# mozack/vdjer

Hardware: AMD Instinct MI355X
Metric: M paired-reads/sec (k-mer build + contig score), IgH 50bp PE (higher is better)
Workload: dtype u8/u64 (2-bit packed bases, integer counts)

## Files before the change

### vdjer_amd/csrc/vdjx_common.h

```cpp
#pragma once

#include <hip/hip_runtime.h>
#include <stdint.h>
#include <stddef.h>
#include <string>
#include <vector>
#include <chrono>
#include <map>
#include <mutex>
#include <utility>

#include "../../include/vdjx.h"
#include "vdjx_env.h"

typedef unsigned long long u64;
typedef unsigned int u32;
typedef unsigned __int128 u128;

#define VDJX_WAVE 64

#define RI_R1 1u
#define RI_RC 2u
#define RI_RCA 4u
#define RI_RCB 8u
#define VDJX_RI_SLOT_WORDS(W) ((W) == 2 ? 4 : 8)
#define RI_TAB_EPOCH_SHIFT 25
#define RI_ENT_NONE 0x3FFFFFFu
#define RI_ENT_MAXCNT 255u
__host__ __device__ inline unsigned long long ri_entry(unsigned y, unsigned z, unsigned fl, unsigned cnt) {
	return (unsigned long long) y | ((unsigned long long) z << 26) | ((unsigned long long) fl << 52) | ((unsigned long long) cnt << 56);
}

void vdjx_set_error(const char* fmt, ...);
inline void vdjx_clear_errors() { (void) hipGetLastError(); }

#define HIP_TRY(expr)                                                                            \
	do {                                                                                         \
		hipError_t e_ = (expr);                                                                  \
		if (e_ != hipSuccess) {                                                                  \
			vdjx_set_error("%s failed: %s (%s:%d)", #expr, hipGetErrorString(e_), __FILE__, __LINE__); \
			return VDJX_EHIP;                                                                    \
		}                                                                                        \
	} while (0)

struct vdjx_prof_entry {
	double ms = 0;
	uint64_t launches = 0;
};

struct vdjx_arena {
	char* base = nullptr;
	size_t reserved = 0, mapped = 0;
	std::vector<std::pair<void*, size_t>> pieces;
	size_t gran = 0;
	int mode = 0;
	struct chunk { char* p; size_t cap; };
	std::vector<chunk> chunks;
	size_t cur = 0;
	size_t used = 0;
	void* alloc(size_t bytes);
	void reset();
	void release(bool for_good = false);
	struct mark_t { size_t cur, used; };
	mark_t mark() const { return {cur, used}; }
	void release_to(mark_t m);
	bool grow(size_t upto);
};

struct vdjx_shard;

#define VDJX_HPIN_BYTES 16384
#define VDJX_HPIN_SYNC_BYTES ((64 * 16 + 2) * 8)
#define VDJX_HPIN_ROOT_RUN 3072
static_assert(VDJX_HPIN_ROOT_RUN * 4 >= VDJX_HPIN_SYNC_BYTES + 64 && VDJX_HPIN_ROOT_RUN * 4 + 4 <= VDJX_HPIN_BYTES, "h_pin layout");

struct vdjx_block_cache {
	struct blk { char* p; size_t cap; };
	std::vector<blk> free_list;
	hipError_t acquire(size_t need, char** out, size_t* cap);
	void release(char* p, size_t cap);
	void drop();
	static void discard(char* p) { if (p) (void) hipFree(p); }
};

struct vdjx_kept {
	void* p = nullptr;
	size_t bytes = 0;
	const bool pinned;
	u32 allocs = 0;
	explicit vdjx_kept(bool pinned_ = false) : pinned(pinned_) {}
	vdjx_kept(const vdjx_kept&) = delete;
	vdjx_kept& operator=(const vdjx_kept&) = delete;
	template <typename T> T* as() const { return (T*) p; }
	hipError_t reserve(size_t need, size_t margin) {
		if (need <= bytes) return hipSuccess;
		release();
		const hipError_t e = pinned ? hipHostMalloc(&p, need + margin, hipHostMallocDefault) : hipMalloc(&p, need + margin);
		if (e != hipSuccess) { p = nullptr; return e; }
		bytes = need + margin;
		allocs++;
		return hipSuccess;
	}
	void release() {
		if (p) (void) (pinned ? hipHostFree(p) : hipFree(p));
		p = nullptr;
		bytes = 0;
	}
};
template <typename T> struct vdjx_buf : vdjx_kept {
	using vdjx_kept::vdjx_kept;
	operator T*() const { return (T*) p; }
	template <typename U> explicit operator U*() const { return (U*) p; }
};
enum vdjx_kept_tag { VDJX_KEPT_INDEX, VDJX_KEPT_RESULT, VDJX_KEPT_OTHER };

struct vdjx_recset {
	vdjx_buf<uint8_t> d_cols;
	bool loaded = false;
	int ncls = 0;
	std::vector<u32> rec[2];
	std::vector<u64> at[2];
	std::vector<u32> len[2];
	size_t given = 0;
};

struct vdjx_ctx {
	int device = 0;
	vdjx_arena arena;
	vdjx_block_cache blocks;
	vdjx_arena shard_arena;
	hipStream_t ri_stream = nullptr;
	hipEvent_t ev_ri_go = nullptr;
	vdjx_arena ri_arena;
	struct vdjx_ri_job* ri_job = nullptr;
	vdjx_shard* live_shard = nullptr;
	hipStream_t stream = nullptr;
	hipStream_t copy_stream = nullptr;
	hipStream_t pairs_stream = nullptr;
	vdjx_buf<void> h_pin{true};
	vdjx_buf<void> d_stage[2];
	hipEvent_t ev_copied[2] = {nullptr, nullptr}, ev_packed[2] = {nullptr, nullptr};
	bool profiling = false;
	std::string prof_only;
	std::vector<std::string> prof_names;
	std::map<std::string, vdjx_prof_entry> prof;
	struct pending_ev { std::string name; hipEvent_t a, b; };
	std::vector<pending_ev> prof_pending;
	std::vector<hipEvent_t> ev_free;
	vdjx_buf<u32> d_vbits, d_jbits;
	bool anchors_loaded = false;
	u32 sub_tuples_set = 0;
	vdjx_buf<u32> d_anchor_tmp;
	vdjx_buf<char> d_vtext;
	vdjx_buf<u32> d_line_off;
	vdjx_buf<u32> d_seed_code;
	vdjx_buf<u32> d_seed_pos;
	size_t n_lines = 0, n_seeds = 0;
	int vk = 0;
	std::vector<u32> h_line_off;
	const vdjx_pool* ri_pool = nullptr;
	vdjx_buf<void> d_ri_tab;
	u32 ri_tab_mask = 0;
	u32 ri_tab_epoch = 0;
	bool ri_canon = false;
	vdjx_buf<u32> d_ri_start;
	vdjx_buf<u32> d_ri_cnt1;
	vdjx_buf<u32> d_ri_recs;
	vdjx_buf<u64> d_ri_csr8;
	vdjx_buf<u32> d_ri_csr_pair;
	vdjx_buf<u32> d_pair_r2;
	vdjx_buf<u32> d_ri_dstart;
	vdjx_buf<u64> d_ri_d8;
	std::vector<std::pair<const char*, size_t>> host_blocks;
	std::mutex host_blocks_mu;
	uint64_t me_key = 0;
	const void* me_src = nullptr;
	vdjx_buf<void> me_pairs;
	vdjx_buf<void> me_hit;
	vdjx_buf<void> wp_buf;
	size_t wp_n = 0;
	std::vector<u64> wp_off;
	std::vector<u32> wp_cnt;
	vdjx_buf<void> me_dense;
	size_t me_gathered_cap = 0;
	std::vector<u64> me_cnt;
	vdjx_buf<void> h_plan{true};
	vdjx_buf<void> h_res{true};
	vdjx_buf<void> me_book;
	size_t me_nsl = 0;
	u32 me_slice_hits = 0;
	hipEvent_t ev_gathered = nullptr;
	hipStream_t up_stream = nullptr;
	hipEvent_t ev_up[5] = {};
	hipEvent_t ev_pairs_copied = nullptr;
	uint32_t root_dp_hint = 0;
	hipEvent_t ev_plan = nullptr;
	bool root_pending = false;
	const vdjx_graph* root_pending_g = nullptr;
	int root_pending_thr = 0;
	uint32_t root_pending_first = 0, root_pending_stride = 1, root_pending_ahead = 0;
	bool root_pending_by_wave = false;
	uint32_t* root_pending_ids = nullptr;
	uint8_t* root_pending_out = nullptr;
	hipEvent_t ev_root_done = nullptr;
	vdjx_buf<char> d_sam_names;
	vdjx_buf<u64> d_sam_noff;
	u32 sam_pairs = 0;
	vdjx_buf<void> d_sam_text;
	vdjx_buf<void> h_sam_text{true};
	vdjx_buf<void> d_sam_keys, d_sam_lens;
	vdjx_buf<void> h_sam_merge{true};
	u32 n_pairs = 0, n_classes = 0;
	vdjx_recset germline, constant, dsegment;
	std::map<std::string, uint64_t> stats;
	template <typename F> void each_kept(F f) {
		vdjx_kept* const index[] = {&d_ri_tab, &d_ri_start, &d_ri_cnt1, &d_ri_recs, &d_ri_csr8, &d_ri_csr_pair, &d_ri_dstart, &d_ri_d8, &d_pair_r2};
		vdjx_kept* const result[] = {&wp_buf, &me_pairs, &me_hit, &me_dense, &me_book, &d_sam_text, &h_sam_text, &d_sam_keys, &d_sam_lens};
		vdjx_kept* const other[] = {&h_pin, &d_stage[0], &d_stage[1], &d_vbits, &d_jbits, &d_anchor_tmp, &d_vtext, &d_line_off, &d_seed_code, &d_seed_pos,
		                            &h_plan, &h_res, &d_sam_names, &d_sam_noff, &h_sam_merge, &germline.d_cols, &constant.d_cols, &dsegment.d_cols};
		for (vdjx_kept* b : index) f(*b, VDJX_KEPT_INDEX);
		for (vdjx_kept* b : result) f(*b, VDJX_KEPT_RESULT);
		for (vdjx_kept* b : other) f(*b, VDJX_KEPT_OTHER);
	}
};

#define VDJX_LONG_W 5
#define VDJX_LONG_M 3
struct vdjx_pool {
	vdjx_ctx* ctx = nullptr;
	int device = 0;
	size_t n_primary = 0, n_records = 0;
	int rl = 0;
	int qstride = 0;
	int W = 2, M = 1, ob = 6;
	bool sym = false;
	char* d_block = nullptr;
	size_t block_cap = 0;
	u64* d_bases = nullptr;
	u64* d_nmask = nullptr;
	u64* d_lowq = nullptr;
	const uint8_t* d_quals = nullptr;
	const uint8_t* d_quals2 = nullptr;
	size_t q_split = ~(size_t) 0;
	u32* pending_bad = nullptr;
};

struct vdjx_graph {
	vdjx_ctx* ctx = nullptr;
	int device = 0;
	int k = 0;
	size_t n = 0, pre_nodes = 0;
	size_t export_bytes = 0;
	char* d_block = nullptr;
	size_t block_cap = 0;
	u64* d_first_inst = nullptr;
	u32 *d_gcnt = nullptr, *d_freq = nullptr, *d_to_ids = nullptr, *d_from_ids = nullptr;
	uint8_t *d_hv = nullptr, *d_hj = nullptr, *d_to_deg = nullptr, *d_from_deg = nullptr;
	char* d_kmers = nullptr;
	u32* d_roots = nullptr;
	size_t n_roots = 0;
};

bool vdjx_ctx_alive(const vdjx_ctx* c);
int vdjx_ri_join(vdjx_ctx* c);
void vdjx_ri_open_gate(vdjx_ctx* c);
bool vdjx_host_block_holds(vdjx_ctx* c, const void* p, size_t bytes);
int vdjx_map_emit_device(vdjx_ctx* c, const char* contigs, size_t n, int len, uint64_t* offsets, const vdjx_pair** d_pairs);

struct vdjx_work {
	vdjx_ctx* c;
	vdjx_arena* ar;
	explicit vdjx_work(vdjx_ctx* ctx) : c(ctx), ar(&ctx->arena) {}
	vdjx_work(vdjx_ctx* ctx, vdjx_arena* arena) : c(ctx), ar(arena) {}
	~vdjx_work() { ar->reset(); }
	template <typename T> hipError_t alloc(T** out, size_t n) {
		*out = (T*) ar->alloc((n ? n : 1) * sizeof(T));
		return *out ? hipSuccess : hipErrorOutOfMemory;
	}
	vdjx_arena::mark_t mark() const { return ar->mark(); }
	void release_to(vdjx_arena::mark_t m) { ar->release_to(m); }
};

struct vdjx_prof_scope {
	vdjx_ctx* c;
	const char* name;
	hipEvent_t a = nullptr, b = nullptr;
	vdjx_prof_scope(vdjx_ctx* ctx, const char* nm);
	~vdjx_prof_scope();
};
void vdjx_prof_collect(vdjx_ctx* ctx, bool force = true);

int vdjx_sort_pairs(vdjx_work& db, hipStream_t st, u64* k_in, u64* k_out, u32* v_in, u32* v_out, u32 n, unsigned end_bit);
int vdjx_sort_pairs_raw(void* tmp, size_t* tmp_bytes, hipStream_t st, u64* k_in, u64* k_out, u32* v_in, u32* v_out, u32 n, unsigned end_bit);

struct vdjx_laps {
	vdjx_ctx* c;
	bool on;
	std::chrono::steady_clock::time_point t;
	explicit vdjx_laps(vdjx_ctx* ctx) : c(ctx) { static const bool e = vdjx_env_set("VDJX_LAPS"); on = e; if (on) t = std::chrono::steady_clock::now(); }
	void mark(const char* name) {
		if (!on) return;
		const auto n = std::chrono::steady_clock::now();
		c->stats[std::string("us_") + name] += (uint64_t) std::chrono::duration_cast<std::chrono::microseconds>(n - t).count();
		t = n;
	}
};

struct vdjx_qrows {
	const uint8_t* a; const uint8_t* b; size_t split; int stride;
	__host__ __device__ inline const uint8_t* row(size_t rec) const { return rec < split ? a + rec * (size_t) stride : b + (rec - split) * (size_t) stride; }
};
__host__ __device__ inline u64 vdjx_mix64(u64 x) {
	u64 z = x + 0x9E3779B97F4A7C15ull;
	z = (z ^ (z >> 30)) * 0xBF58476D1CE4E5B9ull;
	z = (z ^ (z >> 27)) * 0x94D049BB133111EBull;
	return z ^ (z >> 31);
}
__host__ __device__ inline u64 vdjx_mix(u64 lo, u64 hi) {
	u64 x = lo ^ (hi * 0x9E3779B97F4A7C15ull) ^ 0x2545F4914F6CDD1Dull;
	x ^= x >> 32; x *= 0xD6E8FEB86659FD93ull;
	x ^= x >> 32; x *= 0xD6E8FEB86659FD93ull;
	x ^= x >> 32;
	return x;
}

__host__ __device__ inline u64 vdjx_bucket_mix(u64 lo, u64 hi) {
	u32 c = (u32) hi ^ ((u32) (hi >> 32) << 26);
	u32 h = (c ^ (c >> 15)) * 0x9E3779B1u;
	h ^= h >> 15;
	h = (h ^ (u32) lo) * 0x85EBCA6Bu;
	h ^= h >> 13;
	const u32 b = (u32) (lo >> 32);
	h = (h ^ b ^ (b >> 16)) * 0xC2B2AE35u;
	h ^= h >> 16;
	h *= 0x27D4EB2Fu;
	h ^= h >> 15;
	return (u64) h << 32;
}

template <int W>
__device__ inline u64 ri_hash(const u64* __restrict__ w) {
	if (W == 2) return vdjx_mix(w[1], w[0]);
	u64 h = vdjx_mix(w[1], w[0]);
#pragma unroll
	for (int i = 2; i < W; i += 2) h = vdjx_mix(h ^ w[i], i + 1 < W ? w[i + 1] : 0ull);
	return h;
}

__host__ __device__ inline void vdjx_kmer_at(u64 bhi, u64 blo, int rl, int k, int o, u64& khi, u64& klo) {
	u128 b = ((u128) bhi << 64) | blo;
	int sh = 2 * (rl - k - o);
	u128 v = b >> sh;
	if (k < 64) v &= (((u128) 1) << (2 * k)) - 1;
	khi = (u64) (v >> 64);
	klo = (u64) v;
}

__device__ inline void vdjx_wave_lds_fence() {
	__builtin_amdgcn_fence(__ATOMIC_ACQ_REL, "wavefront");
	__builtin_amdgcn_wave_barrier();
}

__device__ inline void vdjx_kmer_at_lane(u64 bhi, u64 blo, int rl, int k, int o, u64& khi, u64& klo) {
	const u32 sh = (u32) (2 * (rl - k - o));
	const u64 big = 0ull - (u64) (sh >> 6);
	const u64 x_lo = (bhi & big) | (blo & ~big), x_hi = bhi & ~big;
	const u32 s = sh & 63u;
	u64 lo = (x_lo >> s) | ((x_hi << 1) << (63u - s));
	u64 hi = x_hi >> s;
	if (k < 32) { lo &= (1ull << (2 * k)) - 1ull; hi = 0; }
	else if (k < 64) hi &= (1ull << (2 * k - 64)) - 1ull;
	khi = hi;
	klo = lo;
}

// ... 224 lines not shown
```

### vdjer_amd/csrc/vdjx_kmer.hip

```cpp
#include "vdjx_common.h"
#include "vdjx_scan.h"
#include "vdjx_part.h"

#include <algorithm>
#include <numeric>
#include <type_traits>
#include <string.h>
#include <stdlib.h>

#define HIST_THREADS 512
#define HIST_BLOCKS 512u
#define LOCAL_SLOTS 2048u
#define K3_SUB_TUPLES g_sub_tuples
__device__ u32 g_sub_tuples = 262144u;
#define NONE32 0xFFFFFFFFu
#define INST_MASK 0x7FFFFFFFu

struct RecView {
	u64 bhi, blo, nm, lq;
};

__device__ inline RecView load_rec(const u64* __restrict__ bases, const u64* __restrict__ nmask,
                                   const u64* __restrict__ lowq, size_t r) {
	RecView v;
	const ulonglong2 b = ((const ulonglong2*) bases)[r];
	v.bhi = b.x; v.blo = b.y;
	v.nm = nmask[r];
	v.lq = lowq ? lowq[r] : 0ull;
	return v;
}

__global__ void k_pick_u32(const u32* __restrict__ src, u32 step, u32 n, u32* __restrict__ out) {
	const u32 i = blockIdx.x * blockDim.x + threadIdx.x;
	if (i < n) out[i] = src[(size_t) i * step];
}

template <typename THI, u32 SLOTS>
__device__ inline int lds_insert(u64* s_klo, THI* s_khi, u64 lo, THI hi, u32 h) {
	const THI EMPTY = (THI) ~(THI) 0, LOCKED = (THI) (EMPTY - 1);
	u32 slot = h & (SLOTS - 1);
	u32 probes = 0;
	while (probes < SLOTS) {
		THI cur = vdjx_peek_acquire(&s_khi[slot]);
		if (cur == EMPTY) {
			THI old = atomicCAS(&s_khi[slot], EMPTY, LOCKED);
			if (old == EMPTY) {
				vdjx_poke(&s_klo[slot], lo);
				vdjx_poke_release(&s_khi[slot], hi);
				return (int) slot;
			}
			cur = old;
			if (cur != LOCKED) cur = vdjx_peek_acquire(&s_khi[slot]);
		}
		if (cur == LOCKED) continue;
		if (cur == hi && vdjx_peek(&s_klo[slot]) == lo) return (int) slot;
		slot = (slot + 1) & (SLOTS - 1);
		probes++;
	}
	return -1;
}

template <typename THI, u32 SLOTS>
__device__ inline int lds_lookup(const u64* s_klo, const THI* s_khi, u64 lo, THI hi, u32 h) {
	const THI EMPTY = (THI) ~(THI) 0;
	u32 slot = h & (SLOTS - 1);
	for (u32 probes = 0; probes < SLOTS; probes++) {
		THI cur = s_khi[slot];
		if (cur == EMPTY) return -1;
		if (cur == hi && s_klo[slot] == lo) return (int) slot;
		slot = (slot + 1) & (SLOTS - 1);
	}
	return -1;
}

#define INST_BITS 38
#define INST_MASK64 ((1ull << INST_BITS) - 1ull)
#define NONE64 0xFFFFFFFFFFFFFFFFull

struct Tup16 {
	u64 lo, x;
	typedef u32 hi_t;
	__device__ inline u64 hi() const { return x >> INST_BITS; }
	__device__ inline u64 inst() const { return x & INST_MASK64; }
	__device__ static inline Tup16 make(u64 lo, u64 hi, u64 inst) { Tup16 t; t.lo = lo; t.x = (hi << INST_BITS) | inst; return t; }
	__device__ static inline Tup16 load(const Tup16* p) { const ulonglong2 v = *(const ulonglong2*) p; Tup16 t; t.lo = v.x; t.x = v.y; return t; }
	__device__ static inline void store(Tup16* p, const Tup16& t) { *(ulonglong2*) p = make_ulonglong2(t.lo, t.x); }
};
struct Tup24 {
	u64 lo, h, i;
	typedef u64 hi_t;
	__device__ inline u64 hi() const { return h; }
	__device__ inline u64 inst() const { return i; }
	__device__ static inline Tup24 make(u64 lo, u64 hi, u64 inst) { Tup24 t; t.lo = lo; t.h = hi; t.i = inst; return t; }
	__device__ static inline Tup24 load(const Tup24* p) { return *p; }
	__device__ static inline void store(Tup24* p, const Tup24& t) { *p = t; }
};

__device__ inline u64 vdjx_clean_offsets(u64 bad, int k, int P) {
	u64 inv = bad;
	int cur = 1;
	while (cur * 2 <= k) { inv |= inv >> cur; cur *= 2; }
	inv |= inv >> (k - cur);
	return ~inv & (P >= 64 ? ~0ull : (1ull << P) - 1ull);
}

#define GL_WAVE_BYTES 3072u

#define GL_ROW_LONG (VDJX_LONG_W + 2)
#define GL_WAVE_BYTES_LONG (64u * GL_ROW_LONG * 8u + 2048u)
struct GateView { u64 bhi, blo, bad; };
__device__ inline GateView load_gate(const u64* __restrict__ bases, const u64* __restrict__ gate, size_t r) {
	GateView v;
	const ulonglong2 b = ((const ulonglong2*) bases)[r];
	v.bhi = b.x; v.blo = b.y;
	v.bad = gate[r];
	return v;
}
__device__ inline vdjx_mask3 load_gate3(const u64* __restrict__ gate, size_t r) {
	vdjx_mask3 b;
	b.w0 = gate[r * VDJX_LONG_M]; b.w1 = gate[r * VDJX_LONG_M + 1]; b.w2 = gate[r * VDJX_LONG_M + 2];
	return b;
}
__device__ inline vdjx_mask3 load_bad3(const u64* __restrict__ nmask, const u64* __restrict__ lowq, size_t r) {
	vdjx_mask3 b;
	b.w0 = nmask[r * VDJX_LONG_M] | (lowq ? lowq[r * VDJX_LONG_M] : 0ull);
	b.w1 = nmask[r * VDJX_LONG_M + 1] | (lowq ? lowq[r * VDJX_LONG_M + 1] : 0ull);
	b.w2 = nmask[r * VDJX_LONG_M + 2] | (lowq ? lowq[r * VDJX_LONG_M + 2] : 0ull);
	return b;
}
__device__ inline void stage_row_long(u64* row, const u64* __restrict__ bases, size_t r) {
#pragma unroll
	for (int w = 0; w < VDJX_LONG_W; w++) row[w] = bases[r * VDJX_LONG_W + w];
	row[VDJX_LONG_W] = 0; row[VDJX_LONG_W + 1] = 0;
}

__device__ inline bool sym_canonical(const ulonglong2 f, int rl, int k, int o, u64& khi, u64& klo) {
	u64 xh, xl, yh, yl;
	vdjx_kmer_at_lane(f.x, f.y, rl, k, o, xh, xl);
	vdjx_kmer_rc(xh, xl, k, yh, yl);
	const bool flip = yh < xh || (yh == xh && yl < xl);
	khi = flip ? yh : xh;
	klo = flip ? yl : xl;
	return flip;
}

template <bool LONG, bool SYM = false>
__global__ __launch_bounds__(HIST_THREADS) void k_gated_hist(const u64* __restrict__ bases, const u64* __restrict__ nmask,
                                                             const u64* __restrict__ lowq, size_t R, int rl, int k, u32 nb_bits,
                                                             size_t rpb, u32* __restrict__ bucket_cnt, u32 dbg_in) {
#ifdef VDJX_ABLATE
	const u32 dbg = dbg_in;
#else
	const u32 dbg = 0u;
#endif
	u32 sink = 0;
	extern __shared__ __attribute__((aligned(16))) u32 hist[];
	const u32 NB = 1u << nb_bits;
	for (u32 i = threadIdx.x; i < NB; i += HIST_THREADS) hist[i] = 0;
	__syncthreads();
	static_assert(!(LONG && SYM), "SYM is the short-read form");
	uint8_t* wv = (uint8_t*) (hist + NB) + (threadIdx.x >> 6) * (LONG ? GL_WAVE_BYTES_LONG : GL_WAVE_BYTES);
	ulonglong2* wb = (ulonglong2*) wv;
	u64* wrow = (u64*) wv;
	uint16_t* wl = (uint16_t*) (wv + (LONG ? 64u * GL_ROW_LONG * 8u : 1024u));
	const u32 lane = threadIdx.x & 63u;
	const size_t r0 = (size_t) blockIdx.x * rpb;
	const size_t r1 = r0 + rpb < R ? r0 + rpb : R;
	const int P = rl - k + 1;
	for (size_t rb = r0; rb < r1; rb += HIST_THREADS) {
		const size_t r = rb + threadIdx.x;
		u64 G = 0;
		vdjx_mask3 bad{~0ull, ~0ull, ~0ull};
		if (r < r1) {
			if (LONG) { bad = load_gate3(lowq, r); stage_row_long(wrow + lane * GL_ROW_LONG, bases, r); }
			else {
				const GateView v = load_gate(bases, lowq, SYM ? 2 * r : r);
				G = vdjx_clean_offsets(v.bad, k, P);
				wb[lane] = make_ulonglong2(v.bhi, v.blo);
			}
		}
		constexpr int LSTEP = 16;
		for (int ob = 0; ob < P; ob += LSTEP) {
			const u32 g = LONG ? vdjx_clean16(bad, ob, k, P) : (u32) (G >> ob) & 0xFFFFu;
			const u32 c = (u32) __popc(g);
			const u32 incl = (u32) vdjx_wave_scan_add((int) c);
			const u32 total = (u32) __builtin_amdgcn_readlane((int) incl, 63);
			if (dbg == 1) { sink += incl; continue; }
			if (!total) continue;
			u32 at = incl - c;
			for (u32 gg = g; gg; gg &= gg - 1) wl[at++] = (uint16_t) ((lane << (LONG ? 8 : 6)) | (u32) (ob + __builtin_ctz(gg)));
			vdjx_wave_lds_fence();
			if (dbg == 2) { sink += wl[lane]; vdjx_wave_lds_fence(); continue; }
			for (u32 i = lane; i < total; i += 64) {
				const u32 e = wl[i];
				u64 khi, klo;
				if (LONG) vdjx_kmer_at_words(wrow + (e >> 8) * GL_ROW_LONG, k, (int) (e & 255u), khi, klo);
				else if (SYM) (void) sym_canonical(wb[e >> 6], rl, k, (int) (e & 63u), khi, klo);
				else {
					const ulonglong2 bb = wb[e >> 6];
					vdjx_kmer_at_lane(bb.x, bb.y, rl, k, (int) (e & 63u), khi, klo);
				}
				if (dbg == 3) { sink += (u32) (vdjx_bucket_mix(klo, khi) >> (64 - nb_bits)); continue; }
				atomicAdd(&hist[(u32) (vdjx_bucket_mix(klo, khi) >> (64 - nb_bits))], 1u);
			}
			vdjx_wave_lds_fence();
		}
	}
	__syncthreads();
	if (dbg) { if (sink == 0x12345u) bucket_cnt[0] = sink; return; }
	for (u32 i = threadIdx.x; i < NB; i += HIST_THREADS) if (hist[i]) atomicAdd(&bucket_cnt[i], hist[i]);
}

template <typename TUP> struct TupBucket {
	u32 shift, mask;
	__device__ inline u32 operator()(const TUP& t) const { return (u32) (vdjx_bucket_mix(t.lo, t.hi()) >> shift) & mask; }
};

#define PARTR_STAGE_BYTES 98304u
template <typename TUP, bool LONG, bool SYM = false>
__global__ __launch_bounds__(PART_THREADS) void k_part_records_g(const u64* __restrict__ bases, const u64* __restrict__ nmask,
                                                                 const u64* __restrict__ lowq, size_t R, u64 rec_base, int rl, int k,
                                                                 u32 shift, u32 nbk, size_t rpb, u32 rr0, u32* __restrict__ gcur,
                                                                 TUP* __restrict__ out) {
	extern __shared__ __attribute__((aligned(16))) uint8_t smem[];
	TUP* stage = (TUP*) smem;
	u32* desc = (u32*) (smem + PARTR_STAGE_BYTES);
	__shared__ part_round pr;
	__shared__ u32 s_n;
	constexpr u32 ROUND = PARTR_STAGE_BYTES / sizeof(TUP);
	constexpr int OB = LONG ? 8 : 6;
	const int P = rl - k + 1;
	const u32 rr_min = ROUND / (u32) P;
	u32 rr = rr0 > rr_min ? rr0 : rr_min;
	const u32 mask = nbk - 1;
	const u32 lane = threadIdx.x & 63u, wave = threadIdx.x >> 6;
	static_assert(!(LONG && SYM), "SYM is the short-read form");
	uint8_t* wv = smem + wave * (LONG ? GL_WAVE_BYTES_LONG : GL_WAVE_BYTES);
	ulonglong2* wb = (ulonglong2*) wv;
	u64* wrow = (u64*) wv;
	uint16_t* wl = (uint16_t*) (wv + (LONG ? 64u * GL_ROW_LONG * 8u : 1024u));
	const size_t r0 = (size_t) blockIdx.x * rpb;
	const size_t r1 = r0 + rpb < R ? r0 + rpb : R;
	size_t rs = r0;
	while (rs < r1) {
		const size_t re = rs + rr < r1 ? rs + rr : r1;
		if (threadIdx.x == 0) s_n = 0;
		pr.begin(nbk);
		for (size_t rb = rs; rb < re; rb += PART_THREADS) {
			const size_t r = rb + threadIdx.x;
			u64 G = 0;
			vdjx_mask3 bad{~0ull, ~0ull, ~0ull};
			if (r < re) {
				if (LONG) { bad = load_gate3(lowq, r); stage_row_long(wrow + lane * GL_ROW_LONG, bases, r); }
				else {
					const GateView v = load_gate(bases, lowq, SYM ? 2 * r : r);
					G = vdjx_clean_offsets(v.bad, k, P);
					wb[lane] = make_ulonglong2(v.bhi, v.blo);
				}
			}
			const u32 loc0 = (u32) (rb - rs) + wave * 64u;
			constexpr int LSTEP = 16;
			for (int ob = 0; ob < P; ob += LSTEP) {
				const u32 g = LONG ? vdjx_clean16(bad, ob, k, P) : (u32) (G >> ob) & 0xFFFFu;
				const u32 c = (u32) __popc(g);
				const u32 incl = (u32) vdjx_wave_scan_add((int) c);
				const u32 total = (u32) __builtin_amdgcn_readlane((int) incl, 63);
				if (!total) continue;
				u32 at = incl - c;
				for (u32 gg = g; gg; gg &= gg - 1) wl[at++] = (uint16_t) ((lane << OB) | (u32) (ob + __builtin_ctz(gg)));
				vdjx_wave_lds_fence();
				u32 dbase = 0;
				if (lane == 0) dbase = atomicAdd(&s_n, total);
				dbase = (u32) __builtin_amdgcn_readlane((int) dbase, 0);
				for (u32 i = lane; i < total; i += 64) {
					const u32 e = wl[i];
					u64 khi, klo;
					if (LONG) vdjx_kmer_at_words(wrow + (e >> 8) * GL_ROW_LONG, k, (int) (e & 255u), khi, klo);
					else if (SYM) (void) sym_canonical(wb[e >> 6], rl, k, (int) (e & 63u), khi, klo);
					else {
						const ulonglong2 bb = wb[e >> 6];
						vdjx_kmer_at_lane(bb.x, bb.y, rl, k, (int) (e & 63u), khi, klo);
					}
					const u32 b = (u32) (vdjx_bucket_mix(klo, khi) >> shift) & mask;
					pr.count(b);
					if (dbase + i < ROUND) desc[dbase + i] = ((loc0 + (e >> OB)) << (OB + 10)) | ((e & ((1u << OB) - 1u)) << 10) | b;
				}
				vdjx_wave_lds_fence();
			}
		}
		__syncthreads();
		if (s_n > ROUND) {
			rr = rr / 2 > rr_min ? rr / 2 : rr_min;
			__syncthreads();
			continue;
		}
		const u32 n = pr.reserve(nbk, gcur);
		for (u32 i = threadIdx.x; i < n; i += PART_THREADS) {
			const u32 d = desc[i];
			const size_t r = rs + (d >> (OB + 10));
			const u32 o = (d >> 10) & ((1u << OB) - 1u);
			u64 khi, klo;
			u64 inst = ((rec_base + (u64) r) << OB) | (u64) o;
			if (LONG) vdjx_kmer_at_words(bases + r * VDJX_LONG_W, k, (int) o, khi, klo);
			else if (SYM) {
				const bool flip = sym_canonical(((const ulonglong2*) bases)[2 * r], rl, k, (int) o, khi, klo);
				inst = flip ? ((rec_base + 2 * (u64) r + 1) << OB) | (u64) (rl - k - (int) o) : ((rec_base + 2 * (u64) r) << OB) | (u64) o;
			} else {
				const ulonglong2 bb = ((const ulonglong2*) bases)[r];
				vdjx_kmer_at_lane(bb.x, bb.y, rl, k, (int) o, khi, klo);
			}
			TUP::store(&stage[pr.slot(d & 1023u)], TUP::make(klo, khi, inst));
		}
		__syncthreads();
		pr.flush(stage, n, out, TupBucket<TUP>{shift, mask});
		rs = re;
	}
}

template <typename TUP>
__global__ __launch_bounds__(512) void k_seg_hist_g(const TUP* __restrict__ in, const u32* __restrict__ seg_start, u32 seg_shift, u32 slices,
                                                    u32 shift, u32 sub_bits, u32* __restrict__ fine_cnt) {
	__shared__ u32 h[PART_MAXB];
	const u32 nbk = 1u << sub_bits;
	for (u32 i = threadIdx.x; i < nbk; i += 512) h[i] = 0;
	__syncthreads();
	size_t t0, t1;
	const u32 seg = part_slice(seg_start, seg_shift, slices, t0, t1);
	for (size_t t = t0 + threadIdx.x; t < t1; t += 512) {
		const TUP x = TUP::load(&in[t]);
		atomicAdd(&h[(u32) (vdjx_bucket_mix(x.lo, x.hi()) >> shift) & (nbk - 1)], 1u);
	}
	__syncthreads();
	for (u32 i = threadIdx.x; i < nbk; i += 512) if (h[i]) atomicAdd(&fine_cnt[((size_t) seg << sub_bits) | i], h[i]);
}

#ifndef RD_THREADS
#define RD_THREADS 768
#define RD_UNR 4
#define RD_WAVES 6
#endif
#define RD_SLOTS 2048u
#define RD_SLOT_BITS 11
#define RD_PQ 4096u
#define RD_LI 512u
#define RD_LROWS 128u
#define RD_MAXLOW 11u
#define ST_CAND 1u
#define ST_MULTI 2u
#define ST_QOK 4u
#define ST_QOK_R 8u
#define ST_ID_SHIFT 8
#define ST_NOID 0xFFFFFFu

struct SurvOutG { u64* lo; u64* hi; u32* gcnt; u64* gfirst; u32* n; u32 cap; u32* n_real; };
#define GC_SHADOW 0x80000000u
#define GC_MASK 0x7FFFFFFFu

__device__ inline bool reads_equal(const u64* __restrict__ bases, const u64* __restrict__ nmask, int rl, u64 a, u64 b) {
	if (rl <= VDJX_SHORT_READ_LEN) {
		const ulonglong2 x = ((const ulonglong2*) bases)[a];
		const ulonglong2 y = ((const ulonglong2*) bases)[b];
		return x.x == y.x && x.y == y.y && nmask[a] == nmask[b];
	}
	u64 d = 0;
#pragma unroll
	for (int w = 0; w < VDJX_LONG_W; w++) d |= bases[a * VDJX_LONG_W + w] ^ bases[b * VDJX_LONG_W + w];
#pragma unroll
	for (int w = 0; w < VDJX_LONG_M; w++) d |= nmask[a * VDJX_LONG_M + w] ^ nmask[b * VDJX_LONG_M + w];
	return d == 0;
}

__device__ inline u32 rd_hash(u64 lo, u64 hi) {
	u32 x = (u32) lo ^ ((u32) (lo >> 32) * 0x9E3779B1u) ^ (((u32) hi ^ (u32) (hi >> 32) * 0x27D4EB2Fu) * 0x85EBCA6Bu);
	x ^= x >> 15; x *= 0xC2B2AE35u; x ^= x >> 13;
	return x;
}

__device__ inline u32 rd_count_min(u32* cnt, u64* mn, u32 idx, u64 val, bool active) {
	u32 c0 = 0;
	const u64 act = __ballot(active);
	if (act) {
		const int leader = __ffsll((long long) act) - 1;
		const u32 lidx = (u32) __builtin_amdgcn_readlane((int) idx, leader);
		const bool same = active && idx == lidx;
		const u64 m = __ballot(same);
		if (__popcll(m) >= 8) {
			const u32 hi_min = vdjx_wave_min(same ? (u32) (val >> 32) : 0xFFFFFFFFu);
			const u32 lo_min = vdjx_wave_min(same && (u32) (val >> 32) == hi_min ? (u32) val : 0xFFFFFFFFu);
			u32 old = 0;
			if (__lane_id() == leader) {
				old = atomicAdd(&cnt[lidx], (u32) __popcll(m));
				atomicMin((unsigned long long*) &mn[lidx], ((unsigned long long) hi_min << 32) | lo_min);
			}
			old = (u32) __builtin_amdgcn_readlane((int) old, leader);
			if (same) c0 = old + (u32) __popcll(m & ((1ull << __lane_id()) - 1ull));
			active = active && !same;
		}
	}
	if (active) { c0 = atomicAdd(&cnt[idx], 1u); atomicMin((unsigned long long*) &mn[idx], (unsigned long long) val); }
	return c0;
}

__global__ __launch_bounds__(1024) void k_bucket_order(const u32* __restrict__ bucket_start, u32 NB, u32* __restrict__ order) {
	__shared__ u32 cls_cnt[33], cls_at[33];
	if (threadIdx.x < 33) cls_cnt[threadIdx.x] = 0;
	__syncthreads();
	for (u32 b = threadIdx.x; b < NB; b += 1024) {
		const u32 n = bucket_start[b + 1] - bucket_start[b];
		atomicAdd(&cls_cnt[n ? 32u - (u32) __builtin_clz(n) : 0u], 1u);
	}
	__syncthreads();
	if (threadIdx.x == 0) { u32 at = 0; for (int cl = 32; cl >= 0; cl--) { cls_at[cl] = at; at += cls_cnt[cl]; } }
	__syncthreads();
	for (u32 b = threadIdx.x; b < NB; b += 1024) {
		const u32 n = bucket_start[b + 1] - bucket_start[b];
		order[atomicAdd(&cls_at[n ? 32u - (u32) __builtin_clz(n) : 0u], 1u)] = b;
	}
}

template <typename TUP, bool SYM = false>
__global__ __launch_bounds__(RD_THREADS, sizeof(TUP) == 16 ? RD_WAVES : RD_WAVES / 2) void k_gated_reduce(const TUP* __restrict__ tup, const u32* __restrict__ bucket_start,
                                                             const u64* __restrict__ bases, const u64* __restrict__ nmask,
                                                             vdjx_qrows quals, int rl, int ob, int k, u64 rec_base,
                                                             u32 mf, u32 cmin, u32 mqq, u32 tlow, SurvOutG so,
                                                             u64* __restrict__ g_distinct, u32* __restrict__ g_err, u32 dbg_in,
                                                             const u32* __restrict__ order) {
#ifdef VDJX_ABLATE
	const u32 dbg = dbg_in;
#else
	const u32 dbg = dbg_in == 9u ? 9u : 0u;
#endif
	typedef typename TUP::hi_t THI;
	__shared__ u64 s_klo[RD_SLOTS];
	__shared__ THI s_khi[RD_SLOTS];
	__shared__ u64 s_first[RD_SLOTS];
	__shared__ u32 s_cnt[RD_SLOTS], s_state[RD_SLOTS];
	__shared__ u32 pq[RD_PQ];
	__shared__ u64 low_inst[RD_LI];
	__shared__ u32 low_n[RD_LROWS];
	__shared__ unsigned short low_slot[RD_LROWS];
	__shared__ u32 s_over, s_ndist, s_nlow, s_npq, s_nsurv, s_base, s_nreal;
	const THI EMPTY = (THI) ~(THI) 0;
	const u32 b = order ? order[blockIdx.x] : blockIdx.x;
	const u32 base = bucket_start[b];
	const u32 n = bucket_start[b + 1] - base;
	const u32 tid = threadIdx.x;
	if (n == 0) return;
	const TUP* T = tup + base;
	const u32 om = (1u << ob) - 1u;
	const u32 per_low = tlow > 1 ? (tlow - 1 < RD_MAXLOW ? tlow - 1 : RD_MAXLOW) : 1;
	const u32 lrows = RD_LI / per_low < RD_LROWS ? RD_LI / per_low : RD_LROWS;
	u32 S = 1;
	while ((u64) S * K3_SUB_TUPLES < n) S <<= 1;
	u32 ndist_total = 0;
	bool verify = S > 1;
	for (;;) {
		if (tid == 0) { s_over = 0; s_ndist = 0; }
		__syncthreads();
		for (u32 s = 0; s < S; s++) {
			for (u32 i = tid; i < RD_SLOTS; i += RD_THREADS) { s_khi[i] = EMPTY; s_cnt[i] = 0; s_first[i] = NONE64; s_state[i] = 0; }
			if (tid == 0) { s_nlow = 0; s_npq = (n >> (32 - RD_SLOT_BITS) || dbg == 9) ? RD_PQ + 1 : 0; s_nsurv = 0; s_nreal = 0; }
			__syncthreads();
			for (u32 t0 = 0; t0 < n; t0 += RD_UNR * RD_THREADS) {
				TUP r_t[RD_UNR];
#pragma unroll
				for (int j = 0; j < RD_UNR; j++) {
					const u32 t = t0 + j * RD_THREADS + tid;
					if (t < n) r_t[j] = TUP::load(&T[t]);
				}
#pragma unroll
				for (int j = 0; j < RD_UNR; j++) {
					const u32 t = t0 + j * RD_THREADS + tid;
					int slot = -1;
					if (t < n) {
						const u32 h = rd_hash(r_t[j].lo, r_t[j].hi());
						if (!(S > 1 && ((h >> 12) & (S - 1)) != s)) {
							slot = lds_insert<THI, RD_SLOTS>(s_klo, s_khi, r_t[j].lo, (THI) r_t[j].hi(), h);
							if (slot < 0) s_over = 1;
						}
					}
					const bool live = slot >= 0 && !verify;
					const u64 inst = r_t[j].inst();
					const u32 c0 = rd_count_min(s_cnt, s_first, (u32) (live ? slot : 0), inst, live);
					bool list = false;
					if (live) {
						u32 st = vdjx_peek(&s_state[slot]);
						if (!(st & ST_MULTI)) {
							const u64 f = vdjx_peek(&s_first[slot]);
							if (f != NONE64 && (f >> ob) != (inst >> ob)) {
								const u32 o1 = (u32) inst & om, o0 = (u32) f & om;
								const u32 d = o1 > o0 ? o1 - o0 : o0 - o1;
								if (d && d < (u32) k && !vdjx_kmer_has_period(r_t[j].hi(), r_t[j].lo, k, d)) { atomicOr(&s_state[slot], ST_MULTI); st |= ST_MULTI; }
							}
						}
						list = !((st & ST_MULTI) && c0 + 1 >= tlow);
					}
					const u32 qi = vdjx_wave_inc(&s_npq, list);
					if (list && qi < RD_PQ) pq[qi] = (t << RD_SLOT_BITS) | (u32) slot;
				}
			}
			__syncthreads();
			if (s_over || verify) { if (s_over) break; continue; }
			if (dbg == 1) return;
			for (u32 i = tid; i < RD_SLOTS; i += RD_THREADS) {
				if (s_khi[i] == EMPTY) continue;
				atomicAdd(&s_ndist, SYM ? 2u : 1u);
				const u32 c = s_cnt[i];
				if (c >= cmin) s_state[i] = (s_state[i] & ST_MULTI) | ST_CAND | ((c < tlow ? atomicAdd(&s_nlow, 1u) : ST_NOID) << ST_ID_SHIFT);
			}
			__syncthreads();
			const u32 nlow = s_nlow;
			const bool listed = s_npq <= RD_PQ;
			const u32 nscan = listed ? s_npq : n;
			for (u32 l0 = 0; l0 == 0 || l0 < nlow; l0 += lrows) {
				for (u32 i = tid; i < RD_LROWS; i += RD_THREADS) low_n[i] = 0;
				__syncthreads();
				for (u32 e = tid; e < nscan; e += RD_THREADS) {
					u32 slot, t;
					TUP x;
					if (listed) {
						slot = pq[e] & (RD_SLOTS - 1); t = pq[e] >> RD_SLOT_BITS;
						if (!(vdjx_peek(&s_state[slot]) & ST_CAND)) continue;
						x = TUP::load(&T[t]);
					} else {
						x = TUP::load(&T[e]);
						const u32 h = rd_hash(x.lo, x.hi());
						if (S > 1 && ((h >> 12) & (S - 1)) != s) continue;
						const int sl = lds_lookup<THI, RD_SLOTS>(s_klo, s_khi, x.lo, (THI) x.hi(), h);
						if (sl < 0) continue;
						slot = (u32) sl;
					}
					const u32 st = vdjx_peek(&s_state[slot]);
					if (!(st & ST_CAND)) continue;
					const u64 inst = x.inst(), fi = s_first[slot];
					const u32 lid = st >> ST_ID_SHIFT;
					if (lid != ST_NOID && lid >= l0 && lid < l0 + lrows) {
						const u32 pos = atomicAdd(&low_n[lid - l0], 1u);
						if (pos < per_low) low_inst[(lid - l0) * per_low + pos] = inst;
						low_slot[lid - l0] = (unsigned short) slot;
					}
					if (l0 == 0 && !(st & ST_MULTI) && (inst >> ob) != (fi >> ob)) {
						const u32 o1 = (u32) inst & om, o0 = (u32) fi & om;
						const u32 d = o1 > o0 ? o1 - o0 : o0 - o1;
						if ((d && d < (u32) k && !vdjx_kmer_has_period(x.hi(), x.lo, k, d))
						    || !reads_equal(bases, nmask, rl, (inst >> ob) - rec_base, (fi >> ob) - rec_base)) atomicOr(&s_state[slot], ST_MULTI);
					}
				}
				__syncthreads();
				if (dbg == 4) return;
				const u32 rows = nlow - l0 < lrows ? nlow - l0 : lrows;
				const u32 lane = tid & 63u;
				for (u32 r = tid >> 6; r < (nlow ? rows : 0u); r += RD_THREADS / 64) {
					const u32 slot = low_slot[r], cnt = low_n[r];
					const u64 fi = s_first[slot];
					u32 qv[RD_MAXLOW];
#pragma unroll
					for (u32 i = 0; i < RD_MAXLOW; i++) {
						qv[i] = 33u;
						if (i < cnt && i < per_low) {
							const u64 inst = low_inst[r * per_low + i];
							const uint8_t* q = quals.row((inst >> ob) - rec_base) + (inst == fi ? 0u : (u32) inst & om);
							if (lane < (u32) k) qv[i] = q[lane];
						}
					}
					u32 sum = 0;
#pragma unroll
					for (u32 i = 0; i < RD_MAXLOW; i++) sum += (u32) (uint8_t) (qv[i] - 33u);
					const bool lowq = lane < (u32) k && sum < mqq;
					if (!__ballot(lowq) && lane == 0) atomicOr(&s_state[slot], ST_QOK);
					if (SYM) {
						u64 fr = NONE64;
#pragma unroll
						for (u32 i = 0; i < RD_MAXLOW; i++)
							if (i < cnt && i < per_low) { const u64 m = vdjx_inst_mirror(low_inst[r * per_low + i], ob, rl, k); fr = m < fr ? m : fr; }
#pragma unroll
						for (u32 i = 0; i < RD_MAXLOW; i++) {
							qv[i] = 33u;
							if (i < cnt && i < per_low) {
								const u64 inst = vdjx_inst_mirror(low_inst[r * per_low + i], ob, rl, k);
								const uint8_t* q = quals.row((inst >> ob) - rec_base) + (inst == fr ? 0u : (u32) inst & om);
								if (lane < (u32) k) qv[i] = q[lane];
							}
						}
						u32 sum_r = 0;
#pragma unroll
						for (u32 i = 0; i < RD_MAXLOW; i++) sum_r += (u32) (uint8_t) (qv[i] - 33u);
						const bool lowq_r = lane < (u32) k && sum_r < mqq;
						if (!__ballot(lowq_r) && lane == 0) atomicOr(&s_state[slot], ST_QOK_R);
					}
				}
				__syncthreads();
			}
			if (dbg == 5) return;
			for (u32 i = tid; i < RD_SLOTS; i += RD_THREADS) {
				const u32 st = s_state[i];
				bool keep = false, keep_r = false;
				if (st & ST_CAND) {
					const u32 craw = s_cnt[i];
					const u32 c = craw > 32765u ? 32765u : craw;
					keep = c >= mf && (st & ST_MULTI) && (craw >= tlow || (st & ST_QOK));
					if (SYM) keep_r = c >= mf && (st & ST_MULTI) && (craw >= tlow || (st & ST_QOK_R));
				}
				if (SYM) {
					s_state[i] = (keep || keep_r) ? (atomicAdd(&s_nsurv, 2u) << 2) | (u32) keep | ((u32) keep_r << 1) : NONE32;
					if (keep || keep_r) atomicAdd(&s_nreal, (u32) keep + (u32) keep_r);
				} else s_state[i] = keep ? atomicAdd(&s_nsurv, 1u) : NONE32;
			}
			__syncthreads();
			if (tid == 0) { s_base = s_nsurv ? atomicAdd(so.n, s_nsurv) : 0; if (SYM && s_nreal) atomicAdd(so.n_real, s_nreal); }
			__syncthreads();
			for (u32 i = tid; i < RD_SLOTS; i += RD_THREADS) {
				if (s_state[i] == NONE32) continue;
				u32 pos = s_base + (SYM ? s_state[i] >> 2 : s_state[i]);
				const u32 cgo = s_cnt[i] > 32765u ? 32765u : s_cnt[i];
				if (pos < so.cap) {
					so.lo[pos] = s_klo[i];
					so.hi[pos] = (u64) s_khi[i];
					so.gcnt[pos] = cgo | (SYM && !(s_state[i] & 1u) ? GC_SHADOW : 0u);
					so.gfirst[pos] = s_first[i];
				}
				if (SYM) {
					pos += 1u;
					if (pos < so.cap) {
						u64 rh, rlo;
						vdjx_kmer_rc((u64) s_khi[i], s_klo[i], k, rh, rlo);
						so.lo[pos] = rlo;
						so.hi[pos] = rh;
						so.gcnt[pos] = cgo | (!(s_state[i] & 2u) ? GC_SHADOW : 0u);
						so.gfirst[pos] = vdjx_inst_mirror(s_first[i], ob, rl, k);
					}
				}
			}
			__syncthreads();
		}
		__syncthreads();
		if (s_over) {
			if (S >= (1u << 20)) { if (tid == 0) atomicAdd(g_err, 1u); break; }
			S <<= 1;
			verify = true;
			__syncthreads();
			continue;
		}
		if (verify) { verify = false; __syncthreads(); continue; }
		ndist_total = s_ndist;
		break;
	}
	if (tid == 0) atomicAdd(&g_distinct[(b & 63u) * 16u], (u64) ndist_total);
}

struct Partial { u64 lo, hi; u32 cg, h; u64 fg; };
#define PART_FLAG 0x80000000u
#define CNT_CAP 32765u
struct PartialS { u64 lo, hic, fgh, fgr; };
static_assert(sizeof(PartialS) == sizeof(Partial), "vdjx_shard_record_bytes(0) is one number");
#define PS_H_BITS 26
#define PS_MAX_SPLIT (1u << (PS_H_BITS - 12))
__device__ inline u64 ps_hi(const PartialS& p) { return p.hic & 0xFFFFFFFFFFFFull; }
__device__ inline u32 ps_cg(const PartialS& p) { const u32 c = (u32) (p.hic >> 48); return (c & 0x7FFFu) | ((c & 0x8000u) ? PART_FLAG : 0u); }
__device__ inline u64 ps_fg(const PartialS& p) { return p.fgh & INST_MASK64; }
__device__ inline u32 ps_h(const PartialS& p) { return (u32) (p.fgh >> INST_BITS); }
#define NEED_SEQ 1u
#define NEED_Q 2u
#define PID_MASK 0x3FFFFFFFu
#define REPLY_KQ 52
#define REPLY_BYTES 408

#define LG_THREADS 768
#define LG_UNR 4
#define LG_FLAG 0x80000000u
#define LG_NOLIST 0x7FFFFFFFu
template <typename TUP, bool SYM = false>
__global__ __launch_bounds__(LG_THREADS, sizeof(TUP) == 16 ? 6 : 3) void k_gated_local(const TUP* __restrict__ tup, const u32* __restrict__ bucket_start,
                                                            const u64* __restrict__ bases, const u64* __restrict__ nmask, u64 rec_base, int k, int rl, int ob,
                                                            u32 tlow, Partial* __restrict__ sparse_g, u32* __restrict__ sparse_ref,
                                                            u32* __restrict__ nd_g, u64* __restrict__ low_inst, u32* __restrict__ g_err,
                                                            const u32* __restrict__ order) {
	typedef typename TUP::hi_t THI;
	const size_t obase = (size_t) bucket_start[order ? order[blockIdx.x] : blockIdx.x];
	__shared__ u64 s_klo[LOCAL_SLOTS];
	__shared__ THI s_khi[LOCAL_SLOTS];
	__shared__ u64 s_mg[LOCAL_SLOTS];
	__shared__ u32 s_cg[LOCAL_SLOTS], s_st[LOCAL_SLOTS];
	__shared__ u32 pq[RD_PQ];
	__shared__ u32 s_ng, s_nlow, s_over, s_npq;
	static_assert(LOCAL_SLOTS == (1u << RD_SLOT_BITS), "list entries carry the slot in RD_SLOT_BITS bits");
	const THI EMPTY = (THI) ~(THI) 0;
	const u32 b = order ? order[blockIdx.x] : blockIdx.x;
	const u32 base = bucket_start[b];
	const u32 n = bucket_start[b + 1] - base;
	const u32 tid = threadIdx.x;
	const u32 om = (1u << ob) - 1u;
	if (n == 0) { if (tid == 0) nd_g[b] = 0; return; }
	const TUP* T = tup + base;
	u32 S = 1;
	while ((u64) S * K3_SUB_TUPLES < n) S <<= 1;
	for (;;) {
		if (tid == 0) { s_ng = 0; s_nlow = 0; s_over = 0; }
		for (u32 s = 0; s < S; s++) {
			for (u32 i = tid; i < LOCAL_SLOTS; i += LG_THREADS) { s_khi[i] = EMPTY; s_cg[i] = 0; s_mg[i] = NONE64; s_st[i] = 0; }
			if (tid == 0) s_npq = n >> (32 - RD_SLOT_BITS) ? RD_PQ + 1 : 0;
			__syncthreads();
			for (u32 t0 = 0; t0 < n; t0 += LG_UNR * LG_THREADS) {
				TUP r_t[LG_UNR];
#pragma unroll
				for (int j = 0; j < LG_UNR; j++) {
					const u32 t = t0 + j * LG_THREADS + tid;
					if (t < n) r_t[j] = TUP::load(&T[t]);
				}
#pragma unroll
				for (int j = 0; j < LG_UNR; j++) {
					const u32 t = t0 + j * LG_THREADS + tid;
					int slot = -1;
					if (t < n) {
						const u32 h = rd_hash(r_t[j].lo, r_t[j].hi());
						if (!(S > 1 && ((h >> 12) & (S - 1)) != s)) {
							slot = lds_insert<THI, LOCAL_SLOTS>(s_klo, s_khi, r_t[j].lo, (THI) r_t[j].hi(), h);
							if (slot < 0) s_over = 1;
						}
					}
					const bool live = slot >= 0;
					const u64 inst = r_t[j].inst();
					const u32 c0 = rd_count_min(s_cg, s_mg, (u32) (live ? slot : 0), inst, live);
					bool list = false;
					if (live) {
						u32 st = vdjx_peek(&s_st[slot]);
						if (!(st & LG_FLAG)) {
							const u64 f = vdjx_peek(&s_mg[slot]);
							if (f != NONE64 && (f >> ob) != (inst >> ob)) {
								const u32 o1 = (u32) inst & om, o0 = (u32) f & om;
								const u32 d = o1 > o0 ? o1 - o0 : o0 - o1;
								if (d && d < (u32) k && !vdjx_kmer_has_period(r_t[j].hi(), r_t[j].lo, k, d)) { atomicOr(&s_st[slot], LG_FLAG); st |= LG_FLAG; }
							}
						}
						list = !((st & LG_FLAG) && c0 + 1 >= tlow);
					}
					const u32 qi = vdjx_wave_inc(&s_npq, list);
					if (list && qi < RD_PQ) pq[qi] = (t << RD_SLOT_BITS) | (u32) slot;
				}
			}
			__syncthreads();
			if (s_over) break;
			for (u32 i = tid; i < LOCAL_SLOTS; i += LG_THREADS) {
				const u32 cg = s_cg[i];
				s_st[i] = (s_st[i] & LG_FLAG) | ((cg && cg < tlow) ? atomicAdd(&s_nlow, cg) : LG_NOLIST);
			}
			__syncthreads();
			const bool listed = s_npq <= RD_PQ;
			const u32 nscan = listed ? s_npq : n;
			for (u32 e = tid; e < nscan; e += LG_THREADS) {
				u32 slot;
				TUP x;
				if (listed) {
					slot = pq[e] & (LOCAL_SLOTS - 1);
					const u32 st0 = vdjx_peek(&s_st[slot]);
					if ((st0 & LG_NOLIST) == LG_NOLIST && (st0 & LG_FLAG)) continue;
					x = TUP::load(&T[pq[e] >> RD_SLOT_BITS]);
				} else {
					x = TUP::load(&T[e]);
					const u32 h = rd_hash(x.lo, x.hi());
					if (S > 1 && ((h >> 12) & (S - 1)) != s) continue;
					const int sl = lds_lookup<THI, LOCAL_SLOTS>(s_klo, s_khi, x.lo, (THI) x.hi(), h);
					if (sl < 0) continue;
					slot = (u32) sl;
				}
				const u32 st = vdjx_peek(&s_st[slot]);
				const u32 loff = st & LG_NOLIST;
				const u64 inst = x.inst();
				u32 cg = vdjx_peek(&s_cg[slot]);
				if (loff != LG_NOLIST) {
					cg &= 0xFFFFu;
					low_inst[base + loff + (atomicAdd(&s_cg[slot], 0x10000u) >> 16)] = inst;
				}
				if (cg < 2 || (st & LG_FLAG)) continue;
				const u64 fi = s_mg[slot];
				const u64 rec = (inst >> ob) - rec_base, frec = (fi >> ob) - rec_base;
				if (rec != frec) {
					const u32 o1 = (u32) inst & om, o0 = (u32) fi & om;
					const u32 d = o1 > o0 ? o1 - o0 : o0 - o1;
					if (d && d < (u32) k && !vdjx_kmer_has_period(x.hi(), x.lo, k, d)) atomicOr(&s_st[slot], LG_FLAG);
					else if (!reads_equal(bases, nmask, rl, rec, frec)) atomicOr(&s_st[slot], LG_FLAG);
				}
			}
			__syncthreads();
			for (u32 i = tid; i < LOCAL_SLOTS; i += LG_THREADS) {
				if (s_khi[i] == EMPTY) continue;
				const u32 st = s_st[i];
				const u32 loff = st & LG_NOLIST;
				const u32 cg = loff != LG_NOLIST ? s_cg[i] & 0xFFFFu : s_cg[i];
				Partial p;
				p.lo = s_klo[i]; p.hi = (u64) s_khi[i];
				p.fg = s_mg[i];
				p.cg = (cg > CNT_CAP ? CNT_CAP : cg) | ((st & LG_FLAG) ? PART_FLAG : 0u);
				p.h = rd_hash(p.lo, p.hi);
				const u32 gi = atomicAdd(&s_ng, 1u);
				sparse_ref[obase + gi] = loff != LG_NOLIST ? base + loff : NONE32;
				if (SYM) {
					u64 fr = vdjx_inst_mirror(p.fg, ob, rl, k);
					if (loff != LG_NOLIST)
						for (u32 j = 0; j < cg; j++) { const u64 m = vdjx_inst_mirror(low_inst[base + loff + j], ob, rl, k); fr = m < fr ? m : fr; }
					PartialS q;
					q.lo = p.lo;
					q.hic = p.hi | ((u64) ((p.cg & 0x7FFFu) | ((p.cg & PART_FLAG) ? 0x8000u : 0u)) << 48);
					q.fgh = p.fg | ((u64) (p.h & ((1u << PS_H_BITS) - 1u)) << INST_BITS);
					q.fgr = fr;
					((PartialS*) sparse_g)[obase + gi] = q;
				} else sparse_g[obase + gi] = p;
			}
			__syncthreads();
		}
		if (!s_over) break;
		S <<= 1;
		if (S > (1u << 20)) { if (tid == 0) atomicAdd(g_err, 1u); break; }
		__syncthreads();
	}
	if (tid == 0) nd_g[b] = s_over ? 0 : s_ng;
}

__global__ __launch_bounds__(256) void k_compact_partials(const Partial* __restrict__ sparse, const u32* __restrict__ sparse_ref,
                                                          const u32* __restrict__ bucket_start, const u32* __restrict__ nd,
                                                          const u32* __restrict__ dstart, Partial* __restrict__ dense, u32* __restrict__ dense_ref,
                                                          const u32* __restrict__ scan, int ob, bool sym) {
	const u32 b = blockIdx.x;
	const u64* src = (const u64*) (sparse + (size_t) bucket_start[b]);
	u64* dst = (u64*) (dense + dstart[b]);
	const u32 m = nd[b];
	const u64 om = (1ull << ob) - 1ull;
	for (u32 i = threadIdx.x; i < m * 4; i += 256) {
		u64 v = src[i];
		if (scan) {
			if ((i & 3u) == 3u) v = ((u64) scan[v >> ob] << ob) | (v & om);
			else if (sym && (i & 3u) == 2u) { const u64 f = v & INST_MASK64; v = (v & ~INST_MASK64) | ((u64) scan[f >> ob] << ob) | (f & om); }
		}
		dst[i] = v;
	}
	for (u32 i = threadIdx.x; i < m; i += 256) dense_ref[dstart[b] + i] = sparse_ref[(size_t) bucket_start[b] + i];
}

__global__ __launch_bounds__(1024) void k_seg_offsets(const u32* __restrict__ seg_cnt, const u32* __restrict__ src_base, u32 G, u32 NBo,
                                                      u32* __restrict__ seg_off) {
	__shared__ u32 tmp[16];
	const u32 s = blockIdx.x;
	const u32* cnt = seg_cnt + (size_t) s * NBo;
	u32* off = seg_off + (size_t) s * (NBo + 1);
	const u32 per = (NBo + 1023) / 1024;
	const u32 lo = threadIdx.x * per;
	const u32 hi = lo + per < NBo ? lo + per : NBo;
	u32 sum = 0;
	for (u32 i = lo; i < hi; i++) sum += cnt[i];
	u32 total;
	u32 run = src_base[s] + vdjx_block_scan(sum, tmp, total);
	for (u32 i = lo; i < hi; i++) { off[i] = run; run += cnt[i]; }
	if (threadIdx.x == 1023) off[NBo] = src_base[s] + total;
}

struct PendOut { u64* lo; u64* hi; u32* cg; u64* mg; u32* need; u32* n; u32 cap; u64* mgr; };

#define MERGE_THREADS 512
#define MERGE_SLOTS 2048u
#define MS_FLAG 0x10000u
__device__ inline bool ms_open(u32 st) { return st != NONE32 && (st >> 30) != 0u; }
template <typename THI, bool SYM = false>
__global__ __launch_bounds__(MERGE_THREADS) void k_bucket_merge(const Partial* __restrict__ recv, const u32* __restrict__ seg_off,
                                                                u32 MG, u32 G, u32 NBo,
                                                                const u32* __restrict__ src_base, u32 s_mult, u32 cmin, u32 tlow,
                                                                SurvOutG so, PendOut po,
                                                                uint2* __restrict__ queries, u32* __restrict__ g_nq,
                                                                u64* __restrict__ g_distinct, u32* __restrict__ g_err, int k) {
	__shared__ u64 s_klo[MERGE_SLOTS];
	__shared__ THI s_khi[MERGE_SLOTS];
	__shared__ u64 s_mg[MERGE_SLOTS];
	__shared__ u64 s_mgr[SYM ? MERGE_SLOTS : 1];
	__shared__ u32 s_cg[MERGE_SLOTS], s_st[MERGE_SLOTS];
	__shared__ u32 s_over, s_ndist, s_total, s_ns, s_np, s_sbase, s_pbase;
	__shared__ u32 s_pend[MERGE_SLOTS / 32];
	const THI EMPTY = (THI) ~(THI) 0;
	const u32 b = blockIdx.x;
	const u32 tid = threadIdx.x;
	if (tid == 0) {
		u32 tot = 0;
		for (u32 s = 0; s < G; s++) tot += seg_off[(size_t) s * (NBo + 1) + (b + 1) * MG] - seg_off[(size_t) s * (NBo + 1) + b * MG];
		s_total = tot;
	}
	__syncthreads();
	const u32 total = s_total;
	if (total == 0) return;
	u32 S = 1;
	while ((u64) S * (MERGE_SLOTS * 3 / 4) < total) S <<= 1;
	S *= s_mult;
	if (SYM && S > PS_MAX_SPLIT) { if (tid == 0) atomicAdd(g_err, 1u); return; }
	auto key_of = [&](u32 at, u64& lo, u64& hi, u32& h) {
		if (SYM) { const PartialS q = ((const PartialS*) recv)[at]; lo = q.lo; hi = ps_hi(q); h = ps_h(q); }
		else { const Partial q = recv[at]; lo = q.lo; hi = q.hi; h = q.h; }
	};
	{
		if (tid == 0) { s_over = 0; s_ndist = 0; }
		for (u32 sp = 0; sp < S; sp++) {
			for (u32 i = tid; i < MERGE_SLOTS; i += MERGE_THREADS) { s_khi[i] = EMPTY; s_cg[i] = 0; s_mg[i] = NONE64; s_st[i] = 0; if (SYM) s_mgr[i] = NONE64; }
			__syncthreads();
			for (u32 s = 0; s < G; s++) {
				const u32 off = seg_off[(size_t) s * (NBo + 1) + b * MG], cnt = seg_off[(size_t) s * (NBo + 1) + (b + 1) * MG] - off;
				for (u32 i = tid; i < cnt; i += MERGE_THREADS) {
					u64 lo, hi, fg, fgr = 0;
					u32 h, cg;
					if (SYM) { const PartialS q = ((const PartialS*) recv)[off + i]; lo = q.lo; hi = ps_hi(q); h = ps_h(q); cg = ps_cg(q); fg = ps_fg(q); fgr = q.fgr; }
					else { const Partial q = recv[off + i]; lo = q.lo; hi = q.hi; h = q.h; cg = q.cg; fg = q.fg; }
					if (((h >> 12) & (S - 1)) != sp) continue;
					const int slot = lds_insert<THI, MERGE_SLOTS>(s_klo, s_khi, lo, (THI) hi, h);
					if (slot < 0) { s_over = 1; continue; }
					atomicAdd(&s_cg[slot], cg & ~PART_FLAG);
					atomicMin((unsigned long long*) &s_mg[slot], (unsigned long long) fg);
					if (SYM) atomicMin((unsigned long long*) &s_mgr[slot], (unsigned long long) fgr);
					atomicAdd(&s_st[slot], 1u | ((cg & PART_FLAG) ? MS_FLAG : 0u));
				}
			}
			__syncthreads();
			if (s_over) break;
			if (tid == 0) { s_ns = 0; s_np = 0; }
			for (u32 i = tid; i < MERGE_SLOTS / 32; i += MERGE_THREADS) s_pend[i] = 0;
			__syncthreads();
			for (u32 i0 = 0; i0 < MERGE_SLOTS; i0 += MERGE_THREADS) {
				const u32 i = i0 + tid;
				u32 need = 0, cg = 0;
				bool live = s_khi[i] != EMPTY;
				if (live) {
					cg = s_cg[i];
					atomicAdd(&s_ndist, SYM ? 2u : 1u);
					if (cg < cmin) live = false;
				}
				const u32 st0 = s_st[i];
				if (live && !(st0 >> 16)) {
					if ((st0 & 0xFFFFu) < 2) live = false;
					else need |= NEED_SEQ;
				}
				if (live && cg < tlow) need |= NEED_Q;
				if (live && !need) s_st[i] = atomicAdd(&s_ns, SYM ? 2u : 1u);
				else s_st[i] = NONE32;
				if (live && need) {
					s_st[i] = atomicAdd(&s_np, 1u) | (need << 30);
					const u32 hm = rd_hash(s_klo[i], (u64) s_khi[i]) & (MERGE_SLOTS - 1);
					atomicOr(&s_pend[hm >> 5], 1u << (hm & 31));
				}
			}
			__syncthreads();
			if (tid == 0) {
				s_sbase = s_ns ? atomicAdd(so.n, s_ns) : 0;
				s_pbase = s_np ? atomicAdd(po.n, s_np) : 0;
			}
			__syncthreads();
			for (u32 i0 = 0; i0 < MERGE_SLOTS; i0 += MERGE_THREADS) {
				const u32 i = i0 + tid;
				const u32 st = s_st[i];
				if (st != NONE32 && !(st >> 30)) {
					const u32 pos = s_sbase + st;
					if (pos < so.cap) {
						const u32 cg = s_cg[i];
						so.lo[pos] = s_klo[i]; so.hi[pos] = (u64) s_khi[i];
						so.gcnt[pos] = cg > CNT_CAP ? CNT_CAP : cg; so.gfirst[pos] = s_mg[i];
					}
					if (SYM && pos + 1 < so.cap) {
						const u32 cg = s_cg[i];
						u64 rh, rlo;
						vdjx_kmer_rc((u64) s_khi[i], s_klo[i], k, rh, rlo);
						so.lo[pos + 1] = rlo; so.hi[pos + 1] = rh;
						so.gcnt[pos + 1] = cg > CNT_CAP ? CNT_CAP : cg; so.gfirst[pos + 1] = s_mgr[i];
					}
				} else if (st != NONE32) {
					const u32 need = st >> 30;
					const u32 pid = s_pbase + (st & PID_MASK);
					if (pid < po.cap) {
						po.lo[pid] = s_klo[i]; po.hi[pid] = (u64) s_khi[i];
						po.cg[pid] = s_cg[i]; po.mg[pid] = s_mg[i];
						if (SYM) po.mgr[pid] = s_mgr[i];
						po.need[pid] = need;
					}
					s_st[i] = pid | (need << 30);
				}
			}
			__syncthreads();
			for (u32 s = 0; s < G; s++) {
				const u32 off = seg_off[(size_t) s * (NBo + 1) + b * MG], cnt = seg_off[(size_t) s * (NBo + 1) + (b + 1) * MG] - off;
				if (tid == 0) s_ns = 0;
				__syncthreads();
				u32 mine = 0;
				for (u32 i = tid; i < cnt; i += MERGE_THREADS) {
					u64 lo, hi;
					u32 h;
					key_of(off + i, lo, hi, h);
					if (((h >> 12) & (S - 1)) != sp) continue;
					if (!((s_pend[(h & (MERGE_SLOTS - 1)) >> 5] >> (h & 31)) & 1u)) continue;
					const int slot = lds_lookup<THI, MERGE_SLOTS>(s_klo, s_khi, lo, (THI) hi, h);
					if (slot >= 0 && ms_open(s_st[slot])) mine++;
				}
// ... 652 lines not shown
		const size_t r = rb + threadIdx.x;
		walk_row(std::true_type{}, SYM ? 2 * r : r, r < r1, 0, make_ulonglong2(0ull, 0ull), 0ull);
		while (qn >= 64) walk_queued(64);
	}
	if (qn) walk_queued(qn);
	if (have_blk) for (u32 i = fill + (u32) lane; i < blk_items; i += 64) raw[blk + i] = IT_HOLE;
#ifdef WALK_STATS
	if ((dbg & 32u) && lane == 0) {
		atomicAdd(&g_cursor[1], (unsigned long long) st_rows); atomicAdd(&g_cursor[2], (unsigned long long) st_rounds); atomicAdd(&g_cursor[3], (unsigned long long) st_filter);
		atomicAdd(&g_cursor[4], (unsigned long long) st_lookup); atomicAdd(&g_cursor[5], (unsigned long long) st_chain); atomicAdd(&g_cursor[6], (unsigned long long) st_items);
	}
#endif
	__syncthreads();
	for (u32 i = threadIdx.x; i < n_ranges; i += WALK_THREADS) if (hist[i]) atomicAdd(&range_cnt[i], hist[i]);
}

static_assert(IT_HOLE == PART_HOLE, "the holes of the walk's blocks are what the partition drops");
struct ItemRange {
	ItemFmt f;
	u32 range_shift, mask;
	__device__ inline u32 operator()(u64 x) const { return (it_scat(f, it_surv(f, x)) >> range_shift) & mask; }
};

#define RC_THREADS 1024
#define RC_UNR 4
template <typename IT> struct RcNone;
template <> struct RcNone<u32> { static constexpr u32 v = 0xFFFFFFFFu; };
template <> struct RcNone<u64> { static constexpr u64 v = 0xFFFFFFFFFFFFFFFFull; };
__device__ inline void rc_min(u32* p, u32 v) { atomicMin(p, v); }
__device__ inline void rc_min(u64* p, u64 v) { atomicMin((unsigned long long*) p, (unsigned long long) v); }

#define RC_CS 17u
#define RC_MS 77u
__device__ inline u32 rc_win(u32 k, u32 s) { return 31u + ((0x261B0E00u >> (8u * k)) & 0xFFu) + s - 1u; }
template <u32 SB, typename IT>
__global__ __launch_bounds__(RC_THREADS) void k_recount(const u64* __restrict__ items, const u32* __restrict__ range_start, ItemFmt f, u32 ns, u64 rec_base, int ob,
                                                        const u32* __restrict__ fbw, u32* __restrict__ ucnt, u64* __restrict__ ufirst, u64* __restrict__ in_first,
                                                        unsigned long long* __restrict__ n_inst) {
	__shared__ u32 c[SB / 16 * RC_CS];
	__shared__ IT mv[SB / 16 * RC_MS];
	__shared__ IT ef[SB * 4];
	__shared__ u32 fbl[SB / 16];
	__shared__ unsigned long long tot;
	constexpr IT NONE = RcNone<IT>::v;
	const u32 b = blockIdx.x;
	const u32 s0 = b * SB;
	const u32 nb = (ns + 15u) >> 4;
	for (u32 i = threadIdx.x; i < SB / 16 * RC_CS; i += RC_THREADS) c[i] = 0;
	for (u32 i = threadIdx.x; i < SB / 16 * RC_MS; i += RC_THREADS) mv[i] = NONE;
	for (u32 i = threadIdx.x; i < SB * 4; i += RC_THREADS) ef[i] = NONE;
	for (u32 i = threadIdx.x; i < SB / 16; i += RC_THREADS) {
		const u32 sb = (s0 >> 4) + i;
		const u32 blk = (sb * f.inv) & f.bmask;
		fbl[i] = sb <= f.bmask && blk < nb ? fbw[blk] : 0u;
	}
	if (threadIdx.x == 0) tot = 0;
	__syncthreads();
	const u32 i0 = range_start[b], i1 = range_start[b + 1];
	const u32 iend = i0 + (i1 - i0 + RC_THREADS * RC_UNR - 1) / (RC_THREADS * RC_UNR) * (RC_THREADS * RC_UNR);
	for (u32 ib = i0 + threadIdx.x; ib < iend; ib += RC_THREADS * RC_UNR) {
		u64 xs[RC_UNR];
#pragma unroll
		for (int u = 0; u < RC_UNR; u++) { const u32 i = ib + (u32) u * RC_THREADS; xs[u] = i < i1 ? items[i] : IT_HOLE; }
#pragma unroll
		for (int u = 0; u < RC_UNR; u++) {
			const u64 x = xs[u];
			const bool live = x != IT_HOLE;
			const u32 p = it_surv(f, x);
			const u32 len = live ? it_len(f, x) : 1u;
			const u32 sl = live ? it_scat(f, p) - s0 : 0u;
			const u32 a = sl & 15u, e = a + len - 1u;
			const u64 inst = x & IT_INST_MASK;
			const bool shaped = live && (a == 0u || e == 15u);
			const u32 cb = (sl >> 4) * RC_CS, mb = (sl >> 4) * RC_MS;
			const u32 slot = mb + (a == 0u ? e : 15u + a);
			const IT val = (IT) (inst + 15u - a);
			bool mine = shaped;
			const u64 act = __ballot(shaped);
			if (act) {
				const int leader = __ffsll((long long) act) - 1;
				const u32 lslot = (u32) __builtin_amdgcn_readlane((int) slot, leader);
				const bool same = shaped && slot == lslot;
				const u64 m = __ballot(same);
				if (__popcll(m) >= 8) {
					const u64 v64 = inst + 15u - a;
					const u32 hi_min = vdjx_wave_min(same ? (u32) (v64 >> 32) : 0xFFFFFFFFu);
					const u32 lo_min = vdjx_wave_min(same && (u32) (v64 >> 32) == hi_min ? (u32) v64 : 0xFFFFFFFFu);
					if (__lane_id() == leader) {
						const u32 n = (u32) __popcll(m);
						atomicAdd(&c[cb + e], n);
						if (a) atomicAdd(&c[cb + a - 1u], 0u - n);
						rc_min(&mv[lslot], (IT) (((u64) hi_min << 32) | lo_min));
					}
					mine = shaped && !same;
				}
			}
			if (live && (mine || !shaped)) {
				atomicAdd(&c[cb + e], 1u);
				if (a) atomicAdd(&c[cb + a - 1u], 0xFFFFFFFFu);
			}
			if (mine) rc_min(&mv[slot], val);
			if (live && !shaped) {
				const u32 k = 31u - (u32) __builtin_clz(len), w = 1u << k;
				rc_min(&mv[mb + rc_win(k, a)], val);
				if (len != w) rc_min(&mv[mb + rc_win(k, e + 1u - w)], val);
			}
			if (live && ((x >> 37) & 1ull)) {
				IT* ep = &ef[sl * 4 + (u32) ((x >> 35) & 3ull)];
				if (vdjx_peek(ep) > (IT) inst) rc_min(ep, (IT) inst);
			}
		}
	}
	__syncthreads();
	const u64 add = rec_base << ob;
	u32 my_cnt = 0;
	for (u32 i = threadIdx.x; i < SB; i += RC_THREADS) {
		const u32 sb = (s0 + i) >> 4;
		const u32 blk = (sb * f.inv) & f.bmask;
		const u32 x = i & 15u, p = (blk << 4) | x;
		if (sb > f.bmask || blk >= nb || p >= ns) continue;
		const u32 cbase = (i >> 4) * RC_CS, mbase = (i >> 4) * RC_MS;
		u32 cc = 0;
		IT mm = NONE;
		IT me = NONE;
		for (u32 e = x; e < 16; e++) { cc += c[cbase + e]; const IT t = mv[mbase + e]; mm = t < mm ? t : mm; if (x) me = t < me ? t : me; }
		for (u32 a = 1; a <= x; a++) { const IT t = mv[mbase + 15 + a]; mm = t < mm ? t : mm; if (a < x) me = t < me ? t : me; }
#pragma unroll
		for (u32 k = 0; k < 4; k++) {
			const u32 w = 1u << k;
			const u32 lo = x >= w ? x - w + 1u : 1u, hi = x < 15u - w ? x : 15u - w;
			for (u32 s = lo ? lo : 1u; s <= hi; s++) { const IT t = mv[mbase + rc_win(k, s)]; mm = t < mm ? t : mm; if (s < x) me = t < me ? t : me; }
		}
		my_cnt += cc;
		ucnt[p] = cc;
		ufirst[p] = mm == NONE ? NONE64 : (u64) mm - 15u + x + add;
		IT e4[4] = {ef[i * 4], ef[i * 4 + 1], ef[i * 4 + 2], ef[i * 4 + 3]};
		if (x && me != NONE) {
			const u32 pa = (fbl[i >> 4] >> (2 * (x - 1))) & 3u;
			const IT t = (IT) (me - 15u + x);
			if (t < e4[pa]) e4[pa] = t;
		}
		for (u32 q = 0; q < 4; q++) in_first[(size_t) p * 4 + q] = e4[q] == NONE ? NONE64 : (u64) e4[q] + add;
	}
	if (my_cnt) atomicAdd(&tot, (unsigned long long) my_cnt);
	__syncthreads();
	if (threadIdx.x == 0 && tot) atomicAdd(n_inst, tot);
}

__global__ void k_count_unseen(const u64* __restrict__ ufirst, u32 n, u32* __restrict__ out) {
	const u32 i = blockIdx.x * blockDim.x + threadIdx.x;
	const bool un = i < n && ufirst[i] == NONE64;
	const u64 m = __ballot(un);
	if (m && __lane_id() == 0) atomicAdd(out, (u32) __popcll(m));
}

__global__ void k_edges_from_in(SurvTable t, u32 n, int k, const u64* __restrict__ in_first, u32* __restrict__ in_from,
                                u64* __restrict__ edge_first, u32* __restrict__ edge_to) {
	const u32 e = blockIdx.x * blockDim.x + threadIdx.x;
	if (e >= n * 4u) return;
	const u64 fs = in_first[e];
	if (fs == NONE64) { in_from[e] = NONE32; return; }
	const u32 v = e >> 2, a = e & 3u;
	const ulonglong2 kk = t.skey[v];
	const u128 kv = ((u128) kk.y << 64) | kk.x;
	const u128 ku = (kv >> 2) | ((u128) a << (2 * (k - 1)));
	const int u = surv_lookup2(t, (u64) ku, (u64) (ku >> 64));
	in_from[e] = u >= 0 ? (u32) u : NONE32;
	if (u >= 0) {
		const u32 oe = (u32) u * 4u + ((u32) kk.x & 3u);
		edge_first[oe] = fs;
		edge_to[oe] = v;
	}
}

struct SurvRec { u64 lo, hi; u32 gcnt, pad; u64 gfirst; };

__global__ void k_surv_pack(const u64* __restrict__ lo, const u64* __restrict__ hi, const u32* __restrict__ gcnt,
                            const u64* __restrict__ gfirst, u32 n, SurvRec* __restrict__ out) {
	u32 i = blockIdx.x * blockDim.x + threadIdx.x;
	if (i >= n) return;
	SurvRec r{lo[i], hi[i], gcnt[i], 0u, gfirst[i]};
	out[i] = r;
}

__global__ void k_surv_unpack(const SurvRec* __restrict__ in, u32 n, u64* __restrict__ lo, u64* __restrict__ hi, u32* __restrict__ gcnt,
                              u64* __restrict__ gfirst, u32* __restrict__ n_real) {
	u32 i = blockIdx.x * blockDim.x + threadIdx.x;
	const bool in_range = i < n;
	SurvRec r{0, 0, GC_SHADOW, 0, 0};
	if (in_range) {
		r = in[i];
		lo[i] = r.lo; hi[i] = r.hi; gcnt[i] = r.gcnt; gfirst[i] = r.gfirst;
	}
	(void) vdjx_wave_inc(n_real, in_range && !(r.gcnt & GC_SHADOW));
}

struct NodeOut {
	u64* first_inst; u32* gcnt; u32* freq; uint8_t* hv; uint8_t* hj; u64* klo; u64* khi; char* kmers;
	uint8_t* to_deg; u32* to_ids; uint8_t* from_deg; u32* from_ids;
};

__global__ void k_rank_keys(const u64* __restrict__ ufirst, const u32* __restrict__ gcnt, u32 n, u64* __restrict__ key, u32* __restrict__ idx) {
	const u32 i = blockIdx.x * blockDim.x + threadIdx.x;
	if (i < n) { key[i] = (gcnt[i] & GC_SHADOW) ? NONE64 : ufirst[i]; idx[i] = i; }
}
__global__ void k_rank_scatter(const u64* __restrict__ key, const u32* __restrict__ idx, u32 n, u32* __restrict__ rank) {
	const u32 j = blockIdx.x * blockDim.x + threadIdx.x;
	if (j >= n) return;
	const u32 i = idx[j];
	rank[i] = key[j] == NONE64 ? i : j;
}

__global__ __launch_bounds__(256) void k_root_count(const uint8_t* __restrict__ from_deg, u32 n, u32* __restrict__ block_cnt) {
	__shared__ u32 cnt;
	if (threadIdx.x == 0) cnt = 0;
	__syncthreads();
	const u32 i = blockIdx.x * 256 + threadIdx.x;
	const bool r = i < n && from_deg[i] == 0;
	const u64 b = __ballot(r);
	if ((threadIdx.x & 63) == 0 && b) atomicAdd(&cnt, (u32) __popcll(b));
	__syncthreads();
	if (threadIdx.x == 0) block_cnt[blockIdx.x] = cnt;
}

__global__ __launch_bounds__(256) void k_root_list(const uint8_t* __restrict__ from_deg, u32 n, const u32* __restrict__ block_start,
                                                   u32* __restrict__ roots) {
	__shared__ u32 wave_cnt[4];
	const u32 i = blockIdx.x * 256 + threadIdx.x;
	const bool r = i < n && from_deg[i] == 0;
	const u64 b = __ballot(r);
	const u32 w = threadIdx.x >> 6, lane = threadIdx.x & 63;
	if (lane == 0) wave_cnt[w] = (u32) __popcll(b);
	__syncthreads();
	u32 base = block_start[blockIdx.x];
	for (u32 j = 0; j < w; j++) base += wave_cnt[j];
	if (r) roots[base + (u32) __popcll(b & ((1ull << lane) - 1))] = i;
}

__device__ inline void sort4_desc64(u64 (&f)[4], u32 (&id)[4]) {
#define CSW(a, b) { const bool sw = kk[a] < kk[b]; if (sw) { u64 t = kk[a]; kk[a] = kk[b]; kk[b] = t; u32 u = id[a]; id[a] = id[b]; id[b] = u; } }
	u64 kk[4];
	for (int i = 0; i < 4; i++) kk[i] = f[i] == NONE64 ? 0ull : f[i] + 1;
	CSW(0, 1) CSW(2, 3) CSW(0, 2) CSW(1, 3) CSW(1, 2)
	for (int i = 0; i < 4; i++) f[i] = kk[i] ? kk[i] - 1 : NONE64;
#undef CSW
}

__global__ void k_node_emit2(const u64* __restrict__ s_lo, const u64* __restrict__ s_hi, const u32* __restrict__ s_gcnt,
                             const u32* __restrict__ s_ucnt, const u64* __restrict__ s_ufirst, const uint8_t* __restrict__ hv,
                             const uint8_t* __restrict__ hj, const u32* __restrict__ rank, const u64* __restrict__ edge_first,
                             const u32* __restrict__ edge_to, const u64* __restrict__ in_first, const u32* __restrict__ in_from,
                             u32 n, int k, NodeOut o) {
	const u32 s = blockIdx.x * blockDim.x + threadIdx.x;
	if (s >= n) return;
	if (s_gcnt[s] & GC_SHADOW) return;
	const u32 r = rank[s];
	o.first_inst[r] = s_ufirst[s];
	o.gcnt[r] = s_gcnt[s];
	o.freq[r] = s_ucnt[s] > 32765u ? 32765u : s_ucnt[s];
	o.hv[r] = hv[s];
	o.hj[r] = hj[s];
	const u128 key = ((u128) s_hi[s] << 64) | s_lo[s];
	for (int j = 0; j < k; j++) {
		const u32 b = (u32) (key >> (2 * (k - 1 - j))) & 3u;
		o.kmers[(size_t) r * k + j] = b == 0 ? 'A' : (b == 1 ? 'T' : (b == 2 ? 'C' : 'G'));
	}
	u64 f[4];
	u32 id[4];
	for (int e = 0; e < 4; e++) {
		f[e] = edge_first[(size_t) s * 4 + e];
		if (f[e] != NONE64 && (s_gcnt[edge_to[(size_t) s * 4 + e]] & GC_SHADOW)) f[e] = NONE64;
		id[e] = f[e] != NONE64 ? rank[edge_to[(size_t) s * 4 + e]] + 1 : 0;
	}
	sort4_desc64(f, id);
	u32 deg = 0;
	for (int e = 0; e < 4; e++) { o.to_ids[(size_t) r * 4 + e] = f[e] != NONE64 ? id[e] : 0; deg += f[e] != NONE64; }
	o.to_deg[r] = (uint8_t) deg;
	for (int e = 0; e < 4; e++) {
		f[e] = in_first[(size_t) s * 4 + e];
		if (f[e] != NONE64 && (in_from[(size_t) s * 4 + e] == NONE32 || (s_gcnt[in_from[(size_t) s * 4 + e]] & GC_SHADOW))) f[e] = NONE64;
		id[e] = f[e] != NONE64 ? rank[in_from[(size_t) s * 4 + e]] + 1 : 0;
	}
	sort4_desc64(f, id);
	deg = 0;
	for (int e = 0; e < 4; e++) { o.from_ids[(size_t) r * 4 + e] = f[e] != NONE64 ? id[e] : 0; deg += f[e] != NONE64; }
	o.from_deg[r] = (uint8_t) deg;
}

namespace {

struct PersistAlloc {
	vdjx_ctx* c;
	explicit PersistAlloc(vdjx_ctx* ctx) : c(ctx) {}
	template <typename T> hipError_t alloc(T** out, size_t n) {
		*out = (T*) c->shard_arena.alloc((n ? n : 1) * sizeof(T));
		return *out ? hipSuccess : hipErrorOutOfMemory;
	}
	vdjx_arena::mark_t mark() const { return c->shard_arena.mark(); }
	void release_to(vdjx_arena::mark_t m) { c->shard_arena.release_to(m); }
};

struct PoolView { const u64* bases; const u64* nmask; vdjx_qrows quals; int rl; int ob; };

template <typename TUP> struct GTuples {
	TUP* t = nullptr;
	u32* bucket_start = nullptr;
	u32 NB = 0, N = 0;
};

struct SurvivorsG {
	u64 *lo = nullptr, *hi = nullptr, *gfirst = nullptr, *ufirst = nullptr;
	u32 *gcnt = nullptr, *ucnt = nullptr;
	u32 n = 0, n_real = 0;
	u64 ndist = 0;
};

inline u32 ceil_log2_u64(u64 x) { u32 b = 0; while ((1ull << b) < x) b++; return b; }

static bool sync_debug() { static const bool on = vdjx_env_set("VDJX_SYNC_DEBUG"); return on; }
static void dbg_sync(vdjx_ctx* c, const char* what) {
	if (!sync_debug()) return;
	const hipError_t e = hipStreamSynchronize(c->stream);
	fprintf(stderr, "[vdjx] %s: %s\n", what, hipGetErrorString(e));
}

struct GatedHist { u32 HB = 0, NBH = 0, N = 0; u32* hstart = nullptr; bool sym = false; };
static bool build_sym(const vdjx_pool* pool, int k) {
	return pool->sym && pool->W == 2 && (k & 1) && pool->n_records % 2 == 0;
}
static bool sym_walk_wanted() { static const bool on = !vdjx_env_set("VDJX_NO_SYM_WALK"); return on; }
static size_t gated_bucket_default() { static const size_t v = (size_t) vdjx_env_num("VDJX_GATED_BUCKET", 3072, 1, 1ll << 32); return v; }
template <typename A>
int stage_gated_hist(vdjx_ctx* c, A& db, const vdjx_pool* pool, int k, size_t per_bucket, u64 geometry_instances, GatedHist* gh, bool sym = false) {
	hipStream_t st = c->stream;
	const size_t R = sym ? pool->n_records / 2 : pool->n_records;
	const int P = pool->rl - k + 1;
	const u64 NI = geometry_instances ? geometry_instances : (u64) R * (u64) P;
	const size_t per = per_bucket ? per_bucket : gated_bucket_default();
	const u32 hb_max = pool->W > 2 ? 14u : 15u;
	u32 HB = ceil_log2_u64((NI + per - 1) / per);
	HB = std::max(8u, std::min(hb_max, HB));
	const u32 NBH = 1u << HB;
#ifdef VDJX_ABLATE
	static const u32 hist_dbg = (u32) vdjx_env_num("VDJX_HIST_DBG", 0, 0, 4);
#else
	constexpr u32 hist_dbg = 0;
#endif
	u32 nblk = (u32) std::min<size_t>(HIST_BLOCKS, (R + 4095) / 4096);
	if (nblk == 0) nblk = 1;
	size_t rpb = (R + nblk - 1) / nblk;
	u32 *hcnt, *hstart;
	HIP_TRY(db.alloc(&hcnt, NBH));
	HIP_TRY(db.alloc(&hstart, NBH + 1));
	HIP_TRY(hipMemsetAsync(hcnt, 0, (size_t) NBH * 4, st));
	const bool lng = pool->W > 2;
	const size_t lds_hist = (size_t) NBH * 4 + (HIST_THREADS / 64) * (lng ? GL_WAVE_BYTES_LONG : GL_WAVE_BYTES);
	HIP_TRY(hipFuncSetAttribute((const void*) k_gated_hist<false>, hipFuncAttributeMaxDynamicSharedMemorySize, (int) lds_hist));
	HIP_TRY(hipFuncSetAttribute((const void*) k_gated_hist<true>, hipFuncAttributeMaxDynamicSharedMemorySize, (int) lds_hist));
	HIP_TRY(hipFuncSetAttribute((const void*) k_gated_hist<false, true>, hipFuncAttributeMaxDynamicSharedMemorySize, (int) lds_hist));
	{
		vdjx_prof_scope ps(c, "k_gated_hist");
		if (lng) hipLaunchKernelGGL(k_gated_hist<true>, dim3(nblk), dim3(HIST_THREADS), lds_hist, st, pool->d_bases, pool->d_nmask, pool->d_lowq, R, pool->rl, k, HB, rpb, hcnt, hist_dbg);
		else if (sym) hipLaunchKernelGGL((k_gated_hist<false, true>), dim3(nblk), dim3(HIST_THREADS), lds_hist, st, pool->d_bases, pool->d_nmask, pool->d_lowq, R, pool->rl, k, HB, rpb, hcnt, hist_dbg);
		else hipLaunchKernelGGL(k_gated_hist<false>, dim3(nblk), dim3(HIST_THREADS), lds_hist, st, pool->d_bases, pool->d_nmask, pool->d_lowq, R, pool->rl, k, HB, rpb, hcnt, hist_dbg);
	}
	dbg_sync(c, "k_gated_hist");
	vdjx_scan_one(st, hcnt, NBH, hstart);
	HIP_TRY(hipMemcpyAsync(c->h_pin, hstart + NBH, 4, hipMemcpyDeviceToHost, st));
	HIP_TRY(hipStreamSynchronize(st));
	HIP_TRY(hipGetLastError());
#ifdef VDJX_ABLATE
	if (hist_dbg) return VDJX_ESTATE;
#endif
	const u32 N = *(const u32*) c->h_pin;
	c->stats["gated_instances"] = sym ? 2ull * N : N;
	gh->HB = HB; gh->NBH = NBH; gh->N = N; gh->hstart = hstart; gh->sym = sym;
	return VDJX_OK;
}

template <typename TUP, typename A>
int stage_gated_cut(vdjx_ctx* c, A& db, const vdjx_pool* pool, u64 rec_base, int k, size_t per_bucket, u64 geometry_instances, const GatedHist& gh, GTuples<TUP>* out) {
	hipStream_t st = c->stream;
	const bool sym = gh.sym;
	const size_t R = sym ? pool->n_records / 2 : pool->n_records;
	const int P = pool->rl - k + 1;
	const size_t per = per_bucket ? per_bucket : gated_bucket_default();
	const u32 hb_max = pool->W > 2 ? 14u : 15u;
	const bool lng = pool->W > 2;
	const u32 HB = gh.HB, NBH = gh.NBH, N = gh.N;
	u32* hstart = gh.hstart;
	size_t rpb;
	out->N = N;
	const u64 Ng = geometry_instances ? geometry_instances : (u64) N;
	static const size_t refine = (size_t) vdjx_env_num("VDJX_REFINE_TUPLES", 4096, 1, 1ll << 32);
	u32 T = 8;
	while (T < HB && ((u64) per << T) < Ng) T++;
	u32 extra = 0;
	const size_t refine_at = per_bucket ? std::max<size_t>(per_bucket, refine / 2) : refine;
	if (T == HB && HB == hb_max && Ng / NBH > refine_at) {
		extra = 1;
		while (extra < 5 && (Ng >> extra) / NBH > refine_at) extra++;
	}
	const u32 Tt = T + extra;
	const u32 NBt = 1u << Tt;
	HIP_TRY(db.alloc(&out->t, (size_t) N + 1));
	constexpr u32 stage_tuples = PARTR_STAGE_BYTES / (u32) sizeof(TUP);
	constexpr u32 lds_partr = PARTR_STAGE_BYTES + stage_tuples * 4;
	u32 cbits = Tt, fbits = 0;
	if (Tt > 10) { cbits = extra ? Tt - 10 : 8; fbits = Tt - cbits; }
	const u32 NBc = 1u << cbits;
	u32 nblk2 = (u32) std::min<size_t>(1024, (R + 2047) / 2048);
	if (nblk2 == 0) nblk2 = 1;
	rpb = (R + nblk2 - 1) / nblk2;
	u32* gcur;
	HIP_TRY(db.alloc(&gcur, NBc));
	TUP* l1 = out->t;
	if (fbits) HIP_TRY(db.alloc(&l1, (size_t) N + 1));
	{
		vdjx_prof_scope ps(c, "k_part_records");
		const u64 NIl = (u64) R * (u64) P;
		u64 rr = N ? (u64) stage_tuples * 3 / 4 * NIl / ((u64) N * (u64) P) : 1u << 16;
		rr = std::max<u64>(PART_THREADS, std::min<u64>(rr / PART_THREADS * PART_THREADS, lng ? 1u << 14 : 1u << 16));
		auto* part_records = lng ? k_part_records_g<TUP, true> : sym ? k_part_records_g<TUP, false, true> : k_part_records_g<TUP, false>;
		HIP_TRY(part_launch(st, part_records, nblk2, lds_partr, hstart, NBc, HB - cbits, gcur, l1, pool->d_bases, pool->d_nmask, pool->d_lowq, R, rec_base,
		                    pool->rl, k, 64 - cbits, NBc, rpb, (u32) rr));
	}
	dbg_sync(c, "k_part_records");
	u32* tstart;
	HIP_TRY(db.alloc(&tstart, NBt + 1));
	out->NB = NBt;
	out->bucket_start = tstart;
	constexpr u32 slices = PART_SLICES;
	if (extra) {
		u32* fine_cnt;
		HIP_TRY(db.alloc(&fine_cnt, NBt));
		HIP_TRY(hipMemsetAsync(fine_cnt, 0, (size_t) NBt * 4, st));
		vdjx_prof_scope ps(c, "k_seg_hist");
		hipLaunchKernelGGL(k_seg_hist_g<TUP>, dim3(NBc * slices), dim3(512), 0, st, l1, hstart, HB - cbits, slices, 64 - Tt, fbits, fine_cnt);
		vdjx_scan_one(st, fine_cnt, NBt, tstart);
	} else {
		hipLaunchKernelGGL(k_pick_u32, dim3((NBt + 1 + 255) / 256), dim3(256), 0, st, hstart, 1u << (HB - Tt), NBt + 1, tstart);
	}
	if (fbits) {
		u32* gcur2;
		HIP_TRY(db.alloc(&gcur2, NBt));
		vdjx_prof_scope ps(c, "k_part_tuples");
		HIP_TRY(part_launch(st, k_part<TUP, TupBucket<TUP>, part_segs>, NBc * slices, PART_LDS_BYTES, tstart, NBt, 0u, gcur2, out->t,
		                    l1, part_segs{hstart, HB - cbits, slices, fbits}, TupBucket<TUP>{64 - Tt, (1u << fbits) - 1u}));
	}
	return VDJX_OK;
}

template <typename TUP, typename A>
int stage_gated_partition(vdjx_ctx* c, A& db, const vdjx_pool* pool, u64 rec_base, int k, size_t per_bucket, u64 geometry_instances, GTuples<TUP>* out, bool sym = false) {
	GatedHist gh;
	int rc = stage_gated_hist(c, db, pool, k, per_bucket, geometry_instances, &gh, sym);
	if (rc) return rc;
	return stage_gated_cut<TUP>(c, db, pool, rec_base, k, per_bucket, geometry_instances, gh, out);
}

static int set_sub_tuples(vdjx_ctx* c) {
	static const u32 sub = (u32) vdjx_env_num("VDJX_SUB_TUPLES", 262144, 1, 0xFFFFFFFFll);
	if (c->sub_tuples_set != sub) {
		HIP_TRY(hipMemcpyToSymbolAsync(HIP_SYMBOL(g_sub_tuples), &sub, 4, 0, hipMemcpyHostToDevice, c->stream));
		c->sub_tuples_set = sub;
	}
	return VDJX_OK;
}
template <typename TUP, typename A>
int bucket_order(vdjx_ctx* c, A& db, const GTuples<TUP>& t, u32** order) {
	*order = nullptr;
	if (t.NB < 1024) return VDJX_OK;
	HIP_TRY(db.alloc(order, t.NB));
	hipLaunchKernelGGL(k_bucket_order, dim3(1), dim3(1024), 0, c->stream, t.bucket_start, t.NB, *order);
	return VDJX_OK;
}

template <typename TUP, typename A>
int stage_gated_reduce(vdjx_ctx* c, A& db, const GTuples<TUP>& t, const PoolView& pv, u64 rec_base, int k, int mf, int mq, SurvivorsG* sv, bool sym = false) {
	hipStream_t st = c->stream;
	int rc = set_sub_tuples(c);
	if (rc) return rc;
	if (mq >= 255) mq = 254;
	const u32 mqq = (u32) (mq < 0 ? 0 : (mq > 214 ? 214 : mq));
	const u32 tlow = 1 + (mqq + 19) / 20;
	const u32 cmin = (u32) std::max(mf, 2);
	const u32 mfu = (u32) std::max(mf, 0);
	const u32 cap = (sym ? t.N : t.N / 2) + 16;
	u32 *g_err, *n_surv;
	u64* g_distinct;
	HIP_TRY(db.alloc(&sv->lo, cap)); HIP_TRY(db.alloc(&sv->hi, cap)); HIP_TRY(db.alloc(&sv->gcnt, cap)); HIP_TRY(db.alloc(&sv->gfirst, cap));
	HIP_TRY(db.alloc(&g_distinct, 64 * 16 + 2));
	g_err = (u32*) (g_distinct + 64 * 16);
	n_surv = g_err + 1;
	u32* n_real = g_err + 2;
	HIP_TRY(hipMemsetAsync(g_distinct, 0, (64 * 16 + 2) * 8, st));
	SurvOutG so{sv->lo, sv->hi, sv->gcnt, sv->gfirst, n_surv, cap, n_real};
	static const u32 rd_dbg = (u32) vdjx_env_num("VDJX_RD_DBG", 0, 0, 9);
	if (t.N) {
		vdjx_prof_scope ps(c, "k_gated_reduce");
		u32* order;
		if ((rc = bucket_order(c, db, t, &order))) return rc;
		if (sym) hipLaunchKernelGGL((k_gated_reduce<TUP, true>), dim3(t.NB), dim3(RD_THREADS), 0, st, t.t, t.bucket_start, pv.bases, pv.nmask, pv.quals, pv.rl, pv.ob, k, rec_base,
		                            mfu, cmin, mqq, tlow, so, g_distinct, g_err, rd_dbg, (const u32*) order);
		else hipLaunchKernelGGL(k_gated_reduce<TUP>, dim3(t.NB), dim3(RD_THREADS), 0, st, t.t, t.bucket_start, pv.bases, pv.nmask, pv.quals, pv.rl, pv.ob, k, rec_base,
		                        mfu, cmin, mqq, tlow, so, g_distinct, g_err, rd_dbg, (const u32*) order);
	}
	u64* spread = (u64*) c->h_pin;
	u32* tail = (u32*) (spread + 64 * 16);
	static_assert((64 * 16 + 2) * 8 == VDJX_HPIN_SYNC_BYTES, "h_pin layout (vdjx_common.h)");
	HIP_TRY(hipMemcpyAsync(spread, g_distinct, VDJX_HPIN_SYNC_BYTES, hipMemcpyDeviceToHost, st));
	HIP_TRY(hipStreamSynchronize(st));
	HIP_TRY(hipGetLastError());
	const u32 ns = tail[1], err = tail[0];
	if (err) { vdjx_set_error("k_gated_reduce: %u buckets could not be split to fit LDS", err); return VDJX_EHIP; }
	if (ns > cap) { vdjx_set_error("survivor capacity logic failed (%u > %u)", ns, cap); return VDJX_EHIP; }
	sv->ndist = 0;
	for (int i = 0; i < 64; i++) sv->ndist += spread[i * 16];
	sv->n = ns;
	sv->n_real = sym ? tail[2] : ns;
	c->stats["kmer_build_shadows"] = ns - sv->n_real;
	return VDJX_OK;
}

struct RecountOut { u32* ucnt; u64* ufirst; u64* in_first; u32* in_from; u64* edge_first; u32* edge_to; };
struct RecountStatus { const u32* g_err = nullptr; const u32* n_items = nullptr; const unsigned long long* n_inst = nullptr; u32 ns = 0; };
#define VDJX_ESYMWALK (-1000)
static int recount_status_check(vdjx_ctx* c, const u32* hp, u32 ns) {
	if (hp[6] || hp[7]) { vdjx_set_error("the mirrored walk found %u + %u places where the chains are not mirror images", hp[6], hp[7]); return VDJX_ESYMWALK; }
	if (hp[0]) { vdjx_set_error("k_walk_items: item buffer too small (%u waves stopped)", hp[0]); return VDJX_EHIP; }
	if (hp[1]) { vdjx_set_error("internal error: %u of %u surviving k-mers were not met again in the records (VDJX_SYNC_DEBUG=1 names them)", hp[1], ns); return VDJX_EHIP; }
	c->stats["recount_items"] = hp[2];
	c->stats["recount_instances"] = *(const unsigned long long*) (hp + 4);
	return VDJX_OK;
}

template <typename A>
int stage_recount(vdjx_ctx* c, A& db, const vdjx_pool* pool, u64 rec_base, int k, SurvivorsG& sv, const RecountOut& ro,
                  bool derive_edges, SurvTable* table_out = nullptr, RecountStatus* defer = nullptr, bool sym_walk = false) {
	hipStream_t st = c->stream;
	const size_t R = pool->n_records;
	const int P = pool->rl - k + 1;
	const u32 ns = sv.n;
	if (ns >= (1u << 26)) { vdjx_set_error("more than 2^26 surviving k-mers: not supported by the recount items"); return VDJX_ELIMIT; }
	if (R >= (1ull << 29)) { vdjx_set_error("more than 2^29 records on one GPU: not supported by the recount items"); return VDJX_ELIMIT; }
	if ((u64) R * (u64) P >= (1ull << 32)) { vdjx_set_error("records*offsets = %llu >= 2^32 on one GPU: shard the pool over more GPUs", (unsigned long long) ((u64) R * (u64) P)); return VDJX_ELIMIT; }
	u32 tmask = 1023;
	while ((size_t) tmask + 1 < (size_t) ns * 2) tmask = tmask * 2 + 1;
	unsigned long long* pred;
	ulonglong2* table;
	u32 *succ0, *succ, *bloom, *clen, *coff, *newidx, *jump_open, *fbw, *gcnt2, *bestsucc, *partner = nullptr;
	u64 *pd, *lo2, *hi2, *gfirst2, *linw;
	ulonglong2 *skey0, *skey;
	u32 bloom_bits = 1u << 16;
	while (bloom_bits < (1u << 30) && (size_t) bloom_bits < (size_t) ns * 16) bloom_bits <<= 1;
	const u32 nb16 = (ns + 15u) >> 4;
	const u32 n_jump = (ceil_log2_u64((u64) ns + 1) + 4) / 5 + 1;
	{
		auto up = [](size_t b) { return (b + 255) & ~(size_t) 255; };
		const size_t b_bloom = up(bloom_bits / 8), b_table = up(((size_t) tmask + 1) * 16), b_pred = up((size_t) ns * 8), b_clen = up((size_t) ns * 4),
		             b_jump = up((size_t) (n_jump + 1) * 4), b_linw = up(((size_t) nb16 + 1) * 8);
		uint8_t* z;
		const size_t zb = b_bloom + b_table + b_pred + b_clen + b_jump + b_linw;
		HIP_TRY(db.alloc(&z, zb));
		HIP_TRY(hipMemsetAsync(z, 0, zb, st));
		table = (ulonglong2*) z; z += b_table;
		bloom = (u32*) z; z += b_bloom;
		pred = (unsigned long long*) z; z += b_pred;
		clen = (u32*) z; z += b_clen;
		jump_open = (u32*) z; z += b_jump;
		linw = (u64*) z;
	}
	HIP_TRY(db.alloc(&skey0, ns)); HIP_TRY(db.alloc(&skey, ns));
	HIP_TRY(db.alloc(&succ0, (size_t) ns * 4)); HIP_TRY(db.alloc(&succ, (size_t) ns * 4));
	HIP_TRY(db.alloc(&pd, ns)); HIP_TRY(db.alloc(&coff, (size_t) ns + 1)); HIP_TRY(db.alloc(&newidx, ns));
	HIP_TRY(db.alloc(&lo2, ns)); HIP_TRY(db.alloc(&hi2, ns)); HIP_TRY(db.alloc(&gcnt2, ns)); HIP_TRY(db.alloc(&gfirst2, ns));
	HIP_TRY(db.alloc(&fbw, nb16));
	HIP_TRY(db.alloc(&bestsucc, ns));
	if (sym_walk) HIP_TRY(db.alloc(&partner, ns));
	const SurvTable tb0{table, tmask, skey0, bloom, bloom_bits - 1};
	const SurvTable tb{table, tmask, skey, bloom, bloom_bits - 1};
	if (table_out) *table_out = tb;
	const dim3 gs((ns + 255) / 256), bs(256);
	{
		vdjx_prof_scope ps(c, "k_surv_table");
		hipLaunchKernelGGL(k_surv_table2, gs, bs, 0, st, sv.lo, sv.hi, ns, table, tmask, skey0, bloom, bloom_bits - 1);
		hipLaunchKernelGGL(k_succ_links2, gs, bs, 0, st, tb0, ns, k, sv.gcnt, succ0, pred, bestsucc);
	}
	{
		vdjx_prof_scope ps(c, "k_chain_order");
		hipLaunchKernelGGL(k_chain_init, gs, bs, 0, st, pred, bestsucc, ns, pd);
		for (u32 j = 0; j < n_jump; j++) hipLaunchKernelGGL(k_chain_jump, gs, bs, 0, st, pd, ns, j ? jump_open + j - 1 : (const u32*) nullptr, jump_open + j);
		hipLaunchKernelGGL(k_chain_len, gs, bs, 0, st, pd, ns, clen);
		{ const int rc_ = vdjx_scan_wide(db, st, clen, ns, coff); if (rc_) return rc_; }
		hipLaunchKernelGGL(k_chain_place, gs, bs, 0, st, pd, coff, ns, newidx);
		hipLaunchKernelGGL(k_chain_permute, gs, bs, 0, st, newidx, ns, sv.lo, sv.hi, sv.gcnt, sv.gfirst, succ0, lo2, hi2, gcnt2, gfirst2, skey, succ);
		hipLaunchKernelGGL(k_table_remap, dim3(tmask / 256 + 1), bs, 0, st, table, tmask + 1, newidx);
		if (sym_walk) hipLaunchKernelGGL(k_partner, gs, bs, 0, st, tb, ns, k, partner);
		hipLaunchKernelGGL(k_chain_words, gs, bs, 0, st, succ, skey, ns, k, linw, fbw, (const u32*) partner);
	}
	dbg_sync(c, "k_chain_order");
	if (sync_debug()) {
		std::vector<u32> ni(ns), seen(ns, 0);
		(void) hipMemcpy(ni.data(), newidx, (size_t) ns * 4, hipMemcpyDeviceToHost);
		u32 dup = 0, oob = 0;
		for (u32 i = 0; i < ns; i++) { if (ni[i] >= ns) oob++; else if (seen[ni[i]]++) dup++; }
		std::vector<u64> pdh(ns);
		std::vector<unsigned long long> prh(ns);
		(void) hipMemcpy(pdh.data(), pd, (size_t) ns * 8, hipMemcpyDeviceToHost);
		(void) hipMemcpy(prh.data(), pred, (size_t) ns * 8, hipMemcpyDeviceToHost);
		u32 unresolved = 0;
		for (u32 i = 0; i < ns; i++) { const u32 p0 = (u32) (pdh[i] >> 32); if (p0 != NONE32 && (u32) (pdh[p0] >> 32) != NONE32) unresolved++; }
		fprintf(stderr, "[vdjx] chain order: %u survivors, %u duplicate new indices, %u out of range, %u unresolved (cycles), %u jump launches\n", ns, dup, oob, unresolved, n_jump);
		for (u32 i = 0, shown = 0; i < ns && shown < 6; i++) if (ni[i] < ns && seen[ni[i]] > 1) {
			fprintf(stderr, "[vdjx]   old %u -> new %u: pd = (%u, %u), pred word %llx\n", i, ni[i], (u32) (pdh[i] >> 32), (u32) pdh[i], prh[i]);
			shown++;
		}
	}
	sv.lo = lo2; sv.hi = hi2; sv.gcnt = gcnt2; sv.gfirst = gfirst2;
	ItemFmt f;
	{
		const u32 sb = ceil_log2_u64(ns);
		static const u32 force_lb = (u32) vdjx_env_num("VDJX_RC_LEN_BITS", 4, 0, 4);
		const u32 lb = std::min(std::min(4u, 26u - sb), force_lb);
		const u32 pb = 26u - lb;
		f.pmask = (1u << pb) - 1u;
		f.len_shift = IT_SURV_SHIFT + pb;
		f.maxlen = 1u << lb;
		const u32 t = ceil_log2_u64(nb16);
		f.bmask = (1u << t) - 1u;
		f.mul = t ? ((0x9E3779B9u >> (32 - t)) | 1u) : 1u;
		u32 x = f.mul;
		for (int i = 0; i < 5; i++) x *= 2u - f.mul * x;
		f.inv = x & f.bmask;
		f.ns = ns;
	}
	const u32 nsp = (f.bmask + 1u) << 4;
	static const bool force_wide = vdjx_env_num("VDJX_RC_WIDE", 0, 0, 1) != 0;
	static const u32 cap_shift = (u32) vdjx_env_num("VDJX_RC_MAX_SHIFT", 12, 8, 12);
	const bool narrow = R < (1ull << (32 - pool->ob)) && !force_wide;
	static const u32 max_ranges = (u32) vdjx_env_num("VDJX_RC_MAX_RANGES", PART_MAXB, 2, PART_MAXB);
	const u32 max_shift = std::max(8u, std::min(narrow ? 11u : 10u, cap_shift));
	u32 range_shift = 8;
	while (range_shift < max_shift && (nsp >> range_shift) > max_ranges) range_shift++;
	const u32 n_ranges = std::max(1u, nsp >> range_shift);
	u32 l2bits = 0;
	while (((n_ranges + (1u << l2bits) - 1) >> l2bits) > max_ranges) l2bits++;
	if (l2bits) l2bits = std::min(10u, std::max(l2bits, (ceil_log2_u64(n_ranges) + 1u) / 2u));
	const u32 n_coarse = (n_ranges + (1u << l2bits) - 1) >> l2bits;
	const u32 n_ranges_p = n_coarse << l2bits;
	constexpr size_t walk_blocks = 7168;
	const size_t Rw = sym_walk ? R / 2 : R;
	u32 nblk = (u32) std::min<size_t>(walk_blocks, (Rw + WALK_THREADS * 8 - 1) / (WALK_THREADS * 8));
	constexpr u32 walk_resident = 1536;
	if (nblk > walk_resident && nblk < walk_blocks) nblk = nblk / walk_resident * walk_resident;
	if (nblk < walk_resident) nblk = (u32) std::min<size_t>(walk_resident, (Rw + WALK_THREADS - 1) / WALK_THREADS);
	if (nblk == 0) nblk = 1;
	const size_t nwaves = (size_t) nblk * (WALK_THREADS / 64);
	const size_t NI = R * (size_t) P;
	u32 blk_items = 4096;
	while (blk_items > 256 && nwaves * blk_items > NI / 2 + 65536) blk_items >>= 1;
	const u64 raw_cap = (u64) NI + (u64) NI / (blk_items / 64) + nwaves * (u64) blk_items + blk_items;
	u64 *raw, *items;
	unsigned long long *g_cursor, *n_inst;
	u32 *range_cnt, *range_start, *g_err, *gcur;
	const vdjx_arena::mark_t tmp_mark = db.mark();
	HIP_TRY(db.alloc(&raw, (size_t) raw_cap));
	HIP_TRY(db.alloc(&g_cursor, 4 + ((size_t) n_ranges_p + 1) / 2));
	n_inst = g_cursor + 1;
	g_err = (u32*) (g_cursor + 2);
	range_cnt = (u32*) (g_cursor + 4);
	HIP_TRY(db.alloc(&range_start, n_ranges_p + 1));
	HIP_TRY(hipMemsetAsync(g_cursor, 0, 32 + (size_t) n_ranges_p * 4, st));
	if (sym_walk) {
		vdjx_prof_scope ps(c, "k_chain_order");
		hipLaunchKernelGGL(k_partner_check, gs, bs, 0, st, partner, linw, ns, g_err + 3);
	}
	const bool lng = pool->W > 2;
	if (lng && R >= (1ull << 27)) { vdjx_set_error("more than 2^27 records of long reads on one GPU: not supported by the recount items"); return VDJX_ELIMIT; }
	const size_t lds_walk = (((size_t) n_ranges_p + 1) & ~(size_t) 1) * 4 + (lng ? (size_t) WALK_THREADS * GL_ROW_LONG * 8 : 0);
	if ((size_t) n_ranges_p * 4 > 64 * 1024) { vdjx_set_error("too many survivor ranges for the walk histogram"); return VDJX_ELIMIT; }
	HIP_TRY(hipFuncSetAttribute((const void*) k_walk_items<false>, hipFuncAttributeMaxDynamicSharedMemorySize, (int) lds_walk));
	HIP_TRY(hipFuncSetAttribute((const void*) k_walk_items<true>, hipFuncAttributeMaxDynamicSharedMemorySize, (int) lds_walk));
	HIP_TRY(hipFuncSetAttribute((const void*) k_walk_items<false, true>, hipFuncAttributeMaxDynamicSharedMemorySize, (int) lds_walk));
#ifdef VDJX_ABLATE
	static const u32 walk_dbg = (u32) vdjx_env_num("VDJX_WALK_DBG", 0, 0, 63);
#else
	constexpr u32 walk_dbg = 0;
#endif
	if (R && walk_dbg != 0u) {
		u64* raw2;
		unsigned long long* cur2;
		u32* cnt2;
		HIP_TRY(db.alloc(&raw2, (size_t) raw_cap));
		HIP_TRY(db.alloc(&cur2, 8));
		HIP_TRY(db.alloc(&cnt2, n_ranges_p));
		HIP_TRY(hipMemsetAsync(cur2, 0, 64, st));
		HIP_TRY(hipMemsetAsync(cnt2, 0, (size_t) n_ranges_p * 4, st));
		vdjx_prof_scope ps(c, "k_walk_dbg");
		if (lng) hipLaunchKernelGGL(k_walk_items<true>, dim3(nblk), dim3(WALK_THREADS), lds_walk, st, pool->d_bases, pool->d_nmask, R, pool->rl, pool->ob, k, tb, succ, linw, f, range_shift,
		                            n_ranges_p, raw2, raw_cap, blk_items, cur2, cnt2, g_err, walk_dbg, (const u32*) nullptr);
		else hipLaunchKernelGGL(k_walk_items<false>, dim3(nblk), dim3(WALK_THREADS), lds_walk, st, pool->d_bases, pool->d_nmask, R, pool->rl, pool->ob, k, tb, succ, linw, f, range_shift,
		                        n_ranges_p, raw2, raw_cap, blk_items, cur2, cnt2, g_err, walk_dbg, (const u32*) nullptr);
		HIP_TRY(hipMemsetAsync(g_err, 0, 4, st));
		if (walk_dbg & 32u) {
			unsigned long long hs[8];
			HIP_TRY(hipMemcpyAsync(hs, cur2, 64, hipMemcpyDeviceToHost, st));
			HIP_TRY(hipStreamSynchronize(st));
			const char* nm[] = {"", "rows", "rounds", "filter", "lookup", "chain", "item_trips"};
			for (int i = 1; i < 7; i++) c->stats[std::string("walk_dbg_") + nm[i]] = hs[i];
		}
	}
	if (R) {
		vdjx_prof_scope ps(c, "k_walk_items");
		if (lng) hipLaunchKernelGGL(k_walk_items<true>, dim3(nblk), dim3(WALK_THREADS), lds_walk, st, pool->d_bases, pool->d_nmask, R, pool->rl, pool->ob, k, tb, succ, linw, f, range_shift,
		                            n_ranges_p, raw, raw_cap, blk_items, g_cursor, range_cnt, g_err, 0u, (const u32*) nullptr);
		else if (sym_walk) hipLaunchKernelGGL((k_walk_items<false, true>), dim3(nblk), dim3(WALK_THREADS), lds_walk, st, pool->d_bases, pool->d_nmask, R / 2, pool->rl, pool->ob, k, tb, succ, linw, f, range_shift,
		                                      n_ranges_p, raw, raw_cap, blk_items, g_cursor, range_cnt, g_err, 0u, (const u32*) partner);
		else hipLaunchKernelGGL(k_walk_items<false>, dim3(nblk), dim3(WALK_THREADS), lds_walk, st, pool->d_bases, pool->d_nmask, R, pool->rl, pool->ob, k, tb, succ, linw, f, range_shift,
		                        n_ranges_p, raw, raw_cap, blk_items, g_cursor, range_cnt, g_err, 0u, (const u32*) nullptr);
	}
	dbg_sync(c, "k_walk_items");
	vdjx_scan_one(st, range_cnt, n_ranges_p, range_start);
	size_t items_cap = NI + 1;
	if (!defer) {
		u32* hp = (u32*) c->h_pin;
		HIP_TRY(hipMemcpyAsync(hp, range_start + n_ranges_p, 4, hipMemcpyDeviceToHost, st));
		HIP_TRY(hipStreamSynchronize(st));
		HIP_TRY(hipGetLastError());
		items_cap = (size_t) hp[0] + 1;
	}
	HIP_TRY(db.alloc(&items, items_cap));
	HIP_TRY(db.alloc(&gcur, n_ranges_p));
	{
		vdjx_prof_scope ps(c, "k_part_items");
		u32 npb = (u32) std::min<size_t>(1024, (NI / 4 + 65535) / 65536);
		if (npb == 0) npb = 1;
		const auto k_part_items = k_part<u64, ItemRange, part_share, true>;
		if (!l2bits) {
			HIP_TRY(part_launch(st, k_part_items, npb, PART_LDS_BYTES, range_start, n_ranges_p, 0u, gcur, items, raw, part_share{g_cursor, n_ranges_p},
			                    ItemRange{f, range_shift, ~0u}));
		} else {
			u64* l1;
			u32* gcur1;
			HIP_TRY(db.alloc(&l1, items_cap));
			HIP_TRY(db.alloc(&gcur1, n_coarse));
			HIP_TRY(part_launch(st, k_part_items, npb, PART_LDS_BYTES, range_start, n_coarse, l2bits, gcur1, l1, raw, part_share{g_cursor, n_coarse},
			                    ItemRange{f, range_shift + l2bits, ~0u}));
			const u32 sl2 = std::max(8u, std::min(64u, 2048u / n_coarse));
			HIP_TRY(part_launch(st, k_part<u64, ItemRange, part_segs>, n_coarse * sl2, PART_LDS_BYTES, range_start, n_ranges_p, 0u, gcur, items,
			                    l1, part_segs{range_start, l2bits, sl2, l2bits}, ItemRange{f, range_shift, (1u << l2bits) - 1u}));
		}
	}
	dbg_sync(c, "k_part_items");
	{
		vdjx_prof_scope ps(c, "k_recount");
#define RC_LAUNCH(SB, IT) hipLaunchKernelGGL((k_recount<SB, IT>), dim3(n_ranges), dim3(RC_THREADS), 0, st, items, range_start, f, ns, rec_base, pool->ob, fbw, ro.ucnt, ro.ufirst, ro.in_first, n_inst)
		if (narrow) {
			switch (range_shift) {
				case 8: RC_LAUNCH(256, u32); break;
				case 9: RC_LAUNCH(512, u32); break;
				case 10: RC_LAUNCH(1024, u32); break;
				default: RC_LAUNCH(2048, u32); break;
			}
		} else {
			switch (range_shift) {
				case 8: RC_LAUNCH(256, u64); break;
				case 9: RC_LAUNCH(512, u64); break;
				default: RC_LAUNCH(1024, u64); break;
			}
		}
#undef RC_LAUNCH
	}
	dbg_sync(c, "k_recount");
	if (derive_edges) {
		hipLaunchKernelGGL(k_count_unseen, dim3((ns + 255) / 256), dim3(256), 0, st, ro.ufirst, ns, g_err + 1);
		HIP_TRY(hipMemsetAsync(ro.edge_first, 0xFF, (size_t) ns * 32, st));
		hipLaunchKernelGGL(k_edges_from_in, dim3((ns * 4 + 255) / 256), dim3(256), 0, st, tb, ns, k, ro.in_first, ro.in_from, ro.edge_first, ro.edge_to);
	}
	if (defer && !sync_debug()) {
		defer->g_err = g_err; defer->n_items = range_start + n_ranges_p; defer->n_inst = n_inst; defer->ns = ns;
		return VDJX_OK;
	}
	if (defer) defer->g_err = nullptr;
	u32* hp = (u32*) c->h_pin;
	HIP_TRY(hipMemcpyAsync(hp, g_err, 8, hipMemcpyDeviceToHost, st));
	HIP_TRY(hipMemcpyAsync(hp + 2, range_start + n_ranges_p, 4, hipMemcpyDeviceToHost, st));
	HIP_TRY(hipMemcpyAsync(hp + 4, n_inst, 8, hipMemcpyDeviceToHost, st));
	HIP_TRY(hipMemcpyAsync(hp + 6, g_err + 2, 8, hipMemcpyDeviceToHost, st));
	HIP_TRY(hipStreamSynchronize(st));
	HIP_TRY(hipGetLastError());
	if (hp[6] || hp[7]) { vdjx_set_error("the mirrored walk found %u + %u places where the chains are not mirror images", hp[6], hp[7]); return VDJX_ESYMWALK; }
	const u32 err[2] = {hp[0], hp[1]}, n_items = hp[2];
	const unsigned long long inst = *(const unsigned long long*) (hp + 4);
	if (err[0]) { vdjx_set_error("k_walk_items: item buffer too small (%u waves stopped)", err[0]); return VDJX_EHIP; }
	if (err[1]) {
		if (sync_debug()) {
			std::vector<u64> uf(ns), lo(ns), hi(ns), gf(ns);
			std::vector<u32> gc(ns);
			(void) hipMemcpy(uf.data(), ro.ufirst, (size_t) ns * 8, hipMemcpyDeviceToHost);
			(void) hipMemcpy(lo.data(), sv.lo, (size_t) ns * 8, hipMemcpyDeviceToHost);
			(void) hipMemcpy(hi.data(), sv.hi, (size_t) ns * 8, hipMemcpyDeviceToHost);
			(void) hipMemcpy(gf.data(), sv.gfirst, (size_t) ns * 8, hipMemcpyDeviceToHost);
			(void) hipMemcpy(gc.data(), sv.gcnt, (size_t) ns * 4, hipMemcpyDeviceToHost);
			for (u32 i = 0, shown = 0; i < ns && shown < 8; i++) if (uf[i] == NONE64) {
				char txt[65];
				for (int j = 0; j < k; j++) { const int sh = 2 * (k - 1 - j); const u32 c2 = (u32) (sh < 64 ? lo[i] >> sh : hi[i] >> (sh - 64)) & 3u; txt[j] = "ATCG"[c2]; }
				txt[k] = 0;
				fprintf(stderr, "[vdjx] unseen survivor %u: %s gated count %u first gated instance record %llu offset %llu\n", i, txt, gc[i],
				        (unsigned long long) (gf[i] >> 6), (unsigned long long) (gf[i] & 63));
				shown++;
			}
		}
		vdjx_set_error("internal error: %u of %u surviving k-mers were not met again in the records", err[1], ns);
		return VDJX_EHIP;
	}
	c->stats["recount_items"] = n_items;
	c->stats["recount_instances"] = inst;
	db.release_to(tmp_mark);
	return VDJX_OK;
}

template <typename A>
int stage_finish2(vdjx_ctx* c, A& db, const SurvivorsG& sv, const RecountOut& ro, u64 n_records_total, int k, int P, int ob, vdjx_graph* g) {
	hipStream_t st = c->stream;
	const u32 ns = sv.n;
	const u32 nr = sv.n_real <= ns ? sv.n_real : ns;
	g->n = nr;
	g->k = k;
	g->ctx = c;
	g->device = c->device;
	if (ns == 0) return VDJX_OK;
	uint8_t *d_hv, *d_hj;
	HIP_TRY(db.alloc(&d_hv, ns));
	HIP_TRY(db.alloc(&d_hj, ns));
	{
		vdjx_prof_scope ps(c, "k_node_flags");
		hipLaunchKernelGGL(k_node_flags, dim3((ns + 255) / 256), dim3(256), 0, st, sv.lo, sv.hi, ns, k, c->d_vbits, c->d_jbits, d_hv, d_hj);
	}
	u64 *rk_key, *rk_key2;
	u32 *rk_idx, *rk_idx2, *rank;
	HIP_TRY(db.alloc(&rk_key, ns));
	HIP_TRY(db.alloc(&rk_key2, ns));
	HIP_TRY(db.alloc(&rk_idx, ns));
	HIP_TRY(db.alloc(&rk_idx2, ns));
	HIP_TRY(db.alloc(&rank, ns));
	unsigned rk_bits = 1;
	while (rk_bits < 64 && (1ull << rk_bits) <= ((n_records_total << ob) | 1ull)) rk_bits++;
	auto up = [](size_t b) { return (b + 255) & ~(size_t) 255; };
	const size_t need = up((size_t) ns * 8) + 5 * up((size_t) ns * 4) + 4 * up(ns) + 2 * up((size_t) ns * 16) + up((size_t) ns * k);
	{
		hipError_t e = c->blocks.acquire(need, &g->d_block, &g->block_cap);
		if (e != hipSuccess) { vdjx_set_error("graph alloc (%zu bytes): %s", need, hipGetErrorString(e)); return VDJX_EHIP; }
	}
	char* bp = g->d_block;
	auto carve = [&](size_t b) { char* r = bp; bp += up(b); return r; };
	NodeOut no;
	no.klo = no.khi = nullptr;
	no.first_inst = g->d_first_inst = (u64*) carve((size_t) ns * 8);
	no.gcnt = g->d_gcnt = (u32*) carve((size_t) ns * 4);
	no.freq = g->d_freq = (u32*) carve((size_t) ns * 4);
	no.to_ids = g->d_to_ids = (u32*) carve((size_t) ns * 16);
	no.from_ids = g->d_from_ids = (u32*) carve((size_t) ns * 16);
	no.hv = g->d_hv = (uint8_t*) carve(ns);
	no.hj = g->d_hj = (uint8_t*) carve(ns);
	no.to_deg = g->d_to_deg = (uint8_t*) carve(ns);
	no.from_deg = g->d_from_deg = (uint8_t*) carve(ns);
	no.kmers = g->d_kmers = carve((size_t) ns * k);
	g->export_bytes = (size_t) (bp - g->d_block);
	g->d_roots = (u32*) carve((size_t) ns * 4);
	{
		vdjx_prof_scope ps(c, "k_node_order");
		hipLaunchKernelGGL(k_rank_keys, dim3((ns + 255) / 256), dim3(256), 0, st, sv.ufirst, sv.gcnt, ns, rk_key, rk_idx);
		{
			size_t tb = 0;
			int rc_ = vdjx_sort_pairs_raw(nullptr, &tb, st, rk_key, rk_key2, rk_idx, rk_idx2, ns, rk_bits);
			if (rc_) return rc_;
			char* tmp;
			HIP_TRY(db.alloc(&tmp, tb + 256));
			if ((rc_ = vdjx_sort_pairs_raw(tmp, &tb, st, rk_key, rk_key2, rk_idx, rk_idx2, ns, rk_bits))) return rc_;
		}
		hipLaunchKernelGGL(k_rank_scatter, dim3((ns + 255) / 256), dim3(256), 0, st, rk_key2, rk_idx2, ns, rank);
		hipLaunchKernelGGL(k_node_emit2, dim3((ns + 255) / 256), dim3(256), 0, st, sv.lo, sv.hi, sv.gcnt, sv.ucnt, sv.ufirst, d_hv, d_hj, rank,
		                   ro.edge_first, ro.edge_to, ro.in_first, ro.in_from, ns, k, no);
	}
	u32 n_roots = 0;
	{
		const u32 nrb = (nr + 255) / 256;
		u32 *rb_cnt, *rb_start;
		HIP_TRY(db.alloc(&rb_cnt, nrb + 1));
		HIP_TRY(db.alloc(&rb_start, nrb + 1));
		vdjx_prof_scope ps(c, "k_root_list");
		if (nrb) hipLaunchKernelGGL(k_root_count, dim3(nrb), dim3(256), 0, st, no.from_deg, nr, rb_cnt);
		vdjx_scan_one(st, rb_cnt, nrb, rb_start);
		if (nrb) hipLaunchKernelGGL(k_root_list, dim3(nrb), dim3(256), 0, st, no.from_deg, nr, rb_start, g->d_roots);
		HIP_TRY(hipMemcpyAsync(c->h_pin, rb_start + nrb, 4, hipMemcpyDeviceToHost, st));
	}
	HIP_TRY(hipStreamSynchronize(st));
	HIP_TRY(hipGetLastError());
	n_roots = *(const u32*) c->h_pin;
	g->n_roots = n_roots;
	vdjx_prof_collect(c, false);
	return VDJX_OK;
}

template <typename TUP>
int kmer_build_impl2(vdjx_ctx* c, const vdjx_pool* pool, int k, int mf, int mq, vdjx_graph* g) {
	const int P = pool->rl - k + 1;
	vdjx_work db(c);
	GTuples<TUP> t;
	const bool sym = build_sym(pool, k);
	c->stats["kmer_build_sym"] = sym ? 1 : 0;
	int rc = stage_gated_partition<TUP>(c, db, pool, 0, k, 0, 0, &t, sym);
	if (rc) return rc;
	PoolView pv{pool->d_bases, pool->d_nmask, vdjx_qrows{pool->d_quals, pool->d_quals2, pool->q_split, pool->qstride}, pool->rl, pool->ob};
	SurvivorsG sv;
	rc = stage_gated_reduce<TUP>(c, db, t, pv, 0, k, mf, mq, &sv, sym);
	if (rc) return rc;
	vdjx_ri_open_gate(c);
	dbg_sync(c, "gated_reduce");
	g->pre_nodes = (size_t) sv.ndist;
	RecountOut ro{};
	if (sv.n) {
		HIP_TRY(db.alloc(&sv.ucnt, sv.n)); HIP_TRY(db.alloc(&sv.ufirst, sv.n));
		HIP_TRY(db.alloc(&ro.in_first, (size_t) sv.n * 4)); HIP_TRY(db.alloc(&ro.in_from, (size_t) sv.n * 4));
		HIP_TRY(db.alloc(&ro.edge_first, (size_t) sv.n * 4)); HIP_TRY(db.alloc(&ro.edge_to, (size_t) sv.n * 4));
		ro.ucnt = sv.ucnt; ro.ufirst = sv.ufirst;
		for (int attempt = 0; attempt < 2; attempt++) {
			const bool sym_walk = sym && sym_walk_wanted() && attempt == 0;
			c->stats["kmer_build_sym_walk"] = sym_walk ? 1 : 0;
			RecountStatus rs;
			rc = stage_recount(c, db, pool, 0, k, sv, ro, true, nullptr, &rs, sym_walk);
			if (rc == VDJX_ESYMWALK && sym_walk) { c->stats["kmer_build_sym_walk_retries"] += 1; continue; }
			if (rc) return rc;
			u32* hp = (u32*) c->h_pin + 1024;
			hp[6] = hp[7] = 0;
			if (rs.g_err) {
				HIP_TRY(hipMemcpyAsync(hp + 8, rs.n_inst, 24, hipMemcpyDeviceToHost, c->stream));
				HIP_TRY(hipMemcpyAsync(hp + 2, rs.n_items, 4, hipMemcpyDeviceToHost, c->stream));
			}
			rc = stage_finish2(c, db, sv, ro, pool->n_records, k, P, pool->ob, g);
			if (rc) return rc;
			if (rs.g_err) { hp[4] = hp[8]; hp[5] = hp[9]; hp[0] = hp[10]; hp[1] = hp[11]; hp[6] = hp[12]; hp[7] = hp[13]; }
			rc = rs.g_err ? recount_status_check(c, hp, rs.ns) : VDJX_OK;
			if (rc != VDJX_ESYMWALK || !sym_walk) return rc == VDJX_ESYMWALK ? VDJX_EHIP : rc;
			c->stats["kmer_build_sym_walk_retries"] += 1;
			if (g->d_block) { c->blocks.release(g->d_block, g->block_cap); g->d_block = nullptr; g->block_cap = 0; }
		}
		return VDJX_EHIP;
	}
	return stage_finish2(c, db, sv, ro, pool->n_records, k, P, pool->ob, g);
}

}

extern "C" int vdjx_kmer_build(vdjx_ctx* c, const vdjx_pool* pool, int k, int mf, int mq, vdjx_graph** out) {
	if (!c || !pool || !out) { vdjx_set_error("vdjx_kmer_build: NULL argument"); return VDJX_EINVAL; }
	*out = nullptr;
	if (pool->ctx != c) { vdjx_set_error("vdjx_kmer_build: pool belongs to another context"); return VDJX_EINVAL; }
	if (k < 1 || k > VDJX_MAX_KMER || k > pool->rl) { vdjx_set_error("k=%d outside [1,min(%d,rl=%d)]", k, VDJX_MAX_KMER, pool->rl); return VDJX_ELIMIT; }
	if (k > 16 && !c->anchors_loaded) { vdjx_set_error("vdjx_kmer_build: call vdjx_anchor_sets_load first (k > 16)"); return VDJX_ESTATE; }
	HIP_TRY(hipSetDevice(c->device));
	vdjx_clear_errors();
	vdjx_graph* g = new vdjx_graph();
	const int rc = k <= 45 ? kmer_build_impl2<Tup16>(c, pool, k, mf, mq, g) : kmer_build_impl2<Tup24>(c, pool, k, mf, mq, g);
	if (rc != VDJX_OK) { vdjx_graph_free(g); return rc; }
	*out = g;
	return VDJX_OK;
}

struct vdjx_shard {
	vdjx_ctx* c = nullptr;
	const vdjx_pool* pool = nullptr;
	int k = 0, mf = 0, mq = 0, rank = 0, nranks = 1;
	u64 rec_stride = 0;
	const u32* scan = nullptr;
	u64 total_records = 0;
	u64 rec_base() const { return scan ? 0 : rec_stride * (u64) rank; }
	u64 records_in_all() const { return scan ? total_records : rec_stride * (u64) nranks; }
	bool sym_capable = false, sym = false;
	bool wide = false;
	u32 NBf = 0, NBo = 0;
	u32 *nd = nullptr, *dstart = nullptr;
	Partial* dense = nullptr;
	u32* dense_ref = nullptr;
	u64* low_inst = nullptr;
	u32 n_dense = 0;
	SurvivorsG local_sv, all_sv;
	u32 sv_cap = 0;
	u32* n_surv = nullptr;
	PendOut po{};
	u32 n_pend = 0;
	uint2* queries = nullptr;
	std::vector<u32> src_base, nq;
	u32 *p_fl = nullptr, *p_S = nullptr, *p_r0 = nullptr;
	u32 mqq = 0, tlow = 0;
	SurvTable tb{};
	int phase = 0;
	bool have_hist = false;
	GatedHist gh;
	u64 agreed = 0;
	Partial* sparse = nullptr;
	u32* sparse_ref = nullptr;
	vdjx_arena::mark_t fill_mark{0, 0};
	const u32* tuple_bucket_start = nullptr;
	u32 NBt = 0;
};

static int shard_begin_impl(vdjx_ctx* c, const vdjx_pool* pool, int k, int mf, int mq, int rank, int nranks,
                            uint64_t rec_stride, const uint32_t* d_scan, uint64_t total_records, vdjx_shard** out) {
	if (!c || !pool || !out) { vdjx_set_error("vdjx_shard_begin: NULL argument"); return VDJX_EINVAL; }
	*out = nullptr;
	if (c->live_shard) { vdjx_set_error("vdjx_shard_begin: a sharded build is already in flight on this context"); return VDJX_ESTATE; }
	if (nranks < 1 || nranks > 256 || rank < 0 || rank >= nranks) { vdjx_set_error("1 <= nranks <= 256, 0 <= rank < nranks"); return VDJX_EINVAL; }
	if (k < 1 || k > VDJX_MAX_KMER || k > pool->rl) { vdjx_set_error("k=%d outside [1,min(%d,rl=%d)]", k, VDJX_MAX_KMER, pool->rl); return VDJX_ELIMIT; }
	if (d_scan) {
		if (total_records < pool->n_records) { vdjx_set_error("total_records %llu < local records %zu", (unsigned long long) total_records, pool->n_records); return VDJX_EINVAL; }
		if (total_records >= (1ull << 32) || total_records >= (1ull << (INST_BITS - pool->ob))) { vdjx_set_error("global record count %llu: scan positions are 32 bits and instance ids record << %d | offset in %d bits", (unsigned long long) total_records, pool->ob, INST_BITS); return VDJX_ELIMIT; }
		rec_stride = (total_records + (uint64_t) nranks - 1) / (uint64_t) nranks;
	} else {
		if (rec_stride < pool->n_records) { vdjx_set_error("rec_stride %llu < local records %zu", (unsigned long long) rec_stride, pool->n_records); return VDJX_EINVAL; }
		if (rec_stride * (uint64_t) nranks >= (1ull << (INST_BITS - pool->ob))) { vdjx_set_error("global record count %llu >= 2^%d (instance ids are record << %d | offset in %d bits)", (unsigned long long) (rec_stride * nranks), INST_BITS - pool->ob, pool->ob, INST_BITS); return VDJX_ELIMIT; }
	}
	if (k > 16 && !c->anchors_loaded) { vdjx_set_error("vdjx_shard_begin: call vdjx_anchor_sets_load first (k > 16)"); return VDJX_ESTATE; }
	if (pool->W > 2 && pool->n_records >= (1ull << 27)) { vdjx_set_error("more than 2^27 records of long reads on one GPU: not supported by the recount items"); return VDJX_ELIMIT; }
	vdjx_shard* s = new vdjx_shard();
	s->c = c; s->pool = pool; s->k = k; s->mf = mf; s->mq = mq; s->rank = rank; s->nranks = nranks;
	s->rec_stride = rec_stride;
	s->scan = d_scan; s->total_records = total_records;
	s->sym_capable = build_sym(pool, k) && s->rec_base() % 2 == 0;
	s->wide = k > 45;
	if (mq >= 255) mq = 254;
	s->mqq = (u32) (mq < 0 ? 0 : (mq > 214 ? 214 : mq));
	s->tlow = 1 + (s->mqq + 19) / 20;
	c->live_shard = s;
	*out = s;
	return VDJX_OK;
}

extern "C" int vdjx_shard_begin(vdjx_ctx* c, const vdjx_pool* pool, int k, int mf, int mq, int rank, int nranks,
                                uint64_t rec_stride, vdjx_shard** out) {
	return shard_begin_impl(c, pool, k, mf, mq, rank, nranks, rec_stride, nullptr, 0, out);
}

extern "C" int vdjx_shard_begin_share(vdjx_ctx* c, const vdjx_pool* pool, int k, int mf, int mq, int rank, int nranks,
                                      const uint32_t* d_scan_index, uint64_t total_records, vdjx_shard** out) {
	if (pool && pool->n_records && !d_scan_index) { vdjx_set_error("vdjx_shard_begin_share: NULL scan index"); return VDJX_EINVAL; }
	static const uint32_t none = 0;
	return shard_begin_impl(c, pool, k, mf, mq, rank, nranks, 0, d_scan_index ? d_scan_index : &none, total_records, out);
}

extern "C" void vdjx_shard_free(vdjx_shard* s) {
	if (!s) return;
	(void) hipSetDevice(s->c->device);
	(void) hipStreamSynchronize(s->c->stream);
	s->c->shard_arena.reset();
	s->c->live_shard = nullptr;
	delete s;
}

extern "C" size_t vdjx_shard_record_bytes(int kind) {
	return kind == 0 ? sizeof(Partial) : kind == 1 ? sizeof(uint2) : kind == 2 ? REPLY_BYTES : kind == 3 ? sizeof(SurvRec) : 0;
}

static u64 shard_geometry_bound(const vdjx_shard* s) {
	const int P = s->pool->rl - s->k + 1;
	return std::max<u64>(1, s->rec_stride * (u64) P / 4);
}

template <typename TUP>
static int shard_local_impl(vdjx_shard* s) {
	vdjx_ctx* c = s->c;
	hipStream_t st = c->stream;
	PersistAlloc db(c);
	const u64 rec_base = s->rec_base();
	GTuples<TUP> t;
	int rc = VDJX_OK;
	if (s->have_hist && s->gh.sym != s->sym) s->have_hist = false;
	const size_t per_b = 0;
	if (!s->have_hist) rc = stage_gated_hist(c, db, s->pool, s->k, per_b, shard_geometry_bound(s) / (s->sym ? 2 : 1), &s->gh, s->sym);
	if (rc) return rc;
	s->have_hist = true;
	const size_t cap = (size_t) s->gh.N + 1;
	const size_t nb_max = ((size_t) 1 << 20) + 16 * (size_t) s->nranks + 2;
	Partial* sparse;
	u32 *g_err, *sparse_ref;
	HIP_TRY(db.alloc(&s->low_inst, cap));
	HIP_TRY(db.alloc(&s->dense_ref, cap));
	HIP_TRY(db.alloc(&s->nd, nb_max));
	HIP_TRY(db.alloc(&s->dstart, nb_max + 1));
	HIP_TRY(db.alloc(&g_err, 1));
	u32* keep_starts;
	HIP_TRY(db.alloc(&keep_starts, nb_max + 1));
	s->fill_mark = db.mark();
	HIP_TRY(db.alloc(&sparse, cap));
	HIP_TRY(db.alloc(&sparse_ref, cap));
	const vdjx_arena::mark_t tuple_mark = db.mark();
	rc = stage_gated_cut<TUP>(c, db, s->pool, rec_base, s->k, per_b, (s->agreed ? s->agreed : shard_geometry_bound(s)) / (s->sym ? 2 : 1), s->gh, &t);
	if (rc) return rc;
	if (t.NB < (u32) s->nranks) { vdjx_set_error("vdjx_shard_local: fewer buckets (%u) than ranks", t.NB); return VDJX_ELIMIT; }
	s->NBo = t.NB / (u32) s->nranks;
	if (s->NBo * (u32) s->nranks != t.NB) s->NBo = (s->NBo + 1 + 15) & ~15u;
	s->NBf = s->NBo * (u32) s->nranks;
	if ((size_t) s->NBf + 1 > nb_max) { vdjx_set_error("vdjx_shard_local: %u buckets", s->NBf); return VDJX_ELIMIT; }
	HIP_TRY(hipMemsetAsync(g_err, 0, 4, st));
	if (s->NBf > t.NB) HIP_TRY(hipMemsetAsync(s->nd + t.NB, 0, (size_t) (s->NBf - t.NB) * 4, st));
	if ((rc = set_sub_tuples(c))) return rc;
	{
		vdjx_prof_scope ps(c, "k_gated_local");
		u32* order;
		if ((rc = bucket_order(c, db, t, &order))) return rc;
		if (s->sym) hipLaunchKernelGGL((k_gated_local<TUP, true>), dim3(t.NB), dim3(LG_THREADS), 0, st, t.t, t.bucket_start, s->pool->d_bases, s->pool->d_nmask, rec_base,
		                               s->k, s->pool->rl, s->pool->ob, s->tlow, sparse, sparse_ref, s->nd, s->low_inst, g_err, (const u32*) order);
		else hipLaunchKernelGGL(k_gated_local<TUP>, dim3(t.NB), dim3(LG_THREADS), 0, st, t.t, t.bucket_start, s->pool->d_bases, s->pool->d_nmask, rec_base,
		                        s->k, s->pool->rl, s->pool->ob, s->tlow, sparse, sparse_ref, s->nd, s->low_inst, g_err, (const u32*) order);
	}
	vdjx_scan_one(st, s->nd, s->NBf, s->dstart);
	u32* d_pick;
	const u32 G = (u32) s->nranks;
	HIP_TRY(db.alloc(&d_pick, G + 1));
	hipLaunchKernelGGL(k_pick_u32, dim3(1), dim3(512), 0, st, s->dstart, s->NBo, G + 1, d_pick);
	std::vector<u32> pick(G + 1);
	u32 err = 0;
	HIP_TRY(hipMemcpyAsync(pick.data(), d_pick, (G + 1) * 4, hipMemcpyDeviceToHost, st));
	HIP_TRY(hipMemcpyAsync(&err, g_err, 4, hipMemcpyDeviceToHost, st));
	HIP_TRY(hipMemcpyAsync(keep_starts, t.bucket_start, ((size_t) t.NB + 1) * 4, hipMemcpyDeviceToDevice, st));
	HIP_TRY(hipStreamSynchronize(st));
	HIP_TRY(hipGetLastError());
	if (err) { vdjx_set_error("k_gated_local: %u buckets could not be split to fit LDS", err); return VDJX_EHIP; }
	s->src_base.assign(pick.begin(), pick.end());
	s->n_dense = pick[G];
	s->sparse = sparse; s->sparse_ref = sparse_ref; s->NBt = t.NB;
	s->dense = nullptr;
	db.release_to(tuple_mark);
	s->tuple_bucket_start = keep_starts;
	return VDJX_OK;
}

extern "C" int vdjx_shard_local(vdjx_shard* s, uint64_t* send_counts, uint32_t* dir_len) {
	if (!s || !send_counts || !dir_len) { vdjx_set_error("vdjx_shard_local: NULL argument"); return VDJX_EINVAL; }
	if (s->phase != 0) { vdjx_set_error("vdjx_shard_local: already called"); return VDJX_ESTATE; }
	HIP_TRY(hipSetDevice(s->c->device));
	vdjx_clear_errors();
	int rc = s->wide ? shard_local_impl<Tup24>(s) : shard_local_impl<Tup16>(s);
	if (rc) return rc;
	vdjx_ri_open_gate(s->c);
	for (int g = 0; g < s->nranks; g++) send_counts[g] = s->src_base[g + 1] - s->src_base[g];
	*dir_len = s->NBo;
	s->phase = 1;
	return VDJX_OK;
}

extern "C" int vdjx_shard_local_fill(vdjx_shard* s, void* d_dir, void* d_partials) {
	if (!s || s->phase < 1) { vdjx_set_error("vdjx_shard_local_fill: call vdjx_shard_local first"); return VDJX_ESTATE; }
	if (!d_dir || (s->n_dense && !d_partials)) { vdjx_set_error("vdjx_shard_local_fill: NULL buffer"); return VDJX_EINVAL; }
	if (((uintptr_t) d_partials & 15u) != 0) { vdjx_set_error("vdjx_shard_local_fill: d_partials must be 16-byte aligned"); return VDJX_EINVAL; }
	HIP_TRY(hipSetDevice(s->c->device));
	vdjx_clear_errors();
	hipStream_t st = s->c->stream;
	HIP_TRY(hipMemcpyAsync(d_dir, s->nd, (size_t) s->NBf * 4, hipMemcpyDeviceToDevice, st));
	if (s->n_dense) {
		vdjx_prof_scope ps(s->c, "k_compact_partials");
		hipLaunchKernelGGL(k_compact_partials, dim3(s->NBt), dim3(256), 0, st, s->sparse, s->sparse_ref, s->tuple_bucket_start, s->nd, s->dstart, (Partial*) d_partials, s->dense_ref, s->scan, s->pool->ob, s->sym);
	}
	s->dense = (Partial*) d_partials;
	HIP_TRY(hipStreamSynchronize(st));
	HIP_TRY(hipGetLastError());
	if (s->sparse) {
		PersistAlloc db(s->c);
		db.release_to(s->fill_mark);
		s->sparse = nullptr; s->sparse_ref = nullptr; s->tuple_bucket_start = nullptr;
	}
	return VDJX_OK;
}

extern "C" int vdjx_shard_count(vdjx_shard* s, uint64_t* gated_instances) {
	if (!s || !gated_instances) { vdjx_set_error("vdjx_shard_count: NULL argument"); return VDJX_EINVAL; }
	if (s->phase != 0) { vdjx_set_error("vdjx_shard_count: call it before vdjx_shard_local"); return VDJX_ESTATE; }
	HIP_TRY(hipSetDevice(s->c->device));
	vdjx_clear_errors();
	if (!s->have_hist) {
		PersistAlloc db(s->c);
		const int rc = stage_gated_hist(s->c, db, s->pool, s->k, 0, shard_geometry_bound(s) / (s->sym_capable ? 2 : 1), &s->gh, s->sym_capable);
		if (rc) return rc;
		s->have_hist = true;
	}
	*gated_instances = (u64) s->gh.N * (s->gh.sym ? 2 : 1);
	return VDJX_OK;
}
extern "C" int vdjx_shard_symmetric(const vdjx_shard* s) { return s && s->sym_capable ? 1 : 0; }
extern "C" int vdjx_shard_geometry2(vdjx_shard* s, uint64_t agreed_instances, int all_symmetric) {
	if (!s) { vdjx_set_error("vdjx_shard_geometry2: NULL argument"); return VDJX_EINVAL; }
	if (all_symmetric && !s->sym_capable) { vdjx_set_error("vdjx_shard_geometry2: this rank's pool is not made of couples"); return VDJX_EINVAL; }
	const int rc = vdjx_shard_geometry(s, agreed_instances);
	if (rc) return rc;
	s->sym = all_symmetric != 0;
	s->c->stats["kmer_build_sym"] = s->sym ? 1 : 0;
	return VDJX_OK;
}
extern "C" int vdjx_shard_geometry(vdjx_shard* s, uint64_t agreed_instances) {
	if (!s) { vdjx_set_error("vdjx_shard_geometry: NULL argument"); return VDJX_EINVAL; }
	if (s->phase != 0) { vdjx_set_error("vdjx_shard_geometry: call it before vdjx_shard_local"); return VDJX_ESTATE; }
	if (agreed_instances < (u64) s->gh.N * (s->gh.sym ? 2 : 1)) { vdjx_set_error("vdjx_shard_geometry: %llu is less than this rank's own %llu gated instances", (unsigned long long) agreed_instances, (unsigned long long) s->gh.N * (s->gh.sym ? 2 : 1)); return VDJX_EINVAL; }
	s->agreed = agreed_instances ? agreed_instances : 1;
	return VDJX_OK;
}

template <typename THI>
static int shard_merge_impl(vdjx_shard* s, const u32* d_recv_dir, const Partial* d_recv, const uint64_t* recv_counts, uint64_t* query_counts) {
	vdjx_ctx* c = s->c;
	hipStream_t st = c->stream;
	PersistAlloc db(c);
	const u32 G = (u32) s->nranks, NBo = s->NBo;
	s->src_base.assign(G + 1, 0);
	for (u32 g = 0; g < G; g++) s->src_base[g + 1] = s->src_base[g] + (u32) recv_counts[g];
	const u32 total = s->src_base[G];
	u32 *d_src_base, *seg_off, *g_nq, *g_err, *n_pend;
	u64* g_distinct;
	HIP_TRY(db.alloc(&d_src_base, G + 1));
	HIP_TRY(db.alloc(&seg_off, (size_t) G * (NBo + 1)));
	HIP_TRY(db.alloc(&g_nq, G));
	HIP_TRY(db.alloc(&g_err, 1));
	HIP_TRY(db.alloc(&n_pend, 1));
	HIP_TRY(db.alloc(&s->n_surv, 1));
	HIP_TRY(db.alloc(&g_distinct, 1));
	HIP_TRY(db.alloc(&s->queries, (size_t) total + 1));
	const u32 cap = (s->sym ? 2 : 1) * total + 2;
	s->sv_cap = cap;
	SurvivorsG& v = s->local_sv;
	HIP_TRY(db.alloc(&v.lo, cap)); HIP_TRY(db.alloc(&v.hi, cap)); HIP_TRY(db.alloc(&v.gcnt, cap)); HIP_TRY(db.alloc(&v.gfirst, cap));
	PendOut& po = s->po;
	HIP_TRY(db.alloc(&po.lo, cap)); HIP_TRY(db.alloc(&po.hi, cap)); HIP_TRY(db.alloc(&po.cg, cap)); HIP_TRY(db.alloc(&po.mg, cap));
	HIP_TRY(db.alloc(&po.need, cap));
	po.mgr = nullptr;
	if (s->sym) HIP_TRY(db.alloc(&po.mgr, cap));
	po.n = n_pend; po.cap = cap;
	HIP_TRY(hipMemcpyAsync(d_src_base, s->src_base.data(), (G + 1) * 4, hipMemcpyHostToDevice, st));
	hipLaunchKernelGGL(k_seg_offsets, dim3(G), dim3(1024), 0, st, d_recv_dir, d_src_base, G, NBo, seg_off);
	const u32 cmin = (u32) std::max(s->mf, 2);
	SurvOutG so{v.lo, v.hi, v.gcnt, v.gfirst, s->n_surv, cap, nullptr};
	s->nq.assign(G, 0);
	u32 MG = 1;
	while (MG < NBo && NBo % (MG * 2) == 0 && (u64) total * (MG * 2) <= (u64) NBo * (MERGE_SLOTS * 3 / 8)) MG <<= 1;
	u32 np = 0, ns = 0, err = 0;
	u64 ndist = 0;
	for (u32 s_mult = 1;; s_mult *= 4) {
		HIP_TRY(hipMemsetAsync(g_nq, 0, (size_t) G * 4, st));
		HIP_TRY(hipMemsetAsync(g_err, 0, 4, st));
		HIP_TRY(hipMemsetAsync(n_pend, 0, 4, st));
		HIP_TRY(hipMemsetAsync(s->n_surv, 0, 4, st));
		HIP_TRY(hipMemsetAsync(g_distinct, 0, 8, st));
		if (total) {
			vdjx_prof_scope ps(c, "k_bucket_merge");
			if (s->sym) hipLaunchKernelGGL((k_bucket_merge<THI, true>), dim3(NBo / MG), dim3(MERGE_THREADS), 0, st, d_recv, seg_off, MG, G, NBo, d_src_base, s_mult, cmin,
			                               s->tlow, so, po, s->queries, g_nq, g_distinct, g_err, s->k);
			else hipLaunchKernelGGL(k_bucket_merge<THI>, dim3(NBo / MG), dim3(MERGE_THREADS), 0, st, d_recv, seg_off, MG, G, NBo, d_src_base, s_mult, cmin,
			                        s->tlow, so, po, s->queries, g_nq, g_distinct, g_err, s->k);
		}
		HIP_TRY(hipMemcpyAsync(s->nq.data(), g_nq, (size_t) G * 4, hipMemcpyDeviceToHost, st));
		HIP_TRY(hipMemcpyAsync(&np, n_pend, 4, hipMemcpyDeviceToHost, st));
		HIP_TRY(hipMemcpyAsync(&ns, s->n_surv, 4, hipMemcpyDeviceToHost, st));
		HIP_TRY(hipMemcpyAsync(&err, g_err, 4, hipMemcpyDeviceToHost, st));
		HIP_TRY(hipMemcpyAsync(&ndist, g_distinct, 8, hipMemcpyDeviceToHost, st));
		HIP_TRY(hipStreamSynchronize(st));
		HIP_TRY(hipGetLastError());
		if (!err) break;
		if (s_mult >= (1u << 16)) { vdjx_set_error("k_bucket_merge: %u buckets could not be split to fit LDS", err); return VDJX_EHIP; }
	}
	s->n_pend = np;
	c->stats["shard_partials_received"] = total;
	c->stats["shard_open_kmers"] = np;
	c->stats["shard_decided_at_merge"] = ns;
	{
		u64 nqs = 0;
		for (u32 q : s->nq) nqs += q;
		c->stats["shard_questions"] = nqs;
	}
	v.n = ns;
	v.ndist = ndist;
	for (u32 g = 0; g < G; g++) query_counts[g] = s->nq[g];
	const size_t sides = s->sym ? 2 : 1;
	HIP_TRY(db.alloc(&s->p_fl, (size_t) np + 1));
	HIP_TRY(db.alloc(&s->p_r0, sides * np + 1));
	HIP_TRY(db.alloc(&s->p_S, sides * np * 64 + 1));
	if (np) {
		HIP_TRY(hipMemsetAsync(s->p_fl, 0, (size_t) np * 4, st));
		HIP_TRY(hipMemsetAsync(s->p_r0, 0xFF, sides * np * 4, st));
		HIP_TRY(hipMemsetAsync(s->p_S, 0, sides * np * 256, st));
	}
	return VDJX_OK;
}

extern "C" int vdjx_shard_merge(vdjx_shard* s, const void* d_recv_dir, const void* d_recv_partials, const uint64_t* recv_counts,
                                uint64_t* query_counts) {
	if (!s || !recv_counts || !query_counts || !d_recv_dir) { vdjx_set_error("vdjx_shard_merge: NULL argument"); return VDJX_EINVAL; }
	if (s->phase != 1) { vdjx_set_error("vdjx_shard_merge: call vdjx_shard_local first (once)"); return VDJX_ESTATE; }
	uint64_t tot = 0;
	for (int g = 0; g < s->nranks; g++) tot += recv_counts[g];
	if (tot >= (1ull << 30)) { vdjx_set_error("vdjx_shard_merge: too many partial aggregates for one owner (%llu): use more ranks", (unsigned long long) tot); return VDJX_ELIMIT; }
	if (tot && !d_recv_partials) { vdjx_set_error("vdjx_shard_merge: NULL buffer"); return VDJX_EINVAL; }
	HIP_TRY(hipSetDevice(s->c->device));
	vdjx_clear_errors();
	int rc = s->wide ? shard_merge_impl<u64>(s, (const u32*) d_recv_dir, (const Partial*) d_recv_partials, recv_counts, query_counts)
	                 : shard_merge_impl<u32>(s, (const u32*) d_recv_dir, (const Partial*) d_recv_partials, recv_counts, query_counts);
	if (rc) return rc;
	s->phase = 2;
	return VDJX_OK;
}

extern "C" int vdjx_shard_queries(vdjx_shard* s, void* d_out) {
	if (!s || s->phase < 2) { vdjx_set_error("vdjx_shard_queries: call vdjx_shard_merge first"); return VDJX_ESTATE; }
	HIP_TRY(hipSetDevice(s->c->device));
	vdjx_clear_errors();
	hipStream_t st = s->c->stream;
	size_t at = 0;
	for (int g = 0; g < s->nranks; g++) {
		if (!s->nq[g]) continue;
		if (!d_out) { vdjx_set_error("vdjx_shard_queries: NULL buffer"); return VDJX_EINVAL; }
		HIP_TRY(hipMemcpyAsync((uint2*) d_out + at, s->queries + s->src_base[g], (size_t) s->nq[g] * sizeof(uint2), hipMemcpyDeviceToDevice, st));
		at += s->nq[g];
	}
	HIP_TRY(hipStreamSynchronize(st));
	return VDJX_OK;
}

extern "C" int vdjx_shard_reply(vdjx_shard* s, const void* d_queries, const uint64_t* counts, void* d_replies) {
	if (!s || !counts) { vdjx_set_error("vdjx_shard_reply: NULL argument"); return VDJX_EINVAL; }
	if (s->phase < 1 || (s->n_dense && !s->dense)) { vdjx_set_error("vdjx_shard_reply: call vdjx_shard_local and vdjx_shard_local_fill first"); return VDJX_ESTATE; }
	vdjx_ctx* c = s->c;
	HIP_TRY(hipSetDevice(c->device));
	vdjx_clear_errors();
	const u32 G = (u32) s->nranks;
	std::vector<u32> off(G + 1, 0);
	for (u32 g = 0; g < G; g++) off[g + 1] = off[g] + (u32) counts[g];
	const u32 nq = off[G];
	if (!nq) return VDJX_OK;
	if (!d_queries || !d_replies) { vdjx_set_error("vdjx_shard_reply: NULL buffer"); return VDJX_EINVAL; }
	PersistAlloc db(c);
	u32* d_off;
	HIP_TRY(db.alloc(&d_off, G + 1));
	hipStream_t st = c->stream;
	HIP_TRY(hipMemcpyAsync(d_off, off.data(), (G + 1) * 4, hipMemcpyHostToDevice, st));
	const vdjx_pool* p = s->pool;
	{
		vdjx_prof_scope ps(c, "k_shard_reply");
		if (s->sym) hipLaunchKernelGGL(k_shard_reply<true>, dim3(nq), dim3(64), 0, st, (const uint2*) d_queries, nq, d_off, G, s->dense, s->dense_ref, s->dstart, s->NBo,
		                               s->low_inst, p->d_bases, p->d_nmask, vdjx_qrows{p->d_quals, p->d_quals2, p->q_split, p->qstride}, s->rec_base(), s->scan, (u32) p->n_records, s->k, p->rl, p->ob, (uint8_t*) d_replies);
		else hipLaunchKernelGGL(k_shard_reply<false>, dim3(nq), dim3(64), 0, st, (const uint2*) d_queries, nq, d_off, G, s->dense, s->dense_ref, s->dstart, s->NBo,
		                        s->low_inst, p->d_bases, p->d_nmask, vdjx_qrows{p->d_quals, p->d_quals2, p->q_split, p->qstride}, s->rec_base(), s->scan, (u32) p->n_records, s->k, p->rl, p->ob, (uint8_t*) d_replies);
	}
	HIP_TRY(hipStreamSynchronize(st));
	HIP_TRY(hipGetLastError());
	return VDJX_OK;
}

extern "C" int vdjx_shard_resolve(vdjx_shard* s, const void* d_replies, uint64_t n_replies, uint64_t* n_survivors, uint64_t* n_distinct) {
	if (!s || !n_survivors || !n_distinct) { vdjx_set_error("vdjx_shard_resolve: NULL argument"); return VDJX_EINVAL; }
	if (s->phase != 2) { vdjx_set_error("vdjx_shard_resolve: call vdjx_shard_merge first (once)"); return VDJX_ESTATE; }
	uint64_t expect = 0;
	for (u32 q : s->nq) expect += q;
	if (n_replies != expect) { vdjx_set_error("vdjx_shard_resolve: %llu answers for %llu questions", (unsigned long long) n_replies, (unsigned long long) expect); return VDJX_EINVAL; }
	vdjx_ctx* c = s->c;
	HIP_TRY(hipSetDevice(c->device));
	vdjx_clear_errors();
	hipStream_t st = c->stream;
	SurvivorsG& v = s->local_sv;
	if (s->n_pend) {
		if (!d_replies) { vdjx_set_error("vdjx_shard_resolve: NULL buffer"); return VDJX_EINVAL; }
		const u32 nr = (u32) n_replies;
		SurvOutG so{v.lo, v.hi, v.gcnt, v.gfirst, s->n_surv, s->sv_cap, nullptr};
		vdjx_prof_scope ps(c, "k_shard_resolve");
		hipLaunchKernelGGL(k_resolve_first, dim3((nr + 255) / 256), dim3(256), 0, st, (const uint8_t*) d_replies, nr, s->po.mg, s->p_r0, (const u64*) s->po.mgr, s->n_pend);
		hipLaunchKernelGGL(k_resolve_add, dim3((nr + 3) / 4), dim3(256), 0, st, (const uint8_t*) d_replies, nr, s->p_r0, s->k, s->p_fl, s->p_S, s->sym ? s->n_pend : 0u);
		if (s->sym) hipLaunchKernelGGL(k_resolve_keep<true>, dim3((s->n_pend + 255) / 256), dim3(256), 0, st, s->po, s->n_pend, s->p_fl, s->p_S, s->k,
		                               (u32) std::max(s->mf, 0), s->mqq, s->tlow, so);
		else hipLaunchKernelGGL(k_resolve_keep<false>, dim3((s->n_pend + 255) / 256), dim3(256), 0, st, s->po, s->n_pend, s->p_fl, s->p_S, s->k,
		                        (u32) std::max(s->mf, 0), s->mqq, s->tlow, so);
	}
	u32 ns = 0;
	HIP_TRY(hipMemcpyAsync(&ns, s->n_surv, 4, hipMemcpyDeviceToHost, st));
	HIP_TRY(hipStreamSynchronize(st));
	HIP_TRY(hipGetLastError());
	c->stats["shard_kept_after_answers"] = ns - v.n;
	v.n = ns;
	*n_survivors = ns;
	*n_distinct = v.ndist;
	s->phase = 3;
	return VDJX_OK;
}

extern "C" int vdjx_shard_survivors(vdjx_shard* s, void* d_out) {
	if (!s || s->phase < 3) { vdjx_set_error("vdjx_shard_survivors: call vdjx_shard_resolve first"); return VDJX_ESTATE; }
	const SurvivorsG& v = s->local_sv;
	if (!v.n) return VDJX_OK;
	if (!d_out) { vdjx_set_error("vdjx_shard_survivors: NULL buffer"); return VDJX_EINVAL; }
	HIP_TRY(hipSetDevice(s->c->device));
	vdjx_clear_errors();
	hipLaunchKernelGGL(k_surv_pack, dim3((v.n + 255) / 256), dim3(256), 0, s->c->stream, v.lo, v.hi, v.gcnt, v.gfirst, v.n, (SurvRec*) d_out);
	HIP_TRY(hipStreamSynchronize(s->c->stream));
	HIP_TRY(hipGetLastError());
	return VDJX_OK;
}

extern "C" int vdjx_shard_edges(vdjx_shard* s, const void* d_surv_all, uint64_t ns_total, void* d_in_first, void* d_ucnt, void* d_ufirst) {
	if (!s || s->phase < 3) { vdjx_set_error("vdjx_shard_edges: call vdjx_shard_resolve first"); return VDJX_ESTATE; }
	if (ns_total >= (1ull << 26)) { vdjx_set_error("vdjx_shard_edges: too many survivors"); return VDJX_ELIMIT; }
	vdjx_ctx* c = s->c;
	HIP_TRY(hipSetDevice(c->device));
	vdjx_clear_errors();
	PersistAlloc db(c);
	SurvivorsG& a = s->all_sv;
	a.n = (u32) ns_total;
	a.n_real = a.n;
	s->phase = 4;
	if (!ns_total) return VDJX_OK;
	if (!d_surv_all || !d_in_first || !d_ucnt || !d_ufirst) { vdjx_set_error("vdjx_shard_edges: NULL buffer"); return VDJX_EINVAL; }
	HIP_TRY(db.alloc(&a.lo, a.n)); HIP_TRY(db.alloc(&a.hi, a.n)); HIP_TRY(db.alloc(&a.gcnt, a.n)); HIP_TRY(db.alloc(&a.gfirst, a.n));
// ... 214 lines not shown
```

### vdjer_amd/csrc/vdjx_part.h

```cpp
#pragma once

#include "vdjx_common.h"

#include <type_traits>

#define PART_THREADS 1024
#define PART_LDS_BYTES 131072
#define PART_MAXB 1024
#define PART_SLICES 8u
#define PART_NONE 0xFFFFFFFFu
#define PART_HOLE 0xFFFFFFFFFFFFFFFFull

namespace {

__device__ inline void part_scan(const u32* cnt, u32* base, u32* tmp, u32 n) {
	const u32 t = threadIdx.x, lane = t & 63, wv = t >> 6;
	const u32 a = 2 * t < n ? cnt[2 * t] : 0, b = 2 * t + 1 < n ? cnt[2 * t + 1] : 0;
	const u32 incl = (u32) vdjx_wave_scan_add((int) (a + b));
	if (lane == 63) tmp[wv] = incl;
	__syncthreads();
	if (wv == 0) {
		const u32 w = lane < PART_THREADS / 64 ? tmp[lane] : 0;
		const u32 wi = (u32) vdjx_wave_scan_add((int) w);
		if (lane < PART_THREADS / 64) tmp[lane] = wi - w;
		if (lane == 63) tmp[PART_THREADS / 64] = wi;
	}
	__syncthreads();
	const u32 excl = tmp[wv] + incl - (a + b);
	if (2 * t < n) base[2 * t] = excl;
	if (2 * t + 1 < n) base[2 * t + 1] = excl + a;
	if (t == 0) base[n] = tmp[PART_THREADS / 64];
	__syncthreads();
}

template <typename T> __device__ inline T part_load(const T* p) { return T::load(p); }
template <typename T> __device__ inline void part_store(T* p, const T& x) { T::store(p, x); }
__device__ inline u64 part_load(const u64* p) { return *p; }
__device__ inline void part_store(u64* p, const u64& x) { *p = x; }

struct part_round {
	u32 cnt[PART_MAXB], base[PART_MAXB + 1], cur[PART_MAXB], gbase[PART_MAXB], tmp[PART_THREADS];

	__device__ inline void begin(u32 nbk) {
		for (u32 i = threadIdx.x; i < nbk; i += PART_THREADS) cnt[i] = 0;
		__syncthreads();
	}
	__device__ inline void count(u32 b) { atomicAdd(&cnt[b], 1u); }
	__device__ inline u32 reserve(u32 nbk, u32* __restrict__ gcur) {
		part_scan(cnt, base, tmp, nbk);
		for (u32 i = threadIdx.x; i < nbk; i += PART_THREADS) {
			cur[i] = base[i];
			gbase[i] = cnt[i] ? atomicAdd(&gcur[i], cnt[i]) : 0u;
		}
		__syncthreads();
		return base[nbk];
	}
	__device__ inline u32 slot(u32 b) { return atomicAdd(&cur[b], 1u); }
	template <typename T, typename Key> __device__ inline void flush(const T* stage, u32 n, T* __restrict__ out, const Key& key) {
		for (u32 i = threadIdx.x; i < n; i += PART_THREADS) {
			const T x = part_load(&stage[i]);
			const u32 b = key(x);
			part_store(&out[gbase[b] + (i - base[b])], x);
		}
		__syncthreads();
	}
};

__device__ inline u32 part_slice(const u32* __restrict__ seg_start, u32 seg_shift, u32 slices, size_t& t0, size_t& t1) {
	const u32 seg = blockIdx.x / slices, sl = blockIdx.x % slices;
	const size_t s0 = seg_start[(size_t) seg << seg_shift], s1 = seg_start[((size_t) seg + 1) << seg_shift];
	const size_t per = (s1 - s0 + slices - 1) / slices;
	t0 = s0 + (size_t) sl * per;
	t1 = t0 + per < s1 ? t0 + per : s1;
	return seg;
}

struct part_share {
	const unsigned long long* n;
	u32 nbk;
	__device__ inline size_t span(u32 round, size_t& t0, size_t& t1, u32& buckets) const {
		const size_t N = (size_t) *n;
		const size_t per = ((N + gridDim.x - 1) / gridDim.x + round - 1) / round * round;
		t0 = (size_t) blockIdx.x * per;
		t1 = t0 + per < N ? t0 + per : N;
		buckets = nbk;
		return 0;
	}
};
struct part_segs {
	const u32* seg_start;
	u32 seg_shift, slices, sub_bits;
	__device__ inline size_t span(u32, size_t& t0, size_t& t1, u32& buckets) const {
		buckets = 1u << sub_bits;
		return (size_t) part_slice(seg_start, seg_shift, slices, t0, t1) << sub_bits;
	}
};

template <typename T, typename Key, typename Range, bool PAIRED = false>
__global__ __launch_bounds__(PART_THREADS) void k_part(const T* __restrict__ in, Range range, Key key, u32* __restrict__ gcur, T* __restrict__ out) {
	extern __shared__ __attribute__((aligned(16))) uint8_t part_smem[];
	T* stage = (T*) part_smem;
	__shared__ part_round pr;
	constexpr u32 PER = PART_LDS_BYTES / sizeof(T) / PART_THREADS;
	constexpr u32 ROUND = PER * PART_THREADS;
	static_assert(!PAIRED || (std::is_same<T, u64>::value && PER % 2 == 0), "the paired loads are for 8-byte elements");
	size_t t0, t1;
	u32 nbk;
	u32* gc = gcur + range.span(ROUND, t0, t1, nbk);
	for (size_t ts = t0; ts < t1; ts += ROUND) {
		const size_t te = ts + ROUND < t1 ? ts + ROUND : t1;
		pr.begin(nbk);
		T r_x[PER];
		u32 r_b[PER];
		if constexpr (PAIRED) {
#pragma unroll
			for (u32 j = 0; j < PER; j += 2) {
				const size_t t = ts + ((size_t) (j / 2) * PART_THREADS + threadIdx.x) * 2;
				r_x[j] = PART_HOLE; r_x[j + 1] = PART_HOLE;
				if (t + 1 < te) { const ulonglong2 v = *(const ulonglong2*) &in[t]; r_x[j] = v.x; r_x[j + 1] = v.y; }
				else if (t < te) r_x[j] = in[t];
			}
#pragma unroll
			for (u32 j = 0; j < PER; j++) {
				r_b[j] = PART_NONE;
				if (r_x[j] != PART_HOLE) { r_b[j] = key(r_x[j]); pr.count(r_b[j]); }
			}
		} else {
#pragma unroll
			for (u32 j = 0; j < PER; j++) {
				const size_t t = ts + (size_t) j * PART_THREADS + threadIdx.x;
				r_b[j] = PART_NONE;
				if (t < te) { r_x[j] = part_load(&in[t]); r_b[j] = key(r_x[j]); }
			}
#pragma unroll
			for (u32 j = 0; j < PER; j++) if (r_b[j] != PART_NONE) pr.count(r_b[j]);
		}
		__syncthreads();
		const u32 n = pr.reserve(nbk, gc);
#pragma unroll
		for (u32 j = 0; j < PER; j++) if (r_b[j] != PART_NONE) part_store(&stage[pr.slot(r_b[j])], r_x[j]);
		__syncthreads();
		pr.flush(stage, n, out, key);
	}
}

__global__ void k_init_cursors(const u32* __restrict__ bucket_start, u32 n, u32 sh, u32* __restrict__ cur) {
	u32 i = blockIdx.x * blockDim.x + threadIdx.x;
	if (i < n) cur[i] = bucket_start[(size_t) i << sh];
}

template <typename... P, typename O, typename... Args>
inline hipError_t part_launch(hipStream_t st, void (*kernel)(P...), u32 grid, u32 lds, const u32* bucket_start, u32 ncur, u32 sh, u32* gcur, O* out,
                              Args... args) {
	const hipError_t e = hipFuncSetAttribute((const void*) kernel, hipFuncAttributeMaxDynamicSharedMemorySize, (int) lds);
	if (e != hipSuccess) return e;
	hipLaunchKernelGGL(k_init_cursors, dim3((ncur + 255) / 256), dim3(256), 0, st, bucket_start, ncur, sh, gcur);
	hipLaunchKernelGGL(kernel, dim3(grid), dim3(PART_THREADS), lds, st, args..., gcur, out);
	return hipSuccess;
}

}
```

Before: 914.7.

## Sample one row in S for the k-mer bucket histogram with overflow-checked retry

The gated histogram now visits only one 64-record row in every S (default 16) for large pools, so it reads far fewer reads. Bucket capacities come from the scaled sample count plus a sqrt-based safety margin. Partition and reduce kernels check each bucket against its capacity and raise an overflow flag. If any bucket overflows, the build rewinds the arena and redoes the cut from the exact histogram. The exchange is a cheaper histogram pass plus larger, padded bucket allocations, with a full rerun of partition and reduce whenever the sample underestimates a bucket.

Result: faster. 939.6, median of 6 (+2.7%).

```diff
diff --git a/profiles/cut_stats.py b/profiles/cut_stats.py
--- /dev/null
+++ b/profiles/cut_stats.py
@@ -0,0 +1,34 @@
+import gc
+import json
+import os
+import sys
+
+sys.path.insert(0, os.path.dirname(os.path.dirname(os.path.abspath(__file__))))
+import torch
+
+import bench
+from vdjer_amd import api
+
+WORKLOADS = (("configs[2]: 10 M pairs, k = 35", 10_000_000, 35, 3, 90, {}),
+             ("configs[3]: 10 M pairs, k = 25", 10_000_000, 25, 2, 60, {}),
+             ("--repertoire private, 10 M pairs", 10_000_000, 35, 3, 90, dict(private_v=True, private_j=True, zipf_s=0.25)),
+             ("--pairs 1000000", 1_000_000, 35, 3, 90, {}))
+SEED = 20261002
+
+for name, pairs, k, mf, mq, rep_kw in WORKLOADS:
+    bench.REP_KW.clear()
+    bench.REP_KW.update(rep_kw)
+    clones = max(4, pairs // (4000 if rep_kw else 500))
+    rep, pool, vc, jc, _ = bench.make_workload(pairs, clones, SEED, 0, 1, "cuda:0")
+    ctx = api.Context(0)
+    ctx.anchor_sets_load(vc, jc)
+    p = ctx.pool_load_device(pool.primary.data_ptr(), pool.primary.shape[0], pool.secondary.data_ptr(), pool.secondary.shape[0], pool.rl)
+    nodes = [int(ctx.kmer_build(p, k, mf, mq).n) for _ in range(3)]
+    out = {"workload": name, "builds": 3, "nodes": nodes}
+    out.update({n: int(ctx.stat(n)) for n in ("kmer_build_cut_sample", "kmer_build_cut_retries", "kmer_build_sym", "kmer_build_sym_walk_retries", "gated_instances")})
+    print(json.dumps(out), flush=True)
+    p.free()
+    ctx.close()
+    del pool, p, ctx
+    gc.collect()
+    torch.cuda.empty_cache()
diff --git a/vdjer_amd/csrc/vdjx_common.h b/vdjer_amd/csrc/vdjx_common.h
--- a/vdjer_amd/csrc/vdjx_common.h
+++ b/vdjer_amd/csrc/vdjx_common.h
@@ -70,7 +70,7 @@
 struct vdjx_shard;
 
 #define VDJX_HPIN_BYTES 16384
-#define VDJX_HPIN_SYNC_BYTES ((64 * 16 + 2) * 8)
+#define VDJX_HPIN_SYNC_BYTES ((64 * 16 + 3) * 8)
 #define VDJX_HPIN_ROOT_RUN 3072
 static_assert(VDJX_HPIN_ROOT_RUN * 4 >= VDJX_HPIN_SYNC_BYTES + 64 && VDJX_HPIN_ROOT_RUN * 4 + 4 <= VDJX_HPIN_BYTES, "h_pin layout");
 
diff --git a/vdjer_amd/csrc/vdjx_kmer.hip b/vdjer_amd/csrc/vdjx_kmer.hip
--- a/vdjer_amd/csrc/vdjx_kmer.hip
+++ b/vdjer_amd/csrc/vdjx_kmer.hip
@@ -144,10 +144,11 @@
 	return flip;
 }
 
-template <bool LONG, bool SYM = false>
+template <bool LONG, bool SYM = false, bool SAMPLED = false>
 __global__ __launch_bounds__(HIST_THREADS) void k_gated_hist(const u64* __restrict__ bases, const u64* __restrict__ nmask,
                                                              const u64* __restrict__ lowq, size_t R, int rl, int k, u32 nb_bits,
-                                                             size_t rpb, u32* __restrict__ bucket_cnt, u32 dbg_in) {
+                                                             size_t rpb, u32* __restrict__ bucket_cnt, u32 dbg_in,
+                                                             u32 S, size_t Rv, u32* __restrict__ sampled) {
 #ifdef VDJX_ABLATE
 	const u32 dbg = dbg_in;
 #else
@@ -165,13 +166,16 @@
 	uint16_t* wl = (uint16_t*) (wv + (LONG ? 64u * GL_ROW_LONG * 8u : 1024u));
 	const u32 lane = threadIdx.x & 63u;
 	const size_t r0 = (size_t) blockIdx.x * rpb;
-	const size_t r1 = r0 + rpb < R ? r0 + rpb : R;
+	const size_t r1 = SAMPLED ? (r0 + rpb < Rv ? r0 + rpb : Rv) : (r0 + rpb < R ? r0 + rpb : R);
 	const int P = rl - k + 1;
+	static_assert(!(LONG && SAMPLED), "the sample is taken of short reads");
+	u32 wtot = 0;
 	for (size_t rb = r0; rb < r1; rb += HIST_THREADS) {
-		const size_t r = rb + threadIdx.x;
+		const size_t v = rb + threadIdx.x;
+		const size_t r = SAMPLED ? ((((v >> 6) * S + S / 2) << 6) | (v & 63)) : v;
 		u64 G = 0;
 		vdjx_mask3 bad{~0ull, ~0ull, ~0ull};
-		if (r < r1) {
+		if (v < r1 && (!SAMPLED || r < R)) {
 			if (LONG) { bad = load_gate3(lowq, r); stage_row_long(wrow + lane * GL_ROW_LONG, bases, r); }
 			else {
 				const GateView v = load_gate(bases, lowq, SYM ? 2 * r : r);
@@ -187,6 +191,7 @@
 			const u32 total = (u32) __builtin_amdgcn_readlane((int) incl, 63);
 			if (dbg == 1) { sink += incl; continue; }
 			if (!total) continue;
+			if (SAMPLED) wtot += total;
 			u32 at = incl - c;
 			for (u32 gg = g; gg; gg &= gg - 1) wl[at++] = (uint16_t) ((lane << (LONG ? 8 : 6)) | (u32) (ob + __builtin_ctz(gg)));
 			vdjx_wave_lds_fence();
@@ -209,6 +214,7 @@
 	__syncthreads();
 	if (dbg) { if (sink == 0x12345u) bucket_cnt[0] = sink; return; }
 	for (u32 i = threadIdx.x; i < NB; i += HIST_THREADS) if (hist[i]) atomicAdd(&bucket_cnt[i], hist[i]);
+	if (SAMPLED && lane == 0 && wtot) atomicAdd(sampled, wtot);
 }
 
 template <typename TUP> struct TupBucket {
@@ -220,8 +226,8 @@
 template <typename TUP, bool LONG, bool SYM = false>
 __global__ __launch_bounds__(PART_THREADS) void k_part_records_g(const u64* __restrict__ bases, const u64* __restrict__ nmask,
                                                                  const u64* __restrict__ lowq, size_t R, u64 rec_base, int rl, int k,
-                                                                 u32 shift, u32 nbk, size_t rpb, u32 rr0, u32* __restrict__ gcur,
-                                                                 TUP* __restrict__ out) {
+                                                                 u32 shift, u32 nbk, size_t rpb, u32 rr0, const u32* __restrict__ lim, u32 lsh,
+                                                                 u32* __restrict__ over, u32* __restrict__ gcur, TUP* __restrict__ out) {
 	extern __shared__ __attribute__((aligned(16))) uint8_t smem[];
 	TUP* stage = (TUP*) smem;
 	u32* desc = (u32*) (smem + PARTR_STAGE_BYTES);
@@ -242,6 +248,7 @@
 	const size_t r0 = (size_t) blockIdx.x * rpb;
 	const size_t r1 = r0 + rpb < R ? r0 + rpb : R;
 	size_t rs = r0;
+	pr.limits(nbk, lim, lsh, over);
 	while (rs < r1) {
 		const size_t re = rs + rr < r1 ? rs + rr : r1;
 		if (threadIdx.x == 0) s_n = 0;
@@ -295,6 +302,7 @@
 			continue;
 		}
 		const u32 n = pr.reserve(nbk, gcur);
+		if (n == PART_DEAD) return;
 		for (u32 i = threadIdx.x; i < n; i += PART_THREADS) {
 			const u32 d = desc[i];
 			const size_t r = rs + (d >> (OB + 10));
@@ -319,13 +327,15 @@
 
 template <typename TUP>
 __global__ __launch_bounds__(512) void k_seg_hist_g(const TUP* __restrict__ in, const u32* __restrict__ seg_start, u32 seg_shift, u32 slices,
-                                                    u32 shift, u32 sub_bits, u32* __restrict__ fine_cnt) {
+                                                    u32 shift, u32 sub_bits, u32* __restrict__ fine_cnt, const u32* __restrict__ seg_end,
+                                                    const u32* __restrict__ over) {
 	__shared__ u32 h[PART_MAXB];
+	if (over && *over) return;
 	const u32 nbk = 1u << sub_bits;
 	for (u32 i = threadIdx.x; i < nbk; i += 512) h[i] = 0;
 	__syncthreads();
 	size_t t0, t1;
-	const u32 seg = part_slice(seg_start, seg_shift, slices, t0, t1);
+	const u32 seg = part_slice(seg_start, seg_shift, slices, t0, t1, seg_end);
 	for (size_t t = t0 + threadIdx.x; t < t1; t += 512) {
 		const TUP x = TUP::load(&in[t]);
 		atomicAdd(&h[(u32) (vdjx_bucket_mix(x.lo, x.hi()) >> shift) & (nbk - 1)], 1u);
@@ -401,25 +411,26 @@
 	return c0;
 }
 
-__global__ __launch_bounds__(1024) void k_bucket_order(const u32* __restrict__ bucket_start, u32 NB, u32* __restrict__ order) {
+__global__ __launch_bounds__(1024) void k_bucket_order(const u32* __restrict__ bucket_start, const u32* __restrict__ bucket_end, u32 NB, u32* __restrict__ order) {
 	__shared__ u32 cls_cnt[33], cls_at[33];
 	if (threadIdx.x < 33) cls_cnt[threadIdx.x] = 0;
 	__syncthreads();
 	for (u32 b = threadIdx.x; b < NB; b += 1024) {
-		const u32 n = bucket_start[b + 1] - bucket_start[b];
+		const u32 n = bucket_end[b] - bucket_start[b];
 		atomicAdd(&cls_cnt[n ? 32u - (u32) __builtin_clz(n) : 0u], 1u);
 	}
 	__syncthreads();
 	if (threadIdx.x == 0) { u32 at = 0; for (int cl = 32; cl >= 0; cl--) { cls_at[cl] = at; at += cls_cnt[cl]; } }
 	__syncthreads();
 	for (u32 b = threadIdx.x; b < NB; b += 1024) {
-		const u32 n = bucket_start[b + 1] - bucket_start[b];
+		const u32 n = bucket_end[b] - bucket_start[b];
 		order[atomicAdd(&cls_at[n ? 32u - (u32) __builtin_clz(n) : 0u], 1u)] = b;
 	}
 }
 
 template <typename TUP, bool SYM = false>
 __global__ __launch_bounds__(RD_THREADS, sizeof(TUP) == 16 ? RD_WAVES : RD_WAVES / 2) void k_gated_reduce(const TUP* __restrict__ tup, const u32* __restrict__ bucket_start,
+                                                             const u32* __restrict__ bucket_end, const u32* __restrict__ cut_over,
                                                              const u64* __restrict__ bases, const u64* __restrict__ nmask,
                                                              vdjx_qrows quals, int rl, int ob, int k, u64 rec_base,
                                                              u32 mf, u32 cmin, u32 mqq, u32 tlow, SurvOutG so,
@@ -441,9 +452,10 @@
 	__shared__ unsigned short low_slot[RD_LROWS];
 	__shared__ u32 s_over, s_ndist, s_nlow, s_npq, s_nsurv, s_base, s_nreal;
 	const THI EMPTY = (THI) ~(THI) 0;
+	if (cut_over && *cut_over) return;
 	const u32 b = order ? order[blockIdx.x] : blockIdx.x;
 	const u32 base = bucket_start[b];
-	const u32 n = bucket_start[b + 1] - base;
+	const u32 n = bucket_end[b] - base;
 	const u32 tid = threadIdx.x;
 	if (n == 0) return;
 	const TUP* T = tup + base;
@@ -671,7 +683,7 @@
 #define LG_NOLIST 0x7FFFFFFFu
 template <typename TUP, bool SYM = false>
 __global__ __launch_bounds__(LG_THREADS, sizeof(TUP) == 16 ? 6 : 3) void k_gated_local(const TUP* __restrict__ tup, const u32* __restrict__ bucket_start,
-                                                            const u64* __restrict__ bases, const u64* __restrict__ nmask, u64 rec_base, int k, int rl, int ob,
+                                                            const u32* __restrict__ bucket_end, const u64* __restrict__ bases, const u64* __restrict__ nmask, u64 rec_base, int k, int rl, int ob,
                                                             u32 tlow, Partial* __restrict__ sparse_g, u32* __restrict__ sparse_ref,
                                                             u32* __restrict__ nd_g, u64* __restrict__ low_inst, u32* __restrict__ g_err,
                                                             const u32* __restrict__ order) {
@@ -687,7 +699,7 @@
 	const THI EMPTY = (THI) ~(THI) 0;
 	const u32 b = order ? order[blockIdx.x] : blockIdx.x;
 	const u32 base = bucket_start[b];
-	const u32 n = bucket_start[b + 1] - base;
+	const u32 n = bucket_end[b] - base;
 	const u32 tid = threadIdx.x;
 	const u32 om = (1u << ob) - 1u;
 	if (n == 0) { if (tid == 0) nd_g[b] = 0; return; }
@@ -1946,10 +1958,15 @@
 
 struct PoolView { const u64* bases; const u64* nmask; vdjx_qrows quals; int rl; int ob; };
 
+#define VDJX_ECUT (-1001)
 template <typename TUP> struct GTuples {
 	TUP* t = nullptr;
 	u32* bucket_start = nullptr;
+	const u32* bucket_end = nullptr;
+	u32* over = nullptr;
 	u32 NB = 0, N = 0;
+	u32 Nsurv = 0;
+	u32 S = 1;
 };
 
 struct SurvivorsG {
@@ -1968,14 +1985,32 @@
 	fprintf(stderr, "[vdjx] %s: %s\n", what, hipGetErrorString(e));
 }
 
-struct GatedHist { u32 HB = 0, NBH = 0, N = 0; u32* hstart = nullptr; bool sym = false; };
+struct GatedHist { u32 HB = 0, NBH = 0, N = 0; u32* hstart = nullptr; bool sym = false; u32 S = 1, cap_total = 0; };
 static bool build_sym(const vdjx_pool* pool, int k) {
 	return pool->sym && pool->W == 2 && (k & 1) && pool->n_records % 2 == 0;
 }
 static bool sym_walk_wanted() { static const bool on = !vdjx_env_set("VDJX_NO_SYM_WALK"); return on; }
 static size_t gated_bucket_default() { static const size_t v = (size_t) vdjx_env_num("VDJX_GATED_BUCKET", 3072, 1, 1ll << 32); return v; }
+
+#define CUT_MARGIN_C 16.5f
+#define CUT_MARGIN_FLOOR 264u
+#define CUT_SAMPLE_MIN_RECORDS ((size_t) 1 << 20)
+struct cut_cap {
+	u32 S, floor;
+	float cS;
+	__device__ u32 operator()(u32 h) const { return S * h + (u32) ceilf(cS * sqrtf((float) h + 1.0f)) + floor; }
+};
+static float cut_margin_c() { static const float v = CUT_MARGIN_C * (float) vdjx_env_num("VDJX_CUT_MARGIN", 100, 0, 100000) / 100.0f; return v; }
+static u32 cut_sample_stride(const vdjx_pool* pool, size_t R) {
+	static const bool given = vdjx_env_set("VDJX_HIST_SAMPLE");
+	static const u32 S = (u32) vdjx_env_num("VDJX_HIST_SAMPLE", 16, 1, 4096);
+	if (pool->W != 2 || S < 2) return 1;
+	if (!given && R < CUT_SAMPLE_MIN_RECORDS) return 1;
+	return (R + 63) / 64 > S / 2 ? S : 1;
+}
+
 template <typename A>
-int stage_gated_hist(vdjx_ctx* c, A& db, const vdjx_pool* pool, int k, size_t per_bucket, u64 geometry_instances, GatedHist* gh, bool sym = false) {
+int stage_gated_hist(vdjx_ctx* c, A& db, const vdjx_pool* pool, int k, size_t per_bucket, u64 geometry_instances, GatedHist* gh, bool sym = false, u32 S = 1) {
 	hipStream_t st = c->stream;
 	const size_t R = sym ? pool->n_records / 2 : pool->n_records;
 	const int P = pool->rl - k + 1;
@@ -1990,36 +2025,95 @@
 #else
 	constexpr u32 hist_dbg = 0;
 #endif
-	u32 nblk = (u32) std::min<size_t>(HIST_BLOCKS, (R + 4095) / 4096);
+	const bool lng = pool->W > 2;
+	if (lng || per_bucket || geometry_instances || (R + 63) / 64 <= S / 2) S = 1;
+	if (S > 1) {
+		const double s_max = (double) NI / S + 64.0 * P, cS = (double) cut_margin_c() * S;
+		if ((double) S * s_max + (double) NBH * (CUT_MARGIN_FLOOR + 1.0) + cS * sqrt((double) NBH * (s_max + NBH)) >= 4.0e9) S = 1;
+	}
+	const size_t rows = (R + 63) / 64;
+	const size_t Rv = S > 1 ? (rows - S / 2 + S - 1) / S * 64 : R;
+	u32 nblk = S > 1 ? (u32) std::min<size_t>(HIST_BLOCKS, (Rv + 1023) / 1024) : (u32) std::min<size_t>(HIST_BLOCKS, (R + 4095) / 4096);
 	if (nblk == 0) nblk = 1;
-	size_t rpb = (R + nblk - 1) / nblk;
-	u32 *hcnt, *hstart;
-	HIP_TRY(db.alloc(&hcnt, NBH));
-	HIP_TRY(db.alloc(&hstart, NBH + 1));
-	HIP_TRY(hipMemsetAsync(hcnt, 0, (size_t) NBH * 4, st));
-	const bool lng = pool->W > 2;
+	size_t rpb = (Rv + nblk - 1) / nblk;
+	if (S > 1) rpb = (rpb + 63) / 64 * 64;
+	u32 *hcnt, *hstart, *blk;
+	HIP_TRY(db.alloc(&blk, 2 * (size_t) NBH + 2));
+	hstart = blk;
+	u32* samp = blk + NBH + 1;
+	hcnt = samp + 1;
+	HIP_TRY(hipMemsetAsync(samp, 0, ((size_t) NBH + 1) * 4, st));
 	const size_t lds_hist = (size_t) NBH * 4 + (HIST_THREADS / 64) * (lng ? GL_WAVE_BYTES_LONG : GL_WAVE_BYTES);
 	HIP_TRY(hipFuncSetAttribute((const void*) k_gated_hist<false>, hipFuncAttributeMaxDynamicSharedMemorySize, (int) lds_hist));
 	HIP_TRY(hipFuncSetAttribute((const void*) k_gated_hist<true>, hipFuncAttributeMaxDynamicSharedMemorySize, (int) lds_hist));
 	HIP_TRY(hipFuncSetAttribute((const void*) k_gated_hist<false, true>, hipFuncAttributeMaxDynamicSharedMemorySize, (int) lds_hist));
+	HIP_TRY(hipFuncSetAttribute((const void*) k_gated_hist<false, false, true>, hipFuncAttributeMaxDynamicSharedMemorySize, (int) lds_hist));
+	HIP_TRY(hipFuncSetAttribute((const void*) k_gated_hist<false, true, true>, hipFuncAttributeMaxDynamicSharedMemorySize, (int) lds_hist));
+	const auto launch_hist = [&](u32 nb, size_t per_blk, u32* cnt, u32 stride, size_t rv, u32* sampled) {
+		auto* hist = lng ? k_gated_hist<true> : stride > 1 ? (sym ? k_gated_hist<false, true, true> : k_gated_hist<false, false, true>) : sym ? k_gated_hist<false, true> : k_gated_hist<false>;
+		hipLaunchKernelGGL(hist, dim3(nb), dim3(HIST_THREADS), lds_hist, st, pool->d_bases, pool->d_nmask, pool->d_lowq, R, pool->rl, k, HB, per_blk, cnt, hist_dbg, stride, rv, sampled);
+	};
 	{
 		vdjx_prof_scope ps(c, "k_gated_hist");
-		if (lng) hipLaunchKernelGGL(k_gated_hist<true>, dim3(nblk), dim3(HIST_THREADS), lds_hist, st, pool->d_bases, pool->d_nmask, pool->d_lowq, R, pool->rl, k, HB, rpb, hcnt, hist_dbg);
-		else if (sym) hipLaunchKernelGGL((k_gated_hist<false, true>), dim3(nblk), dim3(HIST_THREADS), lds_hist, st, pool->d_bases, pool->d_nmask, pool->d_lowq, R, pool->rl, k, HB, rpb, hcnt, hist_dbg);
-		else hipLaunchKernelGGL(k_gated_hist<false>, dim3(nblk), dim3(HIST_THREADS), lds_hist, st, pool->d_bases, pool->d_nmask, pool->d_lowq, R, pool->rl, k, HB, rpb, hcnt, hist_dbg);
+		launch_hist(nblk, rpb, hcnt, S, Rv, samp);
 	}
 	dbg_sync(c, "k_gated_hist");
-	vdjx_scan_one(st, hcnt, NBH, hstart);
-	HIP_TRY(hipMemcpyAsync(c->h_pin, hstart + NBH, 4, hipMemcpyDeviceToHost, st));
+	const cut_cap cap{S, CUT_MARGIN_FLOOR, cut_margin_c() * (float) S};
+	if (S > 1 && sync_debug()) {
+		u32* exact;
+		HIP_TRY(db.alloc(&exact, NBH));
+		HIP_TRY(hipMemsetAsync(exact, 0, (size_t) NBH * 4, st));
+		const u32 nbe = (u32) std::max<size_t>(1, std::min<size_t>(HIST_BLOCKS, (R + 4095) / 4096));
+		launch_hist(nbe, (R + nbe - 1) / nbe, exact, 1u, R, samp);
+		std::vector<u32> he(NBH), hs(NBH);
+		HIP_TRY(hipMemcpyAsync(he.data(), exact, (size_t) NBH * 4, hipMemcpyDeviceToHost, st));
+		HIP_TRY(hipMemcpyAsync(hs.data(), hcnt, (size_t) NBH * 4, hipMemcpyDeviceToHost, st));
+		HIP_TRY(hipStreamSynchronize(st));
+		double worst = 0, n = 0, caps = 0;
+		u32 unseen = 0;
+		for (u32 b = 0; b < NBH; b++) {
+			worst = std::max(worst, ((double) he[b] - (double) S * hs[b]) / ((double) S * sqrt((double) hs[b] + 1.0)));
+			if (!hs[b]) unseen = std::max(unseen, he[b]);
+			n += he[b];
+			caps += (double) S * hs[b] + ceil((double) cap.cS * sqrt((double) hs[b] + 1.0)) + cap.floor;
+		}
+		fprintf(stderr, "[vdjx] sampled cut: S %u, 2^%u buckets, %.0f tuples, worst ratio %.3f, largest unseen bucket %u, capacities / tuples %.3f\n", S, HB, n, worst, unseen, n ? caps / n : 0.0);
+	}
+	if (S > 1) vdjx_scan_one(st, hcnt, NBH, hstart, cap);
+	else vdjx_scan_one(st, hcnt, NBH, hstart);
+	HIP_TRY(hipMemcpyAsync(c->h_pin, hstart + NBH, 8, hipMemcpyDeviceToHost, st));
 	HIP_TRY(hipStreamSynchronize(st));
 	HIP_TRY(hipGetLastError());
 #ifdef VDJX_ABLATE
 	if (hist_dbg) return VDJX_ESTATE;
 #endif
+	gh->HB = HB; gh->NBH = NBH; gh->hstart = hstart; gh->sym = sym; gh->S = S;
+	if (S > 1) {
+		const u64 s = ((const u32*) c->h_pin)[1], n_est = (u64) S * s;
+		gh->N = (u32) n_est;
+		gh->cap_total = *(const u32*) c->h_pin;
+		return VDJX_OK;
+	}
 	const u32 N = *(const u32*) c->h_pin;
 	c->stats["gated_instances"] = sym ? 2ull * N : N;
-	gh->HB = HB; gh->NBH = NBH; gh->N = N; gh->hstart = hstart; gh->sym = sym;
+	gh->N = N;
 	return VDJX_OK;
+}
+
+__global__ __launch_bounds__(1024) void k_cut_totals(const u32* __restrict__ bucket_start, const u32* __restrict__ bucket_end, u32 NB,
+                                                     const u32* __restrict__ over, u32* __restrict__ over_out, unsigned long long* __restrict__ total) {
+	__shared__ u32 wsum[16];
+	const u32 b = blockIdx.x * 1024u + threadIdx.x;
+	const u32 n = b < NB ? bucket_end[b] - bucket_start[b] : 0u;
+	const u32 incl = (u32) vdjx_wave_scan_add((int) n);
+	if ((threadIdx.x & 63u) == 63u) wsum[threadIdx.x >> 6] = incl;
+	__syncthreads();
+	if (threadIdx.x == 0) {
+		unsigned long long t = 0;
+		for (u32 w = 0; w < 16; w++) t += wsum[w];
+		if (t) atomicAdd(total, t);
+		if (blockIdx.x == 0) *over_out = *over;
+	}
 }
 
 template <typename TUP, typename A>
@@ -2032,9 +2126,13 @@
 	const u32 hb_max = pool->W > 2 ? 14u : 15u;
 	const bool lng = pool->W > 2;
 	const u32 HB = gh.HB, NBH = gh.NBH, N = gh.N;
+	const bool smp = gh.S > 1;
+	const size_t room = smp ? gh.cap_total : N;
 	u32* hstart = gh.hstart;
 	size_t rpb;
-	out->N = N;
+	out->N = (u32) room;
+	out->S = gh.S;
+	out->Nsurv = smp ? (u32) std::min<u64>(room, (u64) N + (u64) ceil((double) cut_margin_c() * gh.S * sqrt((double) (N / gh.S) + 1.0)) + CUT_MARGIN_FLOOR) : N;
 	const u64 Ng = geometry_instances ? geometry_instances : (u64) N;
 	static const size_t refine = (size_t) vdjx_env_num("VDJX_REFINE_TUPLES", 4096, 1, 1ll << 32);
 	u32 T = 8;
@@ -2047,7 +2145,7 @@
 	}
 	const u32 Tt = T + extra;
 	const u32 NBt = 1u << Tt;
-	HIP_TRY(db.alloc(&out->t, (size_t) N + 1));
+	HIP_TRY(db.alloc(&out->t, room + 1));
 	constexpr u32 stage_tuples = PARTR_STAGE_BYTES / (u32) sizeof(TUP);
 	constexpr u32 lds_partr = PARTR_STAGE_BYTES + stage_tuples * 4;
 	u32 cbits = Tt, fbits = 0;
@@ -2056,10 +2154,15 @@
 	u32 nblk2 = (u32) std::min<size_t>(1024, (R + 2047) / 2048);
 	if (nblk2 == 0) nblk2 = 1;
 	rpb = (R + nblk2 - 1) / nblk2;
-	u32* gcur;
+	u32 *gcur, *over = nullptr;
 	HIP_TRY(db.alloc(&gcur, NBc));
+	if (smp) {
+		HIP_TRY(db.alloc(&over, 1));
+		HIP_TRY(hipMemsetAsync(over, 0, 4, st));
+	}
+	out->over = over;
 	TUP* l1 = out->t;
-	if (fbits) HIP_TRY(db.alloc(&l1, (size_t) N + 1));
+	if (fbits) HIP_TRY(db.alloc(&l1, room + 1));
 	{
 		vdjx_prof_scope ps(c, "k_part_records");
 		const u64 NIl = (u64) R * (u64) P;
@@ -2067,38 +2170,43 @@
 		rr = std::max<u64>(PART_THREADS, std::min<u64>(rr / PART_THREADS * PART_THREADS, lng ? 1u << 14 : 1u << 16));
 		auto* part_records = lng ? k_part_records_g<TUP, true> : sym ? k_part_records_g<TUP, false, true> : k_part_records_g<TUP, false>;
 		HIP_TRY(part_launch(st, part_records, nblk2, lds_partr, hstart, NBc, HB - cbits, gcur, l1, pool->d_bases, pool->d_nmask, pool->d_lowq, R, rec_base,
-		                    pool->rl, k, 64 - cbits, NBc, rpb, (u32) rr));
+		                    pool->rl, k, 64 - cbits, NBc, rpb, (u32) rr, smp ? (const u32*) hstart : (const u32*) nullptr, HB - cbits, over));
 	}
 	dbg_sync(c, "k_part_records");
 	u32* tstart;
 	HIP_TRY(db.alloc(&tstart, NBt + 1));
 	out->NB = NBt;
 	out->bucket_start = tstart;
+	out->bucket_end = tstart + 1;
+	const u32* seg_end = smp ? gcur : nullptr;
 	constexpr u32 slices = PART_SLICES;
 	if (extra) {
 		u32* fine_cnt;
 		HIP_TRY(db.alloc(&fine_cnt, NBt));
 		HIP_TRY(hipMemsetAsync(fine_cnt, 0, (size_t) NBt * 4, st));
 		vdjx_prof_scope ps(c, "k_seg_hist");
-		hipLaunchKernelGGL(k_seg_hist_g<TUP>, dim3(NBc * slices), dim3(512), 0, st, l1, hstart, HB - cbits, slices, 64 - Tt, fbits, fine_cnt);
+		hipLaunchKernelGGL(k_seg_hist_g<TUP>, dim3(NBc * slices), dim3(512), 0, st, l1, hstart, HB - cbits, slices, 64 - Tt, fbits, fine_cnt, seg_end, (const u32*) over);
 		vdjx_scan_one(st, fine_cnt, NBt, tstart);
 	} else {
 		hipLaunchKernelGGL(k_pick_u32, dim3((NBt + 1 + 255) / 256), dim3(256), 0, st, hstart, 1u << (HB - Tt), NBt + 1, tstart);
+		if (smp && !fbits) out->bucket_end = gcur;
 	}
 	if (fbits) {
 		u32* gcur2;
 		HIP_TRY(db.alloc(&gcur2, NBt));
+		const bool lim2 = smp && !extra;
+		if (lim2) out->bucket_end = gcur2;
 		vdjx_prof_scope ps(c, "k_part_tuples");
 		HIP_TRY(part_launch(st, k_part<TUP, TupBucket<TUP>, part_segs>, NBc * slices, PART_LDS_BYTES, tstart, NBt, 0u, gcur2, out->t,
-		                    l1, part_segs{hstart, HB - cbits, slices, fbits}, TupBucket<TUP>{64 - Tt, (1u << fbits) - 1u}));
+		                    l1, part_segs{hstart, HB - cbits, slices, fbits, seg_end, lim2 ? (const u32*) tstart : (const u32*) nullptr, over}, TupBucket<TUP>{64 - Tt, (1u << fbits) - 1u}));
 	}
 	return VDJX_OK;
 }
 
 template <typename TUP, typename A>
-int stage_gated_partition(vdjx_ctx* c, A& db, const vdjx_pool* pool, u64 rec_base, int k, size_t per_bucket, u64 geometry_instances, GTuples<TUP>* out, bool sym = false) {
+int stage_gated_partition(vdjx_ctx* c, A& db, const vdjx_pool* pool, u64 rec_base, int k, size_t per_bucket, u64 geometry_instances, GTuples<TUP>* out, bool sym = false, u32 S = 1) {
 	GatedHist gh;
-	int rc = stage_gated_hist(c, db, pool, k, per_bucket, geometry_instances, &gh, sym);
+	int rc = stage_gated_hist(c, db, pool, k, per_bucket, geometry_instances, &gh, sym, S);
 	if (rc) return rc;
 	return stage_gated_cut<TUP>(c, db, pool, rec_base, k, per_bucket, geometry_instances, gh, out);
 }
@@ -2116,12 +2224,12 @@
 	*order = nullptr;
 	if (t.NB < 1024) return VDJX_OK;
 	HIP_TRY(db.alloc(order, t.NB));
-	hipLaunchKernelGGL(k_bucket_order, dim3(1), dim3(1024), 0, c->stream, t.bucket_start, t.NB, *order);
+	hipLaunchKernelGGL(k_bucket_order, dim3(1), dim3(1024), 0, c->stream, t.bucket_start, t.bucket_end, t.NB, *order);
 	return VDJX_OK;
 }
 
 template <typename TUP, typename A>
-int stage_gated_reduce(vdjx_ctx* c, A& db, const GTuples<TUP>& t, const PoolView& pv, u64 rec_base, int k, int mf, int mq, SurvivorsG* sv, bool sym = false) {
+int stage_gated_reduce(vdjx_ctx* c, A& db, GTuples<TUP>& t, const PoolView& pv, u64 rec_base, int k, int mf, int mq, SurvivorsG* sv, bool sym = false) {
 	hipStream_t st = c->stream;
 	int rc = set_sub_tuples(c);
 	if (rc) return rc;
@@ -2130,33 +2238,40 @@
 	const u32 tlow = 1 + (mqq + 19) / 20;
 	const u32 cmin = (u32) std::max(mf, 2);
 	const u32 mfu = (u32) std::max(mf, 0);
-	const u32 cap = (sym ? t.N : t.N / 2) + 16;
+	const u32 cap = (sym ? t.Nsurv : t.Nsurv / 2) + 16;
 	u32 *g_err, *n_surv;
 	u64* g_distinct;
 	HIP_TRY(db.alloc(&sv->lo, cap)); HIP_TRY(db.alloc(&sv->hi, cap)); HIP_TRY(db.alloc(&sv->gcnt, cap)); HIP_TRY(db.alloc(&sv->gfirst, cap));
-	HIP_TRY(db.alloc(&g_distinct, 64 * 16 + 2));
+	HIP_TRY(db.alloc(&g_distinct, 64 * 16 + 3));
 	g_err = (u32*) (g_distinct + 64 * 16);
 	n_surv = g_err + 1;
 	u32* n_real = g_err + 2;
-	HIP_TRY(hipMemsetAsync(g_distinct, 0, (64 * 16 + 2) * 8, st));
+	HIP_TRY(hipMemsetAsync(g_distinct, 0, (64 * 16 + 3) * 8, st));
+	if (t.over) hipLaunchKernelGGL(k_cut_totals, dim3((t.NB + 1023) / 1024), dim3(1024), 0, st, t.bucket_start, t.bucket_end, t.NB, (const u32*) t.over, g_err + 3,
+	                               (unsigned long long*) (g_distinct + 64 * 16 + 2));
 	SurvOutG so{sv->lo, sv->hi, sv->gcnt, sv->gfirst, n_surv, cap, n_real};
 	static const u32 rd_dbg = (u32) vdjx_env_num("VDJX_RD_DBG", 0, 0, 9);
 	if (t.N) {
 		vdjx_prof_scope ps(c, "k_gated_reduce");
 		u32* order;
 		if ((rc = bucket_order(c, db, t, &order))) return rc;
-		if (sym) hipLaunchKernelGGL((k_gated_reduce<TUP, true>), dim3(t.NB), dim3(RD_THREADS), 0, st, t.t, t.bucket_start, pv.bases, pv.nmask, pv.quals, pv.rl, pv.ob, k, rec_base,
+		if (sym) hipLaunchKernelGGL((k_gated_reduce<TUP, true>), dim3(t.NB), dim3(RD_THREADS), 0, st, t.t, t.bucket_start, t.bucket_end, (const u32*) t.over, pv.bases, pv.nmask, pv.quals, pv.rl, pv.ob, k, rec_base,
 		                            mfu, cmin, mqq, tlow, so, g_distinct, g_err, rd_dbg, (const u32*) order);
-		else hipLaunchKernelGGL(k_gated_reduce<TUP>, dim3(t.NB), dim3(RD_THREADS), 0, st, t.t, t.bucket_start, pv.bases, pv.nmask, pv.quals, pv.rl, pv.ob, k, rec_base,
+		else hipLaunchKernelGGL(k_gated_reduce<TUP>, dim3(t.NB), dim3(RD_THREADS), 0, st, t.t, t.bucket_start, t.bucket_end, (const u32*) t.over, pv.bases, pv.nmask, pv.quals, pv.rl, pv.ob, k, rec_base,
 		                        mfu, cmin, mqq, tlow, so, g_distinct, g_err, rd_dbg, (const u32*) order);
 	}
 	u64* spread = (u64*) c->h_pin;
 	u32* tail = (u32*) (spread + 64 * 16);
-	static_assert((64 * 16 + 2) * 8 == VDJX_HPIN_SYNC_BYTES, "h_pin layout (vdjx_common.h)");
+	static_assert((64 * 16 + 3) * 8 == VDJX_HPIN_SYNC_BYTES, "h_pin layout (vdjx_common.h)");
 	HIP_TRY(hipMemcpyAsync(spread, g_distinct, VDJX_HPIN_SYNC_BYTES, hipMemcpyDeviceToHost, st));
 	HIP_TRY(hipStreamSynchronize(st));
 	HIP_TRY(hipGetLastError());
 	const u32 ns = tail[1], err = tail[0];
+	if (t.over) {
+		if (tail[3] || ns > cap) return VDJX_ECUT;
+		t.N = (u32) spread[64 * 16 + 2];
+		c->stats["gated_instances"] = sym ? 2ull * t.N : t.N;
+	}
 	if (err) { vdjx_set_error("k_gated_reduce: %u buckets could not be split to fit LDS", err); return VDJX_EHIP; }
 	if (ns > cap) { vdjx_set_error("survivor capacity logic failed (%u > %u)", ns, cap); return VDJX_EHIP; }
 	sv->ndist = 0;
@@ -2555,11 +2670,27 @@
 	GTuples<TUP> t;
 	const bool sym = build_sym(pool, k);
 	c->stats["kmer_build_sym"] = sym ? 1 : 0;
-	int rc = stage_gated_partition<TUP>(c, db, pool, 0, k, 0, 0, &t, sym);
-	if (rc) return rc;
 	PoolView pv{pool->d_bases, pool->d_nmask, vdjx_qrows{pool->d_quals, pool->d_quals2, pool->q_split, pool->qstride}, pool->rl, pool->ob};
 	SurvivorsG sv;
-	rc = stage_gated_reduce<TUP>(c, db, t, pv, 0, k, mf, mq, &sv, sym);
+	u32 S = cut_sample_stride(pool, sym ? pool->n_records / 2 : pool->n_records);
+	c->stats["kmer_build_cut_retries"] += 0;
+	const vdjx_arena::mark_t cut_mark = db.mark();
+	int rc;
+	for (bool first = true;; first = false) {
+		t = GTuples<TUP>();
+		sv = SurvivorsG();
+		rc = stage_gated_partition<TUP>(c, db, pool, 0, k, 0, 0, &t, sym, S);
+		if (rc) return rc;
+		if (first) c->stats["kmer_build_cut_sample"] = t.S;
+		rc = stage_gated_reduce<TUP>(c, db, t, pv, 0, k, mf, mq, &sv, sym);
+		if (rc != VDJX_ECUT || S == 1) break;
+		c->stats["kmer_build_cut_retries"] += 1;
+		fprintf(stderr, "[vdjx] k-mer build: a bucket ran over the capacity its sample of one row in %u gave it; cutting again from the exact histogram\n", S);
+		vdjx_clear_errors();
+		db.release_to(cut_mark);
+		S = 1;
+	}
+	if (rc == VDJX_ECUT) { vdjx_set_error("k-mer build: the exact cut reports buckets over their capacity"); return VDJX_EHIP; }
 	if (rc) return rc;
 	vdjx_ri_open_gate(c);
 	dbg_sync(c, "gated_reduce");
@@ -2754,9 +2885,9 @@
 		vdjx_prof_scope ps(c, "k_gated_local");
 		u32* order;
 		if ((rc = bucket_order(c, db, t, &order))) return rc;
-		if (s->sym) hipLaunchKernelGGL((k_gated_local<TUP, true>), dim3(t.NB), dim3(LG_THREADS), 0, st, t.t, t.bucket_start, s->pool->d_bases, s->pool->d_nmask, rec_base,
+		if (s->sym) hipLaunchKernelGGL((k_gated_local<TUP, true>), dim3(t.NB), dim3(LG_THREADS), 0, st, t.t, t.bucket_start, t.bucket_end, s->pool->d_bases, s->pool->d_nmask, rec_base,
 		                               s->k, s->pool->rl, s->pool->ob, s->tlow, sparse, sparse_ref, s->nd, s->low_inst, g_err, (const u32*) order);
-		else hipLaunchKernelGGL(k_gated_local<TUP>, dim3(t.NB), dim3(LG_THREADS), 0, st, t.t, t.bucket_start, s->pool->d_bases, s->pool->d_nmask, rec_base,
+		else hipLaunchKernelGGL(k_gated_local<TUP>, dim3(t.NB), dim3(LG_THREADS), 0, st, t.t, t.bucket_start, t.bucket_end, s->pool->d_bases, s->pool->d_nmask, rec_base,
 		                        s->k, s->pool->rl, s->pool->ob, s->tlow, sparse, sparse_ref, s->nd, s->low_inst, g_err, (const u32*) order);
 	}
 	vdjx_scan_one(st, s->nd, s->NBf, s->dstart);
diff --git a/vdjer_amd/csrc/vdjx_part.h b/vdjer_amd/csrc/vdjx_part.h
--- a/vdjer_amd/csrc/vdjx_part.h
+++ b/vdjer_amd/csrc/vdjx_part.h
@@ -10,6 +10,7 @@
 #define PART_SLICES 8u
 #define PART_NONE 0xFFFFFFFFu
 #define PART_HOLE 0xFFFFFFFFFFFFFFFFull
+#define PART_DEAD 0xFFFFFFFFu
 
 namespace {
 
@@ -40,20 +41,38 @@
 
 struct part_round {
 	u32 cnt[PART_MAXB], base[PART_MAXB + 1], cur[PART_MAXB], gbase[PART_MAXB], tmp[PART_THREADS];
+	u32 end[PART_MAXB];
+	u32* over;
+	u32 dead, stop;
+
+	__device__ inline bool limits(u32 nbk, const u32* __restrict__ lim, u32 lsh, u32* word, const u32* seen = nullptr) {
+		if (lim) for (u32 i = threadIdx.x; i < nbk; i += PART_THREADS) end[i] = lim[((size_t) i + 1) << lsh];
+		if (threadIdx.x == 0) {
+			over = lim ? word : nullptr;
+			stop = seen ? __hip_atomic_load(seen, __ATOMIC_RELAXED, __HIP_MEMORY_SCOPE_AGENT) : 0u;
+		}
+		__syncthreads();
+		return stop != 0;
+	}
 
 	__device__ inline void begin(u32 nbk) {
 		for (u32 i = threadIdx.x; i < nbk; i += PART_THREADS) cnt[i] = 0;
+		if (threadIdx.x == 0) dead = 0;
 		__syncthreads();
 	}
 	__device__ inline void count(u32 b) { atomicAdd(&cnt[b], 1u); }
 	__device__ inline u32 reserve(u32 nbk, u32* __restrict__ gcur) {
 		part_scan(cnt, base, tmp, nbk);
+		u32* const word = over;
 		for (u32 i = threadIdx.x; i < nbk; i += PART_THREADS) {
 			cur[i] = base[i];
-			gbase[i] = cnt[i] ? atomicAdd(&gcur[i], cnt[i]) : 0u;
+			const u32 n = cnt[i];
+			const u32 g = n ? atomicAdd(&gcur[i], n) : 0u;
+			gbase[i] = g;
+			if (word && (u64) g + n > (u64) end[i]) { dead = 1; atomicExch(word, 1u); }
 		}
 		__syncthreads();
-		return base[nbk];
+		return dead ? PART_DEAD : base[nbk];
 	}
 	__device__ inline u32 slot(u32 b) { return atomicAdd(&cur[b], 1u); }
 	template <typename T, typename Key> __device__ inline void flush(const T* stage, u32 n, T* __restrict__ out, const Key& key) {
@@ -66,9 +85,9 @@
 	}
 };
 
-__device__ inline u32 part_slice(const u32* __restrict__ seg_start, u32 seg_shift, u32 slices, size_t& t0, size_t& t1) {
+__device__ inline u32 part_slice(const u32* __restrict__ seg_start, u32 seg_shift, u32 slices, size_t& t0, size_t& t1, const u32* __restrict__ seg_end = nullptr) {
 	const u32 seg = blockIdx.x / slices, sl = blockIdx.x % slices;
-	const size_t s0 = seg_start[(size_t) seg << seg_shift], s1 = seg_start[((size_t) seg + 1) << seg_shift];
+	const size_t s0 = seg_start[(size_t) seg << seg_shift], s1 = seg_end ? seg_end[seg] : seg_start[((size_t) seg + 1) << seg_shift];
 	const size_t per = (s1 - s0 + slices - 1) / slices;
 	t0 = s0 + (size_t) sl * per;
 	t1 = t0 + per < s1 ? t0 + per : s1;
@@ -86,14 +105,21 @@
 		buckets = nbk;
 		return 0;
 	}
+	__device__ inline const u32* limits(size_t) const { return nullptr; }
+	__device__ inline u32* over_word() const { return nullptr; }
 };
 struct part_segs {
 	const u32* seg_start;
 	u32 seg_shift, slices, sub_bits;
+	const u32* seg_end = nullptr;
+	const u32* lim = nullptr;
+	u32* over = nullptr;
 	__device__ inline size_t span(u32, size_t& t0, size_t& t1, u32& buckets) const {
 		buckets = 1u << sub_bits;
-		return (size_t) part_slice(seg_start, seg_shift, slices, t0, t1) << sub_bits;
+		return (size_t) part_slice(seg_start, seg_shift, slices, t0, t1, seg_end) << sub_bits;
 	}
+	__device__ inline const u32* limits(size_t first) const { return lim ? lim + first : nullptr; }
+	__device__ inline u32* over_word() const { return over; }
 };
 
 template <typename T, typename Key, typename Range, bool PAIRED = false>
@@ -106,7 +132,9 @@
 	static_assert(!PAIRED || (std::is_same<T, u64>::value && PER % 2 == 0), "the paired loads are for 8-byte elements");
 	size_t t0, t1;
 	u32 nbk;
-	u32* gc = gcur + range.span(ROUND, t0, t1, nbk);
+	const size_t first = range.span(ROUND, t0, t1, nbk);
+	u32* gc = gcur + first;
+	if (pr.limits(nbk, range.limits(first), 0u, range.over_word(), range.over_word())) return;
 	for (size_t ts = t0; ts < t1; ts += ROUND) {
 		const size_t te = ts + ROUND < t1 ? ts + ROUND : t1;
 		pr.begin(nbk);
@@ -137,6 +165,7 @@
 		}
 		__syncthreads();
 		const u32 n = pr.reserve(nbk, gc);
+		if (n == PART_DEAD) return;
 #pragma unroll
 		for (u32 j = 0; j < PER; j++) if (r_b[j] != PART_NONE) part_store(&stage[pr.slot(r_b[j])], r_x[j]);
 		__syncthreads();
```
